# ruiminshen/yolo2-pytorch

Measured on NVIDIA H100. Metric: 416x416 images/sec, higher is better.
Workload: dtype f16

## Files before the change

### include/yolo2_b200.h

```cpp
#ifndef YOLO2_B200_H_
#define YOLO2_B200_H_

#ifdef __cplusplus
extern "C" {
#endif

typedef void* yb_stream_t;

#define YB_ERR_BAD_ARG (-1)
#define YB_ERR_UNSUPPORTED (-2)
#define YB_ERR_DRIVER (-3)

#define YB_OUT_F16_NHWC 0
#define YB_OUT_F32_NCHW 1
#define YB_CONV_A_TILED 1
#define YB_CONV_WIDE_N 2
#define YB_CONV_FORCE_BN(bn) ((bn) << 8)
#define YB_CONV_POOL2X2 16
#define YB_CONV_C32_IM2COL 32
#define YB_CONV_NO_STREAMK 8
#define YB_CONV_FORCE_STREAMK (1 << 30)
#define YB_CONV_NO_SMALLK (1 << 28)
#define YB_CONV_PLAIN_STORE (1 << 29)
#define YB_FILTER_THRESHOLD 0
#define YB_FILTER_FIX 1
#define YB_FILTER_NONE 2

int yb_version(void);
const char* yb_last_error(void);
int yb_debug_read(int out[4]);
int yb_conv_set_trace(void* dev_buf);

int yb_pack_weight_f16(const float* w_oihw, void* w_f16, int cout, int cin, int ksize, int mode, yb_stream_t stream);
int yb_bn_fold(const float* gamma, const float* beta, const float* running_mean, const float* running_var, float eps, float* scale,
               float* shift, int channels, yb_stream_t stream);

int yb_conv0_bn_leaky_pool_fwd(const float* x_nchw, const float* w_oihw, const float* scale, const float* shift, float slope,
                               void* y_nhwc_f16, int batch, int height, int width, int cout, yb_stream_t stream);
int yb_conv0_u8_bn_leaky_pool_fwd(const unsigned char* x_nhwc_u8, const float* w_oihw, const float* scale, const float* shift,
                                  float slope, void* y_nhwc_f16, int batch, int height, int width, int cout, yb_stream_t stream);
int yb_conv_bn_act_fwd(const void* x, const void* w, const float* scale, const float* shift, float slope, void* y, int batch,
                       int height, int width, int cin, int cout, int ksize, int x_ld, long long y_ld, int y_ch_off, int out_mode,
                       int flags, yb_stream_t stream);
int yb_conv_bn_act_stats_fwd(const void* x, const void* w, const float* scale, const float* shift, float slope, void* y, int batch,
                             int height, int width, int cin, int cout, int ksize, int x_ld, long long y_ld, int y_ch_off, int flags,
                             double* sums, yb_stream_t stream);
long long yb_conv_workspace_bytes(void);
int yb_conv_choice(int batch, int height, int width, int cin, int cout, int ksize, int out_mode, int flags, int with_workspace, int out[6]);
int yb_conv_bn_act_fwd_ws(const void* x, const void* w, const float* scale, const float* shift, float slope, void* y, int batch,
                          int height, int width, int cin, int cout, int ksize, int x_ld, long long y_ld, int y_ch_off, int out_mode,
                          int flags, void* workspace, long long workspace_bytes, yb_stream_t stream);
int yb_conv_bn_act_split_fwd(const void* x, const void* w_split, const float* scale, const float* shift, float slope, void* y, int batch,
                             int height, int width, int k_channels, int a_channels, int cout, int ksize, int x_ld, long long y_ld,
                             int y_ch_off, int lo_ch_off, int out_mode, int flags, void* workspace, long long workspace_bytes,
                             yb_stream_t stream);
int yb_pack_weight_split_f16(const float* w_oihw, void* w_f16, int cout, int cin, int ksize, int segments, int lo_mask, yb_stream_t stream);
int yb_maxpool2x2_split_f16(const void* x, void* y, int batch, int height, int width, int channels, int x_ld, int x_lo_off, int y_ld,
                            int y_lo_off, yb_stream_t stream);
int yb_conv_ref_fwd(const void* x, const void* w, const float* scale, const float* shift, float slope, void* y, int batch, int height,
                    int width, int cin, int cout, int ksize, int x_ld, long long y_ld, int y_ch_off, int out_mode, yb_stream_t stream);
int yb_maxpool2x2_f16(const void* x, void* y, int batch, int height, int width, int channels, int x_ld, yb_stream_t stream);
int yb_maxpool2x2_s1_f16(const void* x, void* y, int batch, int height, int width, int channels, int x_ld, yb_stream_t stream);
int yb_maxpool2x2_s1_bwd_f16(const void* x, const void* dy, void* dx, int batch, int height, int width, int channels, yb_stream_t stream);
int yb_reorg_f16(const void* x, void* y, int batch, int height, int width, int channels, int x_ld, int y_ld, int y_ch_off,
                 yb_stream_t stream);
int yb_reorg_f32_nchw(const float* x, float* y, int batch, int channels, int height, int width, int stride_h, int stride_w,
                      yb_stream_t stream);

int yb_decode_fwd(const float* feature, const float* anchors_hw, float* iou, float* center_offset, float* size_norm, float* yx_min,
                  float* yx_max, float* logits, float* prob, int batch, int rows, int cols, int num_anchors, int num_cls,
                  yb_stream_t stream);

int yb_filter_nms(const float* score, const float* yx_min, const float* yx_max, const float* prob, int batch, int n, int num_cls,
                  int mode, float threshold, float threshold_cls, float overlap, int limit, int* n_filtered, int* n_keep,
                  int* keep_idx, int* keep_box, int* n_det, int* det_keep, int* det_cls, float* det_score, int det_cap,
                  int* filt_box, int* best_cls, float* best_prob, yb_stream_t stream);
int yb_iou_matrix(const float* yx_min1, const float* yx_max1, const float* yx_min2, const float* yx_max2, float* out, int batch,
                  int n1, int n2, float min_union, yb_stream_t stream);

int yb_region_loss_fwd(const float* feature, const float* anchors_hw, const float* gt_yx_min, const float* gt_yx_max,
                       const long long* gt_cls, int batch, int rows, int cols, int num_anchors, int num_cls, int num_gt, float threshold,
                       int cross_entropy, float* losses, unsigned char* positive, unsigned char* negative, float* best_iou, int* pos_count,
                       float* partial, float* grad_terms, float* grad_bg, yb_stream_t stream);
int yb_region_loss_bwd(const float* grad_terms, const float* grad_bg, const float* weights5, float* dfeature, int batch, int rows, int cols,
                       int num_anchors, int num_cls, yb_stream_t stream);

int yb_conv0_raw_fwd(const float* x_nchw, const float* w_oihw, void* z_nhwc_f16, int batch, int height, int width, int cout,
                     yb_stream_t stream);
int yb_conv0_raw_stats_fwd(const float* x_nchw, const float* w_oihw, void* z_nhwc_f16, double* sums, int batch, int height, int width, int cout,
                           yb_stream_t stream);
int yb_pack_weight_dgrad_f16(const float* w_oihw, void* w_f16, int cout, int cin, int ksize, int cout_pad, yb_stream_t stream);
typedef struct yb_pack_unit {
  const float* w_oihw;
  void* out_fwd;
  void* out_dgrad;
  int cout, cin, ksize, cout_pad, block0, ci_blocks;
} yb_pack_unit;
int yb_pack_weights_batch(const yb_pack_unit* units_dev, int num_units, int total_blocks, yb_stream_t stream);
int yb_bn_stats(const void* z, long long ld, long long rows, int channels, double* sums, yb_stream_t stream);
int yb_bn_finalize(double* sums, long long rows, int channels, float eps, float momentum, float* running_mean, float* running_var,
                   float* mean, float* invstd, yb_stream_t stream);
int yb_bn_act_apply(const void* z, long long ld_z, const float* mean, const float* invstd, const float* gamma, const float* beta,
                    float slope, void* a, long long ld_a, int a_ch_off, int batch, int height, int width, int channels, int pool,
                    yb_stream_t stream);
int yb_bn_act_bwd(int mode, const void* z, long long ld_z, const float* mean, const float* invstd, const float* gamma, const float* beta,
                  float slope, const void* da, long long ld_da, int da_off, const void* dap, long long ld_dap, int dap_off, int batch,
                  int height, int width, int channels, int window, double* sums, void* dz, long long ld_dz, int has_bn, yb_stream_t stream);
int yb_bn_param_grad(double* sums, int channels, float* dgamma, float* dbeta, int reset, float scale, yb_stream_t stream);
int yb_reorg_bwd_f16(const void* dy, long long ld_dy, int dy_off, void* dx, int batch, int height, int width, int channels,
                     yb_stream_t stream);
int yb_head_grad_prepare(const float* dfeature, void* dz_nhwc_f16, float* dbias, int batch, int channels, int channels_pad, int cells,
                         yb_stream_t stream);
int yb_conv0_wgrad(const float* x_nchw, const void* dz_nhwc_f16, float* dw_oihw, int batch, int height, int width, yb_stream_t stream);
int yb_conv0_wgrad_bn(const float* x_nchw, const void* z_nhwc_f16, const void* dap, long long ld_dap, int dap_off, const float* mean, const float* invstd,
                      const float* gamma, const float* beta, float slope, const double* sums, float* dw_oihw, int batch, int height, int width,
                      yb_stream_t stream);
int yb_conv_wgrad(const void* x, const void* dz, float* dw_krsc, int batch, int height, int width, int cin, int cout, int ksize, int x_ld,
                  int dz_ld, yb_stream_t stream);
int yb_unpack_wgrad(const float* dw_krsc, float* dw_oihw, int cout, int cin, int ksize, float scale, yb_stream_t stream);

int yb_grad_guard(float* grads, long long count, float* found_inf, int zero_if_found, yb_stream_t stream);

int yb_resize_batch_u8(const void* src, const long long* src_off, const int* src_hw, void* dst, int batch, int height, int width, int swap_rb,
                       float* yx_min, float* yx_max, int slots, yb_stream_t stream);

int yb_resize_aug_batch_u8(const void* src, const long long* src_off, const int* src_hw, const int* crop, const float* margin, const unsigned char* flip,
                           void* dst, int batch, int height, int width, int swap_rb, float* yx_min, float* yx_max, int slots, yb_stream_t stream);

int yb_warp_affine_u8(const void* src, int src_h, int src_w, void* dst, int dst_h, int dst_w, const double* inverse_matrix6, const int* fill3,
                      yb_stream_t stream);

int yb_totensor_u8(const void* src_nhwc_u8, float* dst_nchw_f32, int batch, int height, int width, yb_stream_t stream);

#define YB_PH_BLUR 1
#define YB_PH_SWAP 2
#define YB_PH_BGR2HSV 3
#define YB_PH_HSV2RGB 4
#define YB_PH_LUT 5
int yb_photometric_batch_u8(const void* src, void* dst, int batch, int height, int width, const void* params, int param_stride, int stages,
                            yb_stream_t stream);

int yb_eval_match(const float* det_yx_min, const float* det_yx_max, const int* det_cls, const int* det_off, const float* gt_yx_min,
                  const float* gt_yx_max, const int* gt_cls, const int* gt_off, int batch, int num_cls, int max_gt, float threshold, float min_union,
                  unsigned char* tp, yb_stream_t stream);

int yb_mb_conv0_bn_relu_fwd(const float* x_nchw, const float* w_oihw, const float* scale, const float* shift, void* y_nhwc_f16, int batch,
                            int height, int width, yb_stream_t stream);
int yb_dwconv3x3_bn_relu_fwd(const void* x, const float* w_c9, const float* scale, const float* shift, void* y, int batch, int height,
                             int width, int channels, int stride, yb_stream_t stream);

int yb_stem7x7_bn_relu_fwd(const float* x_nchw, const float* w_oihw, const float* scale, const float* shift, void* y_nhwc_f16, int batch, int height, int width,
                           yb_stream_t stream);
int yb_maxpool3x3_s2_f16(const void* x, void* y, int batch, int height, int width, int channels, yb_stream_t stream);
int yb_subsample2_f16(const void* x, void* y, int batch, int height, int width, int channels, yb_stream_t stream);
int yb_add_relu_f16(const void* a, const void* b, void* out, long long count, yb_stream_t stream);

int yb_conv1x1_preact_fwd(const void* x, const void* w, const float* pre_scale, const float* pre_shift, int pre_relu, const float* scale,
                          const float* shift, float slope, void* y, int batch, int height, int width, int cin, int cout, int x_ld, long long y_ld,
                          int y_ch_off, int out_mode, int flags, void* workspace, long long workspace_bytes, yb_stream_t stream);
int yb_bn_relu_avgpool2x2_f16(const void* x, int x_ld, const float* scale, const float* shift, void* y, int batch, int height, int width,
                              int channels, yb_stream_t stream);
int yb_maxpool3x3_s2_ld_f16(const void* x, void* y, int y_ld, int y_ch_off, int batch, int height, int width, int channels, yb_stream_t stream);

int yb_stem7x7_raw_fwd(const float* x_nchw, const float* w_oihw, void* z_nhwc_f16, int batch, int height, int width, yb_stream_t stream);
int yb_stem7x7_wgrad(const float* x_nchw, const void* dz_nhwc_f16, float* dw_oihw, int batch, int height, int width, yb_stream_t stream);
int yb_maxpool3x3_s2_bwd_f16(const void* x, const void* dy, void* dx, int batch, int height, int width, int channels, yb_stream_t stream);
int yb_upsample2_zero_f16(const void* x, void* y, int batch, int height, int width, int channels, yb_stream_t stream);
int yb_residual_bwd_f16(const void* y, const void* g_a, const void* g_b, int stride_b, void* out, int batch, int height, int width, int channels,
                        yb_stream_t stream);

int yb_mb_conv0_split_fwd(const float* x_nchw, const float* w_oihw, const float* scale, const float* shift, void* y_hi_lo, int batch, int height, int width,
                          yb_stream_t stream);
int yb_dwconv3x3_split_fwd(const void* x_hi_lo, const float* w_c9, const float* scale, const float* shift, void* y_hi_lo, int batch, int height, int width,
                           int channels, int stride, yb_stream_t stream);
int yb_mb_conv0_raw_fwd(const float* x_nchw, const float* w_oihw, void* z_nhwc_f16, int batch, int height, int width, yb_stream_t stream);
int yb_mb_conv0_wgrad(const float* x_nchw, const void* dz_nhwc_f16, float* dw_oihw, int batch, int height, int width, yb_stream_t stream);
int yb_dwconv3x3_raw_fwd(const void* x, const float* w_c9, void* z, int batch, int height, int width, int channels, int stride, yb_stream_t stream);
int yb_dwconv3x3_dgrad(const void* dz, const float* w_c9, void* da, int batch, int height, int width, int channels, int stride, yb_stream_t stream);
int yb_dwconv3x3_wgrad(const void* a, const void* dz, float* dw_c9, int batch, int height, int width, int channels, int stride, yb_stream_t stream);

int yb_comm_version(int* nccl_version);
int yb_comm_unique_id(void* id128);
int yb_comm_init(void** comm, int nranks, const void* id128, int rank);
int yb_comm_destroy(void* comm);
int yb_allreduce_bucket(void* comm, void* buf, long long count, int dtype, yb_stream_t stream);
int yb_broadcast_buffer(void* comm, void* buf, long long count, int dtype, int root, yb_stream_t stream);

#ifdef __cplusplus
}
#endif
#endif
```

### yolo2-pytorch_b200/b200/engine.py

```python
import os

import torch

from . import ops

STRICT_KEEP = {'layers1.0': 'aw', 'layers1.2': 'aw', 'layers1.4': 'a', 'passthrough': 'aw', 'layers3.0': 'aw'}
PRECISIONS = ('fast', 'strict')


class ConvUnit(object):

    def __init__(self, conv, bn, act):
        self.conv, self.bn, self.act = conv, bn, act
        self._wver = None
        self._bver = None
        self.w16 = self.scale = self.shift = None
        self.split_a = self.split_w = False
        self.out_lo = False

    @property
    def cout(self):
        return self.conv.weight.shape[0]

    @property
    def cin(self):
        return self.conv.weight.shape[1]

    @property
    def ksize(self):
        return self.conv.weight.shape[2]

    @property
    def slope(self):
        return 0.1 if self.act else 1.0

    def refresh(self, first_layer=False, force=False):
        w = self.conv.weight
        wver = (w.data_ptr(), w._version)
        wver = wver + (self.split_a, self.split_w)
        if force or wver != self._wver:
            if first_layer:
                self.w16 = w.detach().contiguous()
            elif self.split_a or self.split_w:
                self.w16 = ops.pack_weight_split_f16(w.detach().contiguous(), self.split_a, self.split_w)
            else:
                self.w16 = ops.pack_weight_f16(w.detach().contiguous(), 0)
            self._wver = wver
        if self.bn is not None:
            ts = (self.bn.weight, self.bn.bias, self.bn.running_mean, self.bn.running_var)
            bver = tuple((t.data_ptr(), t._version) for t in ts)
            if bver != self._bver:
                self.scale, self.shift = ops.bn_fold(*(t.detach().contiguous() for t in ts), eps=self.bn.eps)
                self._bver = bver
        else:
            b = self.conv.bias
            bver = None if b is None else (b.data_ptr(), b._version)
            if bver != self._bver or self.scale is None:
                self.scale = torch.ones(self.cout, dtype=torch.float32, device=w.device)
                self.shift = (b.detach().float().contiguous().clone() if b is not None
                              else torch.zeros(self.cout, dtype=torch.float32, device=w.device))
                self._bver = bver


class StrictPlan(object):

    def __init__(self, eng, batch, height, width, device):
        f16 = dict(dtype=torch.float16, device=device)

        def buf(u, h, w):
            return torch.empty(batch, h, w, u.cout * (2 if u.out_lo else 1), **f16)

        h, w = height // 2, width // 2
        self.a0 = torch.empty(batch, h, w, eng.units1[0].cout, **f16)
        self.l1 = []
        for u, pooled in zip(eng.units1[1:], eng.pools1[1:]):
            out = buf(u, h, w)
            if pooled:
                h, w = h // 2, w // 2
                self.l1.append((out, buf(u, h, w)))
            else:
                self.l1.append((out, None))
        self.pt = buf(eng.unit_pt, h, w)
        h, w = h // 2, w // 2
        self.x1_pool = buf(eng.units1[-1], h, w)
        self.cat_c = eng.unit_pt.cout * 4 + eng.units2[-1].cout
        self.cat = torch.empty(batch, h, w, self.cat_c * (2 if eng.units3[0].split_a else 1), **f16)
        self.l2 = [buf(u, h, w) for u in eng.units2[:-1]]
        self.l3 = buf(eng.units3[0], h, w)
        self.feature = torch.empty(batch, eng.units3[1].cout, h, w, dtype=torch.float32, device=device)
        self.workspace = ops.conv_workspace(device)


class DarknetPlan(object):

    def __init__(self, units1, units2, unit_pt, units3, pools1, batch, height, width, device):
        f16 = dict(dtype=torch.float16, device=device)
        self.batch, self.height, self.width = batch, height, width
        h, w = height // 2, width // 2
        self.a0 = torch.empty(batch, h, w, units1[0].cout, **f16)
        self.l1 = []
        for u, pooled in zip(units1[1:], pools1[1:]):
            out = torch.empty(batch, h, w, u.cout, **f16)
            if pooled:
                h, w = h // 2, w // 2
                self.l1.append((out, torch.empty(batch, h, w, u.cout, **f16)))
            else:
                self.l1.append((out, None))
        self.h16, self.w16 = h, w
        self.pt = torch.empty(batch, h, w, unit_pt.cout, **f16)
        self.x1_pool = torch.empty(batch, h // 2, w // 2, units1[-1].cout, **f16)
        h, w = h // 2, w // 2
        self.h32, self.w32 = h, w
        self.cat_ch = unit_pt.cout * 4 + units2[-1].cout
        self.cat = torch.empty(batch, h, w, self.cat_ch, **f16)
        self.l2 = [torch.empty(batch, h, w, u.cout, **f16) for u in units2[:-1]]
        self.l3 = torch.empty(batch, h, w, units3[0].cout, **f16)
        self.feature = torch.empty(batch, units3[1].cout, h, w, dtype=torch.float32, device=device)
        self.workspace = ops.conv_workspace(device)


class DarknetEngine(object):
    def __init__(self, dnn):
        def unit(m):
            return ConvUnit(m.conv, m.bn if m.has_bn else None, m.has_act)

        self.units1, self.pools1, self._k1 = [], [], []
        mods = list(dnn.layers1)
        for i, m in enumerate(mods):
            if m.is_pool:
                continue
            self.units1.append(unit(m))
            self.pools1.append(i + 1 < len(mods) and mods[i + 1].is_pool)
            self._k1.append('layers1.%d' % i)
        self.units2 = [unit(m) for m in dnn.layers2 if not m.is_pool]
        self._k2 = ['layers2.%d' % i for i, m in enumerate(dnn.layers2) if not m.is_pool]
        self.unit_pt = unit(dnn.passthrough)
        self.units3 = [unit(m) for m in dnn.layers3]
        self.plans = {}
        if not self.pools1[0]:
            raise RuntimeError('Darknet: layers1.0 must be followed by MaxPool2d (fused first-layer kernel)')
        self.precision = 'fast'
        self.set_precision(os.environ.get('YB_PRECISION', 'fast'))

    def unit_keys(self):
        return self._k1 + self._k2 + ['passthrough', 'layers3.0', 'layers3.1']

    def set_precision(self, precision, keep=None):
        if precision not in PRECISIONS:
            raise ValueError('precision must be one of %s' % (PRECISIONS,))
        keep = STRICT_KEEP if keep is None else keep
        units = dict(zip(self.unit_keys(), self.all_units()))
        for key, u in units.items():
            k = keep.get(key, '') if precision == 'strict' else 'aw'
            u.split_a, u.split_w, u.out_lo = 'a' not in k, 'w' not in k, False
        units[self._k1[0]].split_a = units[self._k1[0]].split_w = False
        units[self._k1[1]].split_a = False
        chain1 = self.units1
        for prev, nxt in zip(chain1[:-1], chain1[1:]):
            prev.out_lo = nxt.split_a
        chain1[-1].out_lo = self.unit_pt.split_a or self.units2[0].split_a
        for prev, nxt in zip(self.units2[:-1], self.units2[1:]):
            prev.out_lo = nxt.split_a
        self.units2[-1].out_lo = self.unit_pt.out_lo = self.units3[0].split_a
        self.units3[0].out_lo = self.units3[1].split_a
        chain1[0].out_lo = False
        self.precision = precision
        self.plans = {}
        self.invalidate()

    def all_units(self):
        return self.units1 + self.units2 + [self.unit_pt] + self.units3

    def plan(self, batch, height, width, device, plan_id=0):
        key = (batch, height, width, str(device), plan_id)
        p = self.plans.get(key)
        if p is None and self.precision == 'strict':
            p = self.plans[key] = StrictPlan(self, batch, height, width, device)
        if p is None:
            p = DarknetPlan(self.units1, self.units2, self.unit_pt, self.units3, self.pools1, batch, height, width, device)
            self.plans[key] = p
        return p

    def refresh(self, force=False):
        for i, u in enumerate(self.all_units()):
            u.refresh(first_layer=(i == 0), force=force)

    def invalidate(self):
        for u in self.all_units():
            u._wver = None
            u._bver = None

    def forward(self, x, conv_flags=0, ref=False, collect=None, plan_id=0):
        if not x.is_cuda:
            raise RuntimeError('Darknet: input must be a CUDA tensor; there is no CPU fallback')
        u8 = x.dtype == torch.uint8
        if u8:
            b, h, w, c = x.shape
        else:
            b, c, h, w = x.shape
        if c != 3 or h % 32 or w % 32:
            raise ValueError('Darknet expects fp32 [B,3,H,W] or uint8 [B,H,W,3] with H, W multiples of 32, got %s' % (tuple(x.shape),))
        x = x.contiguous() if u8 else x.contiguous().float()
        self.refresh()
        p = self.plan(b, h, w, x.device, plan_id)
        if self.precision == 'strict':
            return self._forward_strict(x, u8, p, conv_flags, collect)

        def conv(u, src, dst, **kw):
            return ops.conv_bn_act(src, u.w16, u.scale, u.shift, u.slope, out=dst, flags=conv_flags, ref=ref, workspace=p.workspace, **kw)

        u0 = self.units1[0]
        conv0 = ops.conv0_u8_bn_leaky_pool if u8 else ops.conv0_bn_leaky_pool
        cur = conv0(x, u0.w16, u0.scale, u0.shift, u0.slope, out=p.a0)
        if collect is not None:
            collect['layers1.0(pooled)'] = cur
        x1 = None
        last1 = self.units1[-1]
        for u, (out, pooled), key in zip(self.units1[1:], p.l1, self._k1[1:]):
            fuse_pool = (pooled is not None and u is not last1 and collect is None and not ref and u.cin == 32 and u.ksize == 3
                         and u.cout <= 64 and (conv_flags & (ops.CONV_NO_SMALLK | ops.CONV_C32_IM2COL)) == 0 and conv_flags < 256)
            if fuse_pool:
                ops.conv_bn_act(cur, u.w16, u.scale, u.shift, u.slope, out=pooled, flags=conv_flags | ops.CONV_POOL2X2)
                cur = pooled
                continue
            conv(u, cur, out)
            if collect is not None:
                collect[key] = out
            x1 = out
            cur = ops.maxpool2x2(out, out=pooled) if pooled is not None else out
        conv(self.unit_pt, x1, p.pt)
        if collect is not None:
            collect['passthrough'] = p.pt
        ops.reorg_f16(p.pt, p.cat, 0)
        cur = ops.maxpool2x2(x1, out=p.x1_pool)
        for u, out, key in zip(self.units2[:-1], p.l2, self._k2):
            conv(u, cur, out)
            if collect is not None:
                collect[key] = out
            cur = out
        conv(self.units2[-1], cur, p.cat, y_ch_off=self.unit_pt.cout * 4)
        conv(self.units3[0], p.cat, p.l3)
        conv(self.units3[1], p.l3, p.feature, out_mode=ops.OUT_F32_NCHW)
        if collect is not None:
            collect['cat'] = p.cat
            collect['layers3.0'] = p.l3
        return p.feature

    def _forward_strict(self, x, u8, p, conv_flags, collect):
        def view(t, c, lo):
            return (t[..., :c].float() + t[..., c:2 * c].float()) if lo else t[..., :c]

        def conv(u, src, src_c, src_lo, dst, y_ch_off=0, lo_ch_off=None, out_mode=ops.OUT_F16_NHWC):
            split_a = u.split_a and src_lo
            if lo_ch_off is None:
                lo_ch_off = y_ch_off + u.cout if u.out_lo else -1
            if not (split_a or u.split_w or lo_ch_off >= 0):
                return ops.conv_bn_act(src, u.w16, u.scale, u.shift, u.slope, out=dst, flags=conv_flags, workspace=p.workspace, cin=src_c,
                                       y_ch_off=y_ch_off, out_mode=out_mode)
            if u.split_a and not src_lo:
                raise RuntimeError('strict plan: unit expects [hi | lo] input')
            return ops.conv_bn_act_split(src, u.w16, u.scale, u.shift, u.slope, dst, a_channels=src_c * (2 if split_a else 1), y_ch_off=y_ch_off,
                                         lo_ch_off=lo_ch_off, out_mode=out_mode, flags=conv_flags, workspace=p.workspace)

        u0 = self.units1[0]
        conv0 = ops.conv0_u8_bn_leaky_pool if u8 else ops.conv0_bn_leaky_pool
        cur, cur_c, cur_lo = conv0(x, u0.w16, u0.scale, u0.shift, u0.slope, out=p.a0), u0.cout, False
        if collect is not None:
            collect['layers1.0(pooled)'] = cur
        x1 = None
        for u, (out, pooled), key in zip(self.units1[1:], p.l1, self._k1[1:]):
            plain = not (u.split_a or u.split_w or u.out_lo)
            if (plain and pooled is not None and collect is None and u.cin == 32 and u.ksize == 3 and u.cout <= 64 and conv_flags == 0):
                ops.conv_bn_act(cur, u.w16, u.scale, u.shift, u.slope, out=pooled, flags=ops.CONV_POOL2X2)
                cur, cur_c, cur_lo = pooled, u.cout, False
                continue
            conv(u, cur, cur_c, cur_lo, out)
            if collect is not None:
                collect[key] = view(out, u.cout, u.out_lo)
            x1, x1_c, x1_lo = out, u.cout, u.out_lo
            cur, cur_c, cur_lo = out, u.cout, u.out_lo
            if pooled is not None:
                cur = ops.maxpool2x2_split(out, u.cout, pooled) if u.out_lo else ops.maxpool2x2(out, out=pooled)
        cat_lo = self.units3[0].split_a
        upt = self.unit_pt
        conv(upt, x1, x1_c, x1_lo, p.pt)
        if collect is not None:
            collect['passthrough'] = view(p.pt, upt.cout, upt.out_lo)
        ops.reorg_f16(p.pt, p.cat, 0, channels=upt.cout)
        if cat_lo:
            ops.reorg_f16(p.pt, p.cat, p.cat_c, channels=upt.cout, x_ch_off=upt.cout)
        last1 = self.units1[-1]
        cur = ops.maxpool2x2_split(x1, last1.cout, p.x1_pool) if last1.out_lo else ops.maxpool2x2(x1, out=p.x1_pool)
        cur_c, cur_lo = last1.cout, last1.out_lo
        for u, out, key in zip(self.units2[:-1], p.l2, self._k2):
            conv(u, cur, cur_c, cur_lo, out)
            if collect is not None:
                collect[key] = view(out, u.cout, u.out_lo)
            cur, cur_c, cur_lo = out, u.cout, u.out_lo
        u27 = self.units2[-1]
        conv(u27, cur, cur_c, cur_lo, p.cat, y_ch_off=upt.cout * 4, lo_ch_off=(p.cat_c + upt.cout * 4) if cat_lo else -1)
        u30, u31 = self.units3
        conv(u30, p.cat, p.cat_c, cat_lo, p.l3)
        conv(u31, p.l3, u30.cout, u30.out_lo, p.feature, out_mode=ops.OUT_F32_NCHW, lo_ch_off=-1)
        if collect is not None:
            collect['cat'] = view(p.cat, p.cat_c, cat_lo)
            collect['layers3.0'] = view(p.l3, u30.cout, u30.out_lo)
        return p.feature
```

### yolo2-pytorch_b200/b200/lib.py

```python
import ctypes
import os

_HERE = os.path.dirname(os.path.abspath(__file__))
LIB_PATH = os.environ.get('YB_LIB_PATH') or os.path.join(os.path.dirname(_HERE), 'libyolo2_b200.so')

c_int, c_float, c_void_p, c_longlong = ctypes.c_int, ctypes.c_float, ctypes.c_void_p, ctypes.c_longlong
P = c_void_p

SIGNATURES = {
    'yb_version': [],
    'yb_debug_read': [ctypes.POINTER(c_int * 4)],
    'yb_conv_set_trace': [P],
    'yb_pack_weight_f16': [P, P, c_int, c_int, c_int, c_int, P],
    'yb_bn_fold': [P, P, P, P, c_float, P, P, c_int, P],
    'yb_conv0_bn_leaky_pool_fwd': [P, P, P, P, c_float, P, c_int, c_int, c_int, c_int, P],
    'yb_conv0_u8_bn_leaky_pool_fwd': [P, P, P, P, c_float, P, c_int, c_int, c_int, c_int, P],
    'yb_conv_bn_act_fwd': [P, P, P, P, c_float, P, c_int, c_int, c_int, c_int, c_int, c_int, c_int, c_longlong, c_int, c_int, c_int, P],
    'yb_conv_bn_act_stats_fwd': [P, P, P, P, c_float, P, c_int, c_int, c_int, c_int, c_int, c_int, c_int, c_longlong, c_int, c_int, P, P],
    'yb_conv_workspace_bytes': [],
    'yb_conv_choice': [c_int, c_int, c_int, c_int, c_int, c_int, c_int, c_int, c_int, ctypes.POINTER(c_int * 6)],
    'yb_conv_bn_act_fwd_ws': [P, P, P, P, c_float, P, c_int, c_int, c_int, c_int, c_int, c_int, c_int, c_longlong, c_int, c_int, c_int, P,
                              c_longlong, P],
    'yb_conv_bn_act_split_fwd': [P, P, P, P, c_float, P, c_int, c_int, c_int, c_int, c_int, c_int, c_int, c_int, c_longlong, c_int, c_int, c_int,
                                 c_int, P, c_longlong, P],
    'yb_pack_weight_split_f16': [P, P, c_int, c_int, c_int, c_int, c_int, P],
    'yb_maxpool2x2_split_f16': [P, P, c_int, c_int, c_int, c_int, c_int, c_int, c_int, c_int, P],
    'yb_conv_ref_fwd': [P, P, P, P, c_float, P, c_int, c_int, c_int, c_int, c_int, c_int, c_int, c_longlong, c_int, c_int, P],
    'yb_maxpool2x2_f16': [P, P, c_int, c_int, c_int, c_int, c_int, P],
    'yb_maxpool2x2_s1_f16': [P, P, c_int, c_int, c_int, c_int, c_int, P],
    'yb_maxpool2x2_s1_bwd_f16': [P, P, P, c_int, c_int, c_int, c_int, P],
    'yb_reorg_f16': [P, P, c_int, c_int, c_int, c_int, c_int, c_int, c_int, P],
    'yb_reorg_f32_nchw': [P, P, c_int, c_int, c_int, c_int, c_int, c_int, P],
    'yb_decode_fwd': [P, P, P, P, P, P, P, P, P, c_int, c_int, c_int, c_int, c_int, P],
    'yb_filter_nms': [P, P, P, P, c_int, c_int, c_int, c_int, c_float, c_float, c_float, c_int, P, P, P, P, P, P, P, P, c_int, P, P, P, P],
    'yb_iou_matrix': [P, P, P, P, P, c_int, c_int, c_int, c_float, P],
    'yb_region_loss_fwd': [P, P, P, P, P, c_int, c_int, c_int, c_int, c_int, c_int, c_float, c_int, P, P, P, P, P, P, P, P, P],
    'yb_region_loss_bwd': [P, P, P, P, c_int, c_int, c_int, c_int, c_int, P],
    'yb_conv0_raw_fwd': [P, P, P, c_int, c_int, c_int, c_int, P],
    'yb_conv0_raw_stats_fwd': [P, P, P, P, c_int, c_int, c_int, c_int, P],
    'yb_pack_weight_dgrad_f16': [P, P, c_int, c_int, c_int, c_int, P],
    'yb_pack_weights_batch': [P, c_int, c_int, P],
    'yb_bn_stats': [P, c_longlong, c_longlong, c_int, P, P],
    'yb_bn_finalize': [P, c_longlong, c_int, c_float, c_float, P, P, P, P, P],
    'yb_bn_act_apply': [P, c_longlong, P, P, P, P, c_float, P, c_longlong, c_int, c_int, c_int, c_int, c_int, c_int, P],
    'yb_bn_act_bwd': [c_int, P, c_longlong, P, P, P, P, c_float, P, c_longlong, c_int, P, c_longlong, c_int, c_int, c_int, c_int, c_int, c_int,
                      P, P, c_longlong, c_int, P],
    'yb_bn_param_grad': [P, c_int, P, P, c_int, c_float, P],
    'yb_reorg_bwd_f16': [P, c_longlong, c_int, P, c_int, c_int, c_int, c_int, P],
    'yb_head_grad_prepare': [P, P, P, c_int, c_int, c_int, c_int, P],
    'yb_conv0_wgrad': [P, P, P, c_int, c_int, c_int, P],
    'yb_conv0_wgrad_bn': [P, P, P, c_longlong, c_int, P, P, P, P, c_float, P, P, c_int, c_int, c_int, P],
    'yb_conv_wgrad': [P, P, P, c_int, c_int, c_int, c_int, c_int, c_int, c_int, c_int, P],
    'yb_unpack_wgrad': [P, P, c_int, c_int, c_int, c_float, P],
    'yb_grad_guard': [P, c_longlong, P, c_int, P],
    'yb_resize_batch_u8': [P, P, P, P, c_int, c_int, c_int, c_int, P, P, c_int, P],
    'yb_resize_aug_batch_u8': [P, P, P, P, P, P, P, c_int, c_int, c_int, c_int, P, P, c_int, P],
    'yb_warp_affine_u8': [P, c_int, c_int, P, c_int, c_int, ctypes.POINTER(ctypes.c_double * 6), ctypes.POINTER(c_int * 3), P],
    'yb_totensor_u8': [P, P, c_int, c_int, c_int, P],
    'yb_photometric_batch_u8': [P, P, c_int, c_int, c_int, P, c_int, c_int, P],
    'yb_eval_match': [P, P, P, P, P, P, P, P, c_int, c_int, c_int, c_float, c_float, P, P],
    'yb_mb_conv0_raw_fwd': [P, P, P, c_int, c_int, c_int, P],
    'yb_mb_conv0_split_fwd': [P, P, P, P, P, c_int, c_int, c_int, P],
    'yb_dwconv3x3_split_fwd': [P, P, P, P, P, c_int, c_int, c_int, c_int, c_int, P],
    'yb_mb_conv0_wgrad': [P, P, P, c_int, c_int, c_int, P],
    'yb_dwconv3x3_raw_fwd': [P, P, P, c_int, c_int, c_int, c_int, c_int, P],
    'yb_dwconv3x3_dgrad': [P, P, P, c_int, c_int, c_int, c_int, c_int, P],
    'yb_dwconv3x3_wgrad': [P, P, P, c_int, c_int, c_int, c_int, c_int, P],
    'yb_stem7x7_bn_relu_fwd': [P, P, P, P, P, c_int, c_int, c_int, P],
    'yb_maxpool3x3_s2_f16': [P, P, c_int, c_int, c_int, c_int, P],
    'yb_subsample2_f16': [P, P, c_int, c_int, c_int, c_int, P],
    'yb_add_relu_f16': [P, P, P, c_longlong, P],
    'yb_stem7x7_raw_fwd': [P, P, P, c_int, c_int, c_int, P],
    'yb_stem7x7_wgrad': [P, P, P, c_int, c_int, c_int, P],
    'yb_maxpool3x3_s2_bwd_f16': [P, P, P, c_int, c_int, c_int, c_int, P],
    'yb_upsample2_zero_f16': [P, P, c_int, c_int, c_int, c_int, P],
    'yb_residual_bwd_f16': [P, P, P, c_int, P, c_int, c_int, c_int, c_int, P],
    'yb_comm_version': [ctypes.POINTER(c_int)],
    'yb_comm_unique_id': [P],
    'yb_comm_init': [ctypes.POINTER(P), c_int, P, c_int],
    'yb_comm_destroy': [P],
    'yb_allreduce_bucket': [P, P, c_longlong, c_int, P],
    'yb_broadcast_buffer': [P, P, c_longlong, c_int, c_int, P],
    'yb_mb_conv0_bn_relu_fwd': [P, P, P, P, P, c_int, c_int, c_int, P],
    'yb_dwconv3x3_bn_relu_fwd': [P, P, P, P, P, c_int, c_int, c_int, c_int, c_int, P],
    'yb_conv1x1_preact_fwd': [P, P, P, P, c_int, P, P, c_float, P, c_int, c_int, c_int, c_int, c_int, c_int, c_longlong, c_int, c_int, c_int, P,
                              c_longlong, P],
    'yb_bn_relu_avgpool2x2_f16': [P, c_int, P, P, P, c_int, c_int, c_int, c_int, P],
    'yb_maxpool3x3_s2_ld_f16': [P, P, c_int, c_int, c_int, c_int, c_int, c_int, P],
}

_lib = None


def load():
    global _lib
    if _lib is not None:
        return _lib
    if not os.path.exists(LIB_PATH):
        raise ImportError(
            'libyolo2_b200.so not found at %s -- build it with `python yolo2-pytorch_b200/build.py` '
            '(nvcc, sm_90a).  There is no CPU or PyTorch fallback for this path.' % LIB_PATH)
    lib = ctypes.CDLL(LIB_PATH)
    for name, argtypes in SIGNATURES.items():
        fn = getattr(lib, name)
        fn.argtypes = argtypes
        fn.restype = c_longlong if name == 'yb_conv_workspace_bytes' else c_int
    lib.yb_last_error.argtypes = []
    lib.yb_last_error.restype = ctypes.c_char_p
    _lib = lib
    return lib


def last_error():
    return load().yb_last_error().decode('utf-8', 'replace')


def debug_read():
    buf = (c_int * 4)()
    load().yb_debug_read(ctypes.byref(buf))
    return list(buf)


def check(rc, what):
    if rc != 0:
        raise RuntimeError('%s failed (code %d): %s' % (what, rc, last_error()))
```

### yolo2-pytorch_b200/b200/ops.py

```python
import ctypes

import torch

from . import lib as _l

OUT_F16_NHWC, OUT_F32_NCHW = 0, 1
CONV_A_TILED, CONV_WIDE_N = 1, 2
CONV_NO_STREAMK, CONV_FORCE_STREAMK, CONV_NO_SMALLK, CONV_PLAIN_STORE = 8, 1 << 30, 1 << 28, 1 << 29
CONV_POOL2X2, CONV_C32_IM2COL, CONV_C32_SWAP = 16, 32, 64
FILTER_THRESHOLD, FILTER_FIX, FILTER_NONE = 0, 1, 2


launch_count = 0


def _ck(rc, what):
    global launch_count
    _l.check(rc, what)
    launch_count += 1


def conv_force_bn(bn):
    return bn << 8


def conv_force_mt(mt):
    return mt << 20


def conv_force_pair(v):
    return v << 22


CONV_ALLOW_PAIR = 4


def _p(t):
    return None if t is None else ctypes.c_void_p(t.data_ptr())


def _s():
    return ctypes.c_void_p(torch.cuda.current_stream().cuda_stream)


def _req(t, dtype, name):
    if not (isinstance(t, torch.Tensor) and t.is_cuda):
        raise RuntimeError('%s must be a CUDA tensor: the GPU path has no CPU fallback' % name)
    if t.dtype != dtype:
        raise TypeError('%s must be %s, got %s' % (name, dtype, t.dtype))
    if not t.is_contiguous():
        raise ValueError('%s must be contiguous' % name)
    return t


def pack_weight_f16(w, mode=0):
    _req(w, torch.float32, 'weight')
    cout, cin, k, _ = w.shape
    shape = (cout, k, k, cin) if mode == 0 else (cin, k, k, cout)
    out = torch.empty(shape, dtype=torch.float16, device=w.device)
    _ck(_l.load().yb_pack_weight_f16(_p(w), _p(out), cout, cin, k, mode, _s()), 'yb_pack_weight_f16')
    return out


SPLIT_SEGMENTS = {(True, False): (2, 0b00), (False, True): (2, 0b10), (True, True): (3, 0b100)}


def pack_weight_split_f16(w, split_a, split_w):
    _req(w, torch.float32, 'weight')
    cout, cin, k, _ = w.shape
    segments, lo_mask = SPLIT_SEGMENTS[(bool(split_a), bool(split_w))]
    out = torch.empty(cout, k, k, segments * cin, dtype=torch.float16, device=w.device)
    _ck(_l.load().yb_pack_weight_split_f16(_p(w), _p(out), cout, cin, k, segments, lo_mask, _s()), 'yb_pack_weight_split_f16')
    return out


def bn_fold(gamma, beta, mean, var, eps=1e-5):
    for n, t in (('gamma', gamma), ('beta', beta), ('mean', mean), ('var', var)):
        _req(t, torch.float32, n)
    c = gamma.numel()
    scale = torch.empty(c, dtype=torch.float32, device=gamma.device)
    shift = torch.empty_like(scale)
    _ck(_l.load().yb_bn_fold(_p(gamma), _p(beta), _p(mean), _p(var), float(eps), _p(scale), _p(shift), c, _s()), 'yb_bn_fold')
    return scale, shift


def conv0_bn_leaky_pool(x, w, scale, shift, slope, out=None):
    _req(x, torch.float32, 'x'); _req(w, torch.float32, 'w'); _req(scale, torch.float32, 'scale'); _req(shift, torch.float32, 'shift')
    b, c, h, wd = x.shape
    if c != 3:
        raise ValueError('conv0 expects 3 input channels')
    cout = w.shape[0]
    if out is None:
        out = torch.empty(b, h // 2, wd // 2, cout, dtype=torch.float16, device=x.device)
    _req(out, torch.float16, 'out')
    _ck(_l.load().yb_conv0_bn_leaky_pool_fwd(_p(x), _p(w), _p(scale), _p(shift), float(slope), _p(out), b, h, wd, cout, _s()),
             'yb_conv0_bn_leaky_pool_fwd')
    return out


def conv0_u8_bn_leaky_pool(x, w, scale, shift, slope, out=None):
    _req(x, torch.uint8, 'x'); _req(w, torch.float32, 'w'); _req(scale, torch.float32, 'scale'); _req(shift, torch.float32, 'shift')
    b, h, wd, c = x.shape
    if c != 3:
        raise ValueError('conv0 expects 3 input channels')
    cout = w.shape[0]
    if out is None:
        out = torch.empty(b, h // 2, wd // 2, cout, dtype=torch.float16, device=x.device)
    _req(out, torch.float16, 'out')
    _ck(_l.load().yb_conv0_u8_bn_leaky_pool_fwd(_p(x), _p(w), _p(scale), _p(shift), float(slope), _p(out), b, h, wd, cout, _s()),
        'yb_conv0_u8_bn_leaky_pool_fwd')
    return out


def _conv_common(fn_name, x, w, scale, shift, slope, out, batch, height, width, cin, cout, k, x_ld, y_ld, y_ch_off, out_mode, flags,
                 workspace=None):
    if workspace is not None and fn_name == 'yb_conv_bn_act_fwd':
        fn_name = 'yb_conv_bn_act_fwd_ws'
    fn = getattr(_l.load(), fn_name)
    args = [_p(x), _p(w), _p(scale), _p(shift), float(slope), _p(out), batch, height, width, cin, cout, k, x_ld, y_ld, y_ch_off, out_mode]
    if fn_name != 'yb_conv_ref_fwd':
        args.append(flags)
    if fn_name == 'yb_conv_bn_act_fwd_ws':
        _req(workspace, torch.uint8, 'workspace')
        args += [_p(workspace), workspace.numel()]
    args.append(_s())
    _ck(fn(*args), fn_name)


def conv_workspace(device='cuda'):
    return torch.zeros(int(_l.load().yb_conv_workspace_bytes()), dtype=torch.uint8, device=device)


CONV_KERNELS = ('conv_igemm_kernel', 'conv_wide_kernel', 'conv_c32_kernel')


def conv_choice(batch, height, width, cin, cout, k, out_mode=OUT_F16_NHWC, flags=0, workspace=True):
    out = (ctypes.c_int * 6)()
    _l.check(_l.load().yb_conv_choice(batch, height, width, cin, cout, k, out_mode, flags, int(bool(workspace)), ctypes.byref(out)),
             'yb_conv_choice')
    return dict(kernel=CONV_KERNELS[out[0]], bk=out[1], bn=out[2], rows=out[3], streamk=bool(out[4]), grid=out[5])


def conv_bn_act(x, w, scale, shift, slope, out=None, out_mode=OUT_F16_NHWC, y_ch_off=0, cin=None, flags=0, ref=False, workspace=None):
    _req(x, torch.float16, 'x'); _req(w, torch.float16, 'w'); _req(scale, torch.float32, 'scale'); _req(shift, torch.float32, 'shift')
    b, h, wd, x_ld = x.shape
    cout, k, _, wcin = w.shape
    cin = wcin if cin is None else cin
    if cin != wcin:
        raise ValueError('weight Cin %d != %d' % (wcin, cin))
    if out is None:
        oh, ow = (h // 2, wd // 2) if (flags & CONV_POOL2X2) else (h, wd)
        out = (torch.empty(b, oh, ow, cout, dtype=torch.float16, device=x.device) if out_mode == OUT_F16_NHWC
               else torch.empty(b, cout, h, wd, dtype=torch.float32, device=x.device))
    if out_mode == OUT_F16_NHWC:
        _req(out, torch.float16, 'out')
        y_ld = out.shape[-1]
    else:
        _req(out, torch.float32, 'out')
        y_ld = 0
    _conv_common('yb_conv_ref_fwd' if ref else 'yb_conv_bn_act_fwd', x, w, scale, shift, slope, out, b, h, wd, cin, cout, k, x_ld, y_ld,
                 y_ch_off, out_mode, flags, workspace=None if ref else workspace)
    return out


def conv1x1_preact(x, w, pre_scale, pre_shift, pre_relu, scale, shift, slope, out=None, out_mode=OUT_F16_NHWC, y_ch_off=0, cin=None, flags=0,
                   workspace=None):
    _req(x, torch.float16, 'x'); _req(w, torch.float16, 'w'); _req(scale, torch.float32, 'scale'); _req(shift, torch.float32, 'shift')
    _req(pre_scale, torch.float32, 'pre_scale'); _req(pre_shift, torch.float32, 'pre_shift')
    b, h, wd, x_ld = x.shape
    cout, k, _, wcin = w.shape
    cin = wcin if cin is None else cin
    if cin != wcin or k != 1:
        raise ValueError('conv1x1_preact: weight [%d,%d,%d,%d] does not match a 1x1 conv over %d channels' % (cout, k, k, wcin, cin))
    if pre_scale.numel() < cin or pre_shift.numel() < cin:
        raise ValueError('conv1x1_preact: pre_scale / pre_shift need %d channels' % cin)
    if out is None:
        out = (torch.empty(b, h, wd, cout, dtype=torch.float16, device=x.device) if out_mode == OUT_F16_NHWC
               else torch.empty(b, cout, h, wd, dtype=torch.float32, device=x.device))
    if out_mode == OUT_F16_NHWC:
        _req(out, torch.float16, 'out')
        y_ld = out.shape[-1]
    else:
        _req(out, torch.float32, 'out')
        y_ld = 0
    ws_ptr, ws_bytes = (None, 0) if workspace is None else (_p(_req(workspace, torch.uint8, 'workspace')), workspace.numel())
    _ck(_l.load().yb_conv1x1_preact_fwd(_p(x), _p(w), _p(pre_scale), _p(pre_shift), int(bool(pre_relu)), _p(scale), _p(shift), float(slope),
                                        _p(out), b, h, wd, cin, cout, x_ld, y_ld, y_ch_off, out_mode, flags, ws_ptr, ws_bytes, _s()),
        'yb_conv1x1_preact_fwd')
    return out


def conv_bn_act_split(x, w, scale, shift, slope, out, a_channels, y_ch_off=0, lo_ch_off=-1, out_mode=OUT_F16_NHWC, flags=0, workspace=None):
    _req(x, torch.float16, 'x'); _req(w, torch.float16, 'w'); _req(scale, torch.float32, 'scale'); _req(shift, torch.float32, 'shift')
    b, h, wd, x_ld = x.shape
    cout, k, _, kch = w.shape
    if out_mode == OUT_F16_NHWC:
        _req(out, torch.float16, 'out')
        y_ld = out.shape[-1]
    else:
        _req(out, torch.float32, 'out')
        y_ld = 0
    ws_ptr, ws_bytes = (None, 0) if workspace is None else (_p(_req(workspace, torch.uint8, 'workspace')), workspace.numel())
    _ck(_l.load().yb_conv_bn_act_split_fwd(_p(x), _p(w), _p(scale), _p(shift), float(slope), _p(out), b, h, wd, kch, int(a_channels), cout, k, x_ld,
                                           y_ld, y_ch_off, lo_ch_off, out_mode, flags, ws_ptr, ws_bytes, _s()), 'yb_conv_bn_act_split_fwd')
    return out


def maxpool2x2_split(x, channels, out):
    _req(x, torch.float16, 'x'); _req(out, torch.float16, 'out')
    b, h, w, x_ld = x.shape
    _ck(_l.load().yb_maxpool2x2_split_f16(_p(x), _p(out), b, h, w, channels, x_ld, channels, out.shape[-1], channels, _s()), 'yb_maxpool2x2_split_f16')
    return out


def conv_bn_act_stats(x, w, scale, shift, slope, sums, out=None, flags=0):
    _req(x, torch.float16, 'x'); _req(w, torch.float16, 'w'); _req(scale, torch.float32, 'scale'); _req(shift, torch.float32, 'shift')
    _req(sums, torch.float64, 'sums')
    b, h, wd, x_ld = x.shape
    cout, k, _, cin = w.shape
    if sums.numel() != 2 * cout:
        raise ValueError('sums must hold 2 * Cout doubles')
    if out is None:
        out = torch.empty(b, h, wd, cout, dtype=torch.float16, device=x.device)
    _req(out, torch.float16, 'out')
    _ck(_l.load().yb_conv_bn_act_stats_fwd(_p(x), _p(w), _p(scale), _p(shift), float(slope), _p(out), b, h, wd, cin, cout, k, x_ld, out.shape[-1], 0,
                                           flags, _p(sums), _s()), 'yb_conv_bn_act_stats_fwd')
    return out


def maxpool2x2(x, channels=None, out=None):
    _req(x, torch.float16, 'x')
    b, h, w, x_ld = x.shape
    c = x_ld if channels is None else channels
    if out is None:
        out = torch.empty(b, h // 2, w // 2, c, dtype=torch.float16, device=x.device)
    _req(out, torch.float16, 'out')
    _ck(_l.load().yb_maxpool2x2_f16(_p(x), _p(out), b, h, w, c, x_ld, _s()), 'yb_maxpool2x2_f16')
    return out


def maxpool2x2_s1(x, out=None):
    _req(x, torch.float16, 'x')
    b, h, w, c = x.shape
    if out is None:
        out = torch.empty_like(x)
    _req(out, torch.float16, 'out')
    _ck(_l.load().yb_maxpool2x2_s1_f16(_p(x), _p(out), b, h, w, c, c, _s()), 'yb_maxpool2x2_s1_f16')
    return out


def reorg_f16(x, out, y_ch_off=0, channels=None, x_ch_off=0):
    _req(x, torch.float16, 'x'); _req(out, torch.float16, 'out')
    b, h, w, x_ld = x.shape
    c = x_ld if channels is None else channels
    if x_ch_off % 8 or x_ch_off + c > x_ld:
        raise ValueError('reorg: bad channel slice')
    xp = ctypes.c_void_p(x.data_ptr() + 2 * x_ch_off)
    _ck(_l.load().yb_reorg_f16(xp, _p(out), b, h, w, c, x_ld, out.shape[-1], y_ch_off, _s()), 'yb_reorg_f16')
    return out


def reorg_f32_nchw(x, stride_h=2, stride_w=2):
    _req(x, torch.float32, 'x')
    b, c, h, w = x.shape
    out = torch.empty(b, c * stride_h * stride_w, h // stride_h, w // stride_w, dtype=torch.float32, device=x.device)
    if out.numel():
        _ck(_l.load().yb_reorg_f32_nchw(_p(x), _p(out), b, c, h, w, stride_h, stride_w, _s()), 'yb_reorg_f32_nchw')
    return out


def decode(feature, anchors, num_cls, with_prob=True):
    _req(feature, torch.float32, 'feature'); _req(anchors, torch.float32, 'anchors')
    b, ch, rows, cols = feature.shape
    a = anchors.shape[0]
    cells = rows * cols
    dev = feature.device
    out = dict(
        iou=torch.empty(b, cells, a, dtype=torch.float32, device=dev),
        center_offset=torch.empty(b, cells, a, 2, dtype=torch.float32, device=dev),
        size_norm=torch.empty(b, cells, a, 2, dtype=torch.float32, device=dev),
        yx_min=torch.empty(b, cells, a, 2, dtype=torch.float32, device=dev),
        yx_max=torch.empty(b, cells, a, 2, dtype=torch.float32, device=dev),
    )
    logits = prob = None
    if num_cls > 1:
        logits = out['logits'] = torch.empty(b, cells, a, num_cls, dtype=torch.float32, device=dev)
    if with_prob:
        prob = out['prob'] = torch.empty(b, cells, a, max(num_cls, 1), dtype=torch.float32, device=dev)
    if ch != a * (5 + (num_cls if num_cls > 1 else 0)):
        raise ValueError('feature has %d channels, expected %d' % (ch, a * (5 + (num_cls if num_cls > 1 else 0))))
    _ck(_l.load().yb_decode_fwd(_p(feature), _p(anchors), _p(out['iou']), _p(out['center_offset']), _p(out['size_norm']),
                                     _p(out['yx_min']), _p(out['yx_max']), _p(logits), _p(prob), b, rows, cols, a, num_cls, _s()),
             'yb_decode_fwd')
    return out


def filter_nms(score, yx_min, yx_max, prob, mode, threshold, threshold_cls, overlap, limit=200, expand=False, details=False):
    _req(score, torch.float32, 'score'); _req(yx_min, torch.float32, 'yx_min'); _req(yx_max, torch.float32, 'yx_max')
    if prob is not None:
        _req(prob, torch.float32, 'prob')
    b, n = score.shape
    num_cls = prob.shape[-1] if prob is not None else 1
    dev = score.device
    i32 = dict(dtype=torch.int32, device=dev)
    res = dict(n_filtered=torch.empty(b, **i32), n_keep=torch.empty(b, **i32),
               keep_idx=torch.empty(b, limit, **i32), keep_box=torch.empty(b, limit, **i32))
    n_det = det_keep = det_cls = det_score = None
    det_cap = 0
    if expand:
        det_cap = limit * num_cls
        n_det = res['n_det'] = torch.empty(b, **i32)
        det_keep = res['det_keep'] = torch.empty(b, det_cap, **i32)
        det_cls = res['det_cls'] = torch.empty(b, det_cap, **i32)
        det_score = res['det_score'] = torch.empty(b, det_cap, dtype=torch.float32, device=dev)
    filt_box = best_cls = best_prob = None
    if details:
        filt_box = res['filt_box'] = torch.empty(b, n, **i32)
        if prob is not None:
            best_cls = res['best_cls'] = torch.empty(b, n, **i32)
            best_prob = res['best_prob'] = torch.empty(b, n, dtype=torch.float32, device=dev)
    _ck(_l.load().yb_filter_nms(_p(score), _p(yx_min), _p(yx_max), _p(prob), b, n, num_cls, mode, float(threshold),
                                     float(threshold_cls), float(overlap), limit, _p(res['n_filtered']), _p(res['n_keep']),
                                     _p(res['keep_idx']), _p(res['keep_box']), _p(n_det), _p(det_keep), _p(det_cls), _p(det_score),
                                     det_cap, _p(filt_box), _p(best_cls), _p(best_prob), _s()), 'yb_filter_nms')
    return res


def iou_matrix(yx_min1, yx_max1, yx_min2, yx_max2, min_union=1.1920928955078125e-07):
    for n, t in (('yx_min1', yx_min1), ('yx_max1', yx_max1), ('yx_min2', yx_min2), ('yx_max2', yx_max2)):
        _req(t, torch.float32, n)
    batched = yx_min1.dim() == 3
    b = yx_min1.shape[0] if batched else 1
    n1, n2 = yx_min1.shape[-2], yx_min2.shape[-2]
    out = torch.empty((b, n1, n2) if batched else (n1, n2), dtype=torch.float32, device=yx_min1.device)
    _ck(_l.load().yb_iou_matrix(_p(yx_min1), _p(yx_max1), _p(yx_min2), _p(yx_max2), _p(out), b, n1, n2, float(min_union), _s()),
             'yb_iou_matrix')
    return out


def region_loss_forward(feature, anchors, gt_yx_min, gt_yx_max, gt_cls, threshold, cross_entropy=True):
    _req(feature, torch.float32, 'feature'); _req(anchors, torch.float32, 'anchors')
    _req(gt_yx_min, torch.float32, 'gt_yx_min'); _req(gt_yx_max, torch.float32, 'gt_yx_max')
    b, ch, rows, cols = feature.shape
    a = anchors.shape[0]
    per = ch // a
    num_cls = per - 5 if per > 5 else 1
    g = gt_yx_min.shape[1]
    if num_cls > 1:
        _req(gt_cls, torch.int64, 'gt_cls')
    cells = rows * cols
    dev = feature.device
    out = dict(losses=torch.empty(5, dtype=torch.float32, device=dev),
               positive=torch.empty(b, cells, a, dtype=torch.uint8, device=dev),
               negative=torch.empty(b, cells, a, dtype=torch.uint8, device=dev),
               best_iou=torch.empty(b, cells, a, dtype=torch.float32, device=dev),
               grad_terms=torch.empty_like(feature),
               grad_bg=torch.empty(b, a, cells, dtype=torch.float32, device=dev))
    pos_count = torch.empty(b, dtype=torch.int32, device=dev)
    partial = torch.empty(b * 5, dtype=torch.float32, device=dev)
    _ck(_l.load().yb_region_loss_fwd(_p(feature), _p(anchors), _p(gt_yx_min), _p(gt_yx_max), _p(gt_cls if num_cls > 1 else None), b, rows,
                                     cols, a, num_cls, g, float(threshold), int(bool(cross_entropy)), _p(out['losses']),
                                     _p(out['positive']), _p(out['negative']), _p(out['best_iou']), _p(pos_count), _p(partial),
                                     _p(out['grad_terms']), _p(out['grad_bg']), _s()), 'yb_region_loss_fwd')
    out['pos_count'] = pos_count
    return out


def region_loss_backward(grad_terms, grad_bg, weights5, num_anchors):
    _req(grad_terms, torch.float32, 'grad_terms'); _req(grad_bg, torch.float32, 'grad_bg'); _req(weights5, torch.float32, 'weights5')
    b, ch, rows, cols = grad_terms.shape
    per = ch // num_anchors
    num_cls = per - 5 if per > 5 else 1
    out = torch.empty_like(grad_terms)
    _ck(_l.load().yb_region_loss_bwd(_p(grad_terms), _p(grad_bg), _p(weights5), _p(out), b, rows, cols, num_anchors, num_cls, _s()),
        'yb_region_loss_bwd')
    return out


def call(name, *args):
    conv = [(_p(a) if isinstance(a, torch.Tensor) or a is None else a) for a in args]
    _ck(getattr(_l.load(), name)(*conv, _s()), name)
```

### yolo2-pytorch_b200/b200/pipeline.py

```python
import torch

from . import ops


class DetectPipeline(object):
    RESULT_KEYS = ('n_filtered', 'n_keep', 'keep_box', 'n_det', 'det_keep', 'det_cls', 'det_score', 'best_cls', 'iou', 'yx_min', 'yx_max')

    def __init__(self, inference, config, batch, height, width, slots=2, lanes=1, use_graph=True, limit=200, device=None, uint8_input=False):
        self.inference = inference
        self.dnn = inference.dnn
        self.engine = self.dnn.engine
        self.config = config
        self.batch, self.height, self.width = batch, height, width
        self.device = torch.device('cuda', torch.cuda.current_device()) if device is None else device
        self.limit = limit
        self.fix = config.getboolean('detect', 'fix')
        self.mode = ops.FILTER_FIX if self.fix else ops.FILTER_THRESHOLD
        self.threshold = 0.0 if self.fix else config.getfloat('detect', 'threshold')
        self.threshold_cls = config.getfloat('detect', 'threshold_cls') if self.fix else 0.0
        self.overlap = config.getfloat('detect', 'overlap')
        self.anchors = inference.anchors.detach().to(device=self.device, dtype=torch.float32).contiguous()
        if uint8_input:
            self.x = [torch.zeros(batch, height, width, 3, dtype=torch.uint8, device=self.device) for _ in range(slots)]
        else:
            self.x = [torch.zeros(batch, 3, height, width, dtype=torch.float32, device=self.device) for _ in range(slots)]
        self.lanes = max(1, min(lanes, slots))
        self.streams = [torch.cuda.Stream(device=self.device) for _ in range(self.lanes)]
        self.out = [None] * slots
        self.graphs = [None] * slots
        self.host = [None] * slots
        self.use_graph = use_graph
        self.copy_stream = torch.cuda.Stream(device=self.device)
        self.loaded = [None] * slots
        self.done = [None] * slots
        self.launches_per_run = None

    def lane_of(self, slot):
        return slot % self.lanes

    def _forward(self, x, plan_id=0):
        feature = self.engine.forward(x, plan_id=plan_id)
        a = self.anchors.size(0)
        per = feature.size(1) // a
        num_cls = per - 5 if per > 5 else 1
        dec = ops.decode(feature, self.anchors, num_cls, with_prob=True)
        b = feature.size(0)
        n = dec['iou'][0].numel()
        res = ops.filter_nms(dec['iou'].view(b, n), dec['yx_min'].view(b, n, 2), dec['yx_max'].view(b, n, 2),
                             dec['prob'].view(b, n, -1), self.mode, self.threshold, self.threshold_cls, self.overlap, self.limit,
                             expand=True, details=True)
        out = dict(feature=feature)
        out.update(dec)
        out.update(res)
        return out

    def prepare(self):
        cur = torch.cuda.current_stream(self.device)
        for lane, st in enumerate(self.streams):
            st.wait_stream(cur)
            with torch.cuda.stream(st):
                for _ in range(2):
                    before = ops.launch_count
                    self.out[lane] = self._forward(self.x[lane], plan_id=lane)
                    self.launches_per_run = ops.launch_count - before
            cur.wait_stream(st)
        torch.cuda.synchronize(self.device)
        if self.use_graph:
            for s in range(len(self.x)):
                g = torch.cuda.CUDAGraph()
                with torch.cuda.graph(g, stream=self.streams[self.lane_of(s)]):
                    self.out[s] = self._forward(self.x[s], plan_id=self.lane_of(s))
                self.graphs[s] = g
            torch.cuda.synchronize(self.device)
        return self

    def load(self, slot, host_tensor):
        if self.done[slot] is not None:
            self.copy_stream.wait_event(self.done[slot])
        with torch.cuda.stream(self.copy_stream):
            self.x[slot].copy_(host_tensor, non_blocking=True)
            ev = torch.cuda.Event()
            ev.record(self.copy_stream)
        self.loaded[slot] = ev

    def run(self, slot, fetch=False):
        st = self.streams[self.lane_of(slot)]
        if self.loaded[slot] is not None:
            st.wait_event(self.loaded[slot])
            self.loaded[slot] = None
        with torch.cuda.stream(st):
            if self.graphs[slot] is not None:
                self.graphs[slot].replay()
            else:
                self.out[slot] = self._forward(self.x[slot], plan_id=self.lane_of(slot))
            if fetch:
                self._fetch(slot)
            ev = torch.cuda.Event()
            ev.record(st)
        self.done[slot] = ev
        return self.out[slot]

    def _fetch(self, slot):
        out = self.out[slot]
        if self.host[slot] is None:
            self.host[slot] = {k: torch.empty(out[k].shape, dtype=out[k].dtype, pin_memory=True) for k in self.RESULT_KEYS}
        for k in self.RESULT_KEYS:
            self.host[slot][k].copy_(out[k], non_blocking=True)
        return self.host[slot]

    def fetch(self, slot):
        st = self.streams[self.lane_of(slot)]
        with torch.cuda.stream(st):
            host = self._fetch(slot)
            ev = torch.cuda.Event()
            ev.record(st)
        self.done[slot] = ev
        return host

    def wait_all(self, stream=None):
        stream = torch.cuda.current_stream(self.device) if stream is None else stream
        for st in self.streams:
            stream.wait_stream(st)

    def start_after(self, event):
        for st in self.streams:
            st.wait_event(event)
        self.copy_stream.wait_event(event)

    def result_bytes(self):
        out = self.out[0]
        return sum(out[k].numel() * out[k].element_size() for k in self.RESULT_KEYS)

    def detections(self, host, bi):
        nk = int(host['n_keep'][bi])
        if nk == 0:
            return None
        kbox = host['keep_box'][bi, :nk].long()
        iou = host['iou'][bi].reshape(-1)[kbox]
        yx_min, yx_max = host['yx_min'][bi].reshape(-1, 2), host['yx_max'][bi].reshape(-1, 2)
        if not self.fix:
            return iou, yx_min[kbox], yx_max[kbox], host['best_cls'][bi][kbox].long(), iou
        nd = int(host['n_det'][bi])
        dbox = kbox[host['det_keep'][bi, :nd].long()]
        return iou, yx_min[dbox], yx_max[dbox], host['det_cls'][bi, :nd].long(), host['det_score'][bi, :nd]
```

### yolo2-pytorch_b200/csrc/capi.cu

```cuda
#include "../../include/yolo2_b200.h"
#include "yb_common.h"
#include <stdarg.h>
#include <stdint.h>

namespace yb {

char* err_buf() {
  static thread_local char buf[512] = {0};
  return buf;
}

int fail(int code, const char* fmt, ...) {
  va_list ap;
  va_start(ap, fmt);
  vsnprintf(err_buf(), 512, fmt, ap);
  va_end(ap);
  return code;
}

int check_launch(const char* what) {
  const cudaError_t e = cudaGetLastError();
  if (e != cudaSuccess) return fail(static_cast<int>(e), "%s: %s", what, cudaGetErrorString(e));
  return 0;
}

int sm_count() {
  static int cached[64] = {0};
  int dev = 0;
  if (cudaGetDevice(&dev) != cudaSuccess || dev < 0 || dev >= 64) return 132;
  if (cached[dev] == 0) {
    int n = 0;
    if (cudaDeviceGetAttribute(&n, cudaDevAttrMultiProcessorCount, dev) != cudaSuccess || n <= 0) n = 132;
    cached[dev] = n;
  }
  return cached[dev];
}

static int* g_dbg_host = nullptr;
static int* g_dbg_dev = nullptr;

int* debug_word_device() {
  static bool tried = false;
  if (!tried) {
    tried = true;
    void* h = nullptr;
    if (cudaHostAlloc(&h, 4 * sizeof(int), cudaHostAllocMapped) == cudaSuccess) {
      memset(h, 0, 4 * sizeof(int));
      void* d = nullptr;
      if (cudaHostGetDevicePointer(&d, h, 0) == cudaSuccess) {
        g_dbg_host = static_cast<int*>(h);
        g_dbg_dev = static_cast<int*>(d);
      }
    } else {
      cudaGetLastError();
    }
  }
  return g_dbg_dev;
}

long long conv_workspace_bytes();
int conv_choice(int, int, int, int, int, int, int, int, int, int*);
int conv_igemm_forward(const void*, const void*, const float*, const float*, float, void*, int, int, int, int, int, int, int, long long,
                       int, int, int, void*, long long, double*, int, int, const float*, const float*, int, cudaStream_t);
int bn_relu_avgpool2x2(const void*, int, const float*, const float*, void*, int, int, int, int, cudaStream_t);
int maxpool3x3_s2_ld(const void*, void*, int, int, int, int, int, int, cudaStream_t);
int pack_weight_split(const float*, void*, int, int, int, int, int, cudaStream_t);
int maxpool2x2_split(const void*, void*, int, int, int, int, int, int, int, int, cudaStream_t);
int conv_ref_forward(const void*, const void*, const float*, const float*, float, void*, int, int, int, int, int, int, int, long long,
                     int, int, cudaStream_t);
int pack_weight(const float*, void*, int, int, int, int, int, cudaStream_t);
int pack_weights_batch(const void*, int, int, cudaStream_t);
void conv_set_trace(void*);
int bn_fold(const float*, const float*, const float*, const float*, float, float*, float*, int, cudaStream_t);
int conv0_tc_forward(const void*, int, const float*, const float*, const float*, float, void*, int, int, int, int, int, double*, cudaStream_t);
int maxpool2x2(const void*, void*, int, int, int, int, int, cudaStream_t);
int maxpool2x2_s1(const void*, void*, int, int, int, int, int, cudaStream_t);
int maxpool2x2_s1_bwd(const void*, const void*, void*, int, int, int, int, cudaStream_t);
int reorg_nhwc(const void*, void*, int, int, int, int, int, int, int, cudaStream_t);
int reorg_nchw(const float*, float*, int, int, int, int, int, int, cudaStream_t);
int decode_forward(const float*, const float*, float*, float*, float*, float*, float*, float*, float*, int, int, int, int, int,
                   cudaStream_t);
int filter_nms(const float*, const float*, const float*, const float*, int, int, int, int, float, float, float, int, int*, int*, int*,
               int*, int*, int*, int*, float*, int, int*, int*, float*, cudaStream_t);
int iou_matrix(const float*, const float*, const float*, const float*, float*, int, int, int, float, cudaStream_t);
int region_loss_forward(const float*, const float*, const float*, const float*, const long long*, int, int, int, int, int, int, float, int,
                        float*, unsigned char*, unsigned char*, float*, int*, float*, float*, float*, cudaStream_t);
int region_loss_backward(const float*, const float*, const float*, float*, int, int, int, int, int, cudaStream_t);
int bn_stats(const void*, long long, long long, int, double*, cudaStream_t);
int bn_finalize(double*, long long, int, float, float, float*, float*, float*, float*, cudaStream_t);
int bn_act_apply(const void*, long long, const float*, const float*, const float*, const float*, float, void*, long long, int, int, int, int, int,
                 int, cudaStream_t);
int bn_act_bwd(int, const void*, long long, const float*, const float*, const float*, const float*, float, const void*, long long, int,
               const void*, long long, int, int, int, int, int, int, double*, void*, long long, int, cudaStream_t);
int bn_param_grad(double*, int, float*, float*, int, float, cudaStream_t);
int reorg_bwd(const void*, long long, int, void*, int, int, int, int, cudaStream_t);
int head_grad_prepare(const float*, void*, float*, int, int, int, int, cudaStream_t);
int conv0_wgrad(const float*, const void*, float*, int, int, int, cudaStream_t);
int conv0_wgrad_bn(const float*, const void*, const void*, long long, int, const float*, const float*, const float*, const float*, float, const double*, float*, int, int, int,
                   cudaStream_t);
int resize_batch_u8(const void*, const long long*, const int*, void*, int, int, int, int, float*, float*, int, cudaStream_t);
int totensor_u8(const void*, float*, int, int, int, cudaStream_t);
int photometric_batch_u8(const void*, void*, int, int, int, const void*, int, int, cudaStream_t);
int warp_affine_u8(const void*, int, int, void*, int, int, const double*, const int*, cudaStream_t);
int resize_aug_batch_u8(const void*, const long long*, const int*, const int*, const float*, const unsigned char*, void*, int, int, int, int, float*, float*,
                        int, cudaStream_t);
int eval_match(const float*, const float*, const int*, const int*, const float*, const float*, const int*, const int*, int, int, int, float, float,
               unsigned char*, cudaStream_t);
int unpack_wgrad(const float*, float*, int, int, int, float, cudaStream_t);
int grad_guard(float*, long long, float*, int, cudaStream_t);
int conv_wgrad_forward(const void*, const void*, float*, int, int, int, int, int, int, int, int, cudaStream_t);
int stem7x7(const float*, const float*, const float*, const float*, void*, int, int, int, int, cudaStream_t);
int stem7x7_wgrad(const float*, const void*, float*, int, int, int, cudaStream_t);
int maxpool3x3_s2(const void*, void*, int, int, int, int, cudaStream_t);
int maxpool3x3_s2_bwd(const void*, const void*, void*, int, int, int, int, cudaStream_t);
int subsample2(const void*, void*, int, int, int, int, cudaStream_t);
int upsample2_zero(const void*, void*, int, int, int, int, cudaStream_t);
int add_relu(const void*, const void*, void*, long long, cudaStream_t);
int residual_bwd(const void*, const void*, const void*, int, void*, int, int, int, int, cudaStream_t);
int comm_version(int*);
int comm_unique_id(void*);
int comm_init(void**, int, const void*, int);
int comm_destroy(void*);
int allreduce_bucket(void*, void*, long long, int, cudaStream_t);
int broadcast_buffer(void*, void*, long long, int, int, cudaStream_t);
int mb_conv0(const float*, const float*, const float*, const float*, void*, int, int, int, int, int, cudaStream_t);
int dwconv3x3_split(const void*, const float*, const float*, const float*, void*, int, int, int, int, int, cudaStream_t);
int dwconv3x3(const void*, const float*, const float*, const float*, void*, int, int, int, int, int, int, cudaStream_t);
int dw_dgrad(const void*, const float*, void*, int, int, int, int, int, cudaStream_t);
int dw_wgrad(const void*, const void*, float*, int, int, int, int, int, cudaStream_t);
int mb_conv0_wgrad(const float*, const void*, float*, int, int, int, cudaStream_t);

}

#define S(stream) static_cast<cudaStream_t>(stream)

extern "C" {

int yb_version(void) { return 100; }

const char* yb_last_error(void) { return yb::err_buf(); }

int yb_debug_read(int out[4]) {
  if (out == nullptr) return YB_ERR_BAD_ARG;
  if (yb::g_dbg_host == nullptr) { out[0] = out[1] = out[2] = out[3] = 0; return 0; }
  for (int i = 0; i < 4; ++i) { out[i] = yb::g_dbg_host[i]; yb::g_dbg_host[i] = 0; }
  return 0;
}

int yb_conv_set_trace(void* dev_buf) { yb::conv_set_trace(dev_buf); return 0; }

int yb_pack_weight_f16(const float* w_oihw, void* w_f16, int cout, int cin, int ksize, int mode, yb_stream_t stream) {
  return yb::pack_weight(w_oihw, w_f16, cout, cin, ksize, mode, 0, S(stream));
}

int yb_bn_fold(const float* gamma, const float* beta, const float* running_mean, const float* running_var, float eps, float* scale,
               float* shift, int channels, yb_stream_t stream) {
  return yb::bn_fold(gamma, beta, running_mean, running_var, eps, scale, shift, channels, S(stream));
}

int yb_conv0_bn_leaky_pool_fwd(const float* x_nchw, const float* w_oihw, const float* scale, const float* shift, float slope,
                               void* y_nhwc_f16, int batch, int height, int width, int cout, yb_stream_t stream) {
  return yb::conv0_tc_forward(x_nchw, 0, w_oihw, scale, shift, slope, y_nhwc_f16, batch, height, width, cout, 0, nullptr, S(stream));
}

int yb_conv0_u8_bn_leaky_pool_fwd(const unsigned char* x_nhwc_u8, const float* w_oihw, const float* scale, const float* shift,
                                  float slope, void* y_nhwc_f16, int batch, int height, int width, int cout, yb_stream_t stream) {
  return yb::conv0_tc_forward(x_nhwc_u8, 1, w_oihw, scale, shift, slope, y_nhwc_f16, batch, height, width, cout, 0, nullptr, S(stream));
}

int yb_conv_bn_act_fwd(const void* x, const void* w, const float* scale, const float* shift, float slope, void* y, int batch,
                       int height, int width, int cin, int cout, int ksize, int x_ld, long long y_ld, int y_ch_off, int out_mode,
                       int flags, yb_stream_t stream) {
  return yb::conv_igemm_forward(x, w, scale, shift, slope, y, batch, height, width, cin, cout, ksize, x_ld, y_ld, y_ch_off, out_mode,
                                flags, nullptr, 0, nullptr, 0, -1, nullptr, nullptr, 0, S(stream));
}

int yb_conv_bn_act_stats_fwd(const void* x, const void* w, const float* scale, const float* shift, float slope, void* y, int batch,
                             int height, int width, int cin, int cout, int ksize, int x_ld, long long y_ld, int y_ch_off, int flags,
                             double* sums, yb_stream_t stream) {
  return yb::conv_igemm_forward(x, w, scale, shift, slope, y, batch, height, width, cin, cout, ksize, x_ld, y_ld, y_ch_off, 0, flags, nullptr, 0,
                                sums, 0, -1, nullptr, nullptr, 0, S(stream));
}

long long yb_conv_workspace_bytes(void) { return yb::conv_workspace_bytes(); }

int yb_conv_choice(int batch, int height, int width, int cin, int cout, int ksize, int out_mode, int flags, int with_workspace, int out[6]) {
  return yb::conv_choice(batch, height, width, cin, cout, ksize, out_mode, flags, with_workspace, out);
}

int yb_conv_bn_act_fwd_ws(const void* x, const void* w, const float* scale, const float* shift, float slope, void* y, int batch,
                          int height, int width, int cin, int cout, int ksize, int x_ld, long long y_ld, int y_ch_off, int out_mode,
                          int flags, void* workspace, long long workspace_bytes, yb_stream_t stream) {
  return yb::conv_igemm_forward(x, w, scale, shift, slope, y, batch, height, width, cin, cout, ksize, x_ld, y_ld, y_ch_off, out_mode,
                                flags, workspace, workspace_bytes, nullptr, 0, -1, nullptr, nullptr, 0, S(stream));
}

int yb_conv_bn_act_split_fwd(const void* x, const void* w_split, const float* scale, const float* shift, float slope, void* y, int batch,
                             int height, int width, int k_channels, int a_channels, int cout, int ksize, int x_ld, long long y_ld,
                             int y_ch_off, int lo_ch_off, int out_mode, int flags, void* workspace, long long workspace_bytes,
                             yb_stream_t stream) {
  return yb::conv_igemm_forward(x, w_split, scale, shift, slope, y, batch, height, width, k_channels, cout, ksize, x_ld, y_ld, y_ch_off,
                                out_mode, flags, workspace, workspace_bytes, nullptr, a_channels, lo_ch_off, nullptr, nullptr, 0,
                                S(stream));
}

int yb_conv1x1_preact_fwd(const void* x, const void* w, const float* pre_scale, const float* pre_shift, int pre_relu, const float* scale,
                          const float* shift, float slope, void* y, int batch, int height, int width, int cin, int cout, int x_ld, long long y_ld,
                          int y_ch_off, int out_mode, int flags, void* workspace, long long workspace_bytes, yb_stream_t stream) {
  if (pre_scale == nullptr) return yb::fail(YB_ERR_BAD_ARG, "conv_preact: null pre_scale");
  return yb::conv_igemm_forward(x, w, scale, shift, slope, y, batch, height, width, cin, cout, 1, x_ld, y_ld, y_ch_off, out_mode, flags,
                                workspace, workspace_bytes, nullptr, 0, -1, pre_scale, pre_shift, pre_relu, S(stream));
}

int yb_bn_relu_avgpool2x2_f16(const void* x, int x_ld, const float* scale, const float* shift, void* y, int batch, int height, int width,
                              int channels, yb_stream_t stream) {
  return yb::bn_relu_avgpool2x2(x, x_ld, scale, shift, y, batch, height, width, channels, S(stream));
}

int yb_maxpool3x3_s2_ld_f16(const void* x, void* y, int y_ld, int y_ch_off, int batch, int height, int width, int channels, yb_stream_t stream) {
  return yb::maxpool3x3_s2_ld(x, y, y_ld, y_ch_off, batch, height, width, channels, S(stream));
}

int yb_pack_weight_split_f16(const float* w_oihw, void* w_f16, int cout, int cin, int ksize, int segments, int lo_mask, yb_stream_t stream) {
  return yb::pack_weight_split(w_oihw, w_f16, cout, cin, ksize, segments, lo_mask, S(stream));
}

int yb_maxpool2x2_split_f16(const void* x, void* y, int batch, int height, int width, int channels, int x_ld, int x_lo_off, int y_ld,
                            int y_lo_off, yb_stream_t stream) {
  return yb::maxpool2x2_split(x, y, batch, height, width, channels, x_ld, x_lo_off, y_ld, y_lo_off, S(stream));
}

int yb_conv_ref_fwd(const void* x, const void* w, const float* scale, const float* shift, float slope, void* y, int batch, int height,
                    int width, int cin, int cout, int ksize, int x_ld, long long y_ld, int y_ch_off, int out_mode, yb_stream_t stream) {
  return yb::conv_ref_forward(x, w, scale, shift, slope, y, batch, height, width, cin, cout, ksize, x_ld, y_ld, y_ch_off, out_mode,
                              S(stream));
}

int yb_maxpool2x2_f16(const void* x, void* y, int batch, int height, int width, int channels, int x_ld, yb_stream_t stream) {
  return yb::maxpool2x2(x, y, batch, height, width, channels, x_ld, S(stream));
}

int yb_maxpool2x2_s1_f16(const void* x, void* y, int batch, int height, int width, int channels, int x_ld, yb_stream_t stream) {
  return yb::maxpool2x2_s1(x, y, batch, height, width, channels, x_ld, S(stream));
}

int yb_maxpool2x2_s1_bwd_f16(const void* x, const void* dy, void* dx, int batch, int height, int width, int channels, yb_stream_t stream) {
  return yb::maxpool2x2_s1_bwd(x, dy, dx, batch, height, width, channels, S(stream));
}

int yb_reorg_f16(const void* x, void* y, int batch, int height, int width, int channels, int x_ld, int y_ld, int y_ch_off,
                 yb_stream_t stream) {
  return yb::reorg_nhwc(x, y, batch, height, width, channels, x_ld, y_ld, y_ch_off, S(stream));
}

int yb_reorg_f32_nchw(const float* x, float* y, int batch, int channels, int height, int width, int stride_h, int stride_w,
                      yb_stream_t stream) {
  return yb::reorg_nchw(x, y, batch, channels, height, width, stride_h, stride_w, S(stream));
}

int yb_decode_fwd(const float* feature, const float* anchors_hw, float* iou, float* center_offset, float* size_norm, float* yx_min,
                  float* yx_max, float* logits, float* prob, int batch, int rows, int cols, int num_anchors, int num_cls,
                  yb_stream_t stream) {
  return yb::decode_forward(feature, anchors_hw, iou, center_offset, size_norm, yx_min, yx_max, logits, prob, batch, rows, cols,
                            num_anchors, num_cls, S(stream));
}

int yb_filter_nms(const float* score, const float* yx_min, const float* yx_max, const float* prob, int batch, int n, int num_cls,
                  int mode, float threshold, float threshold_cls, float overlap, int limit, int* n_filtered, int* n_keep,
                  int* keep_idx, int* keep_box, int* n_det, int* det_keep, int* det_cls, float* det_score, int det_cap,
                  int* filt_box, int* best_cls, float* best_prob, yb_stream_t stream) {
  return yb::filter_nms(score, yx_min, yx_max, prob, batch, n, num_cls, mode, threshold, threshold_cls, overlap, limit, n_filtered,
                        n_keep, keep_idx, keep_box, n_det, det_keep, det_cls, det_score, det_cap, filt_box, best_cls, best_prob,
                        S(stream));
}

int yb_iou_matrix(const float* yx_min1, const float* yx_max1, const float* yx_min2, const float* yx_max2, float* out, int batch,
                  int n1, int n2, float min_union, yb_stream_t stream) {
  return yb::iou_matrix(yx_min1, yx_max1, yx_min2, yx_max2, out, batch, n1, n2, min_union, S(stream));
}

int yb_region_loss_fwd(const float* feature, const float* anchors_hw, const float* gt_yx_min, const float* gt_yx_max,
                       const long long* gt_cls, int batch, int rows, int cols, int num_anchors, int num_cls, int num_gt, float threshold,
                       int cross_entropy, float* losses, unsigned char* positive, unsigned char* negative, float* best_iou, int* pos_count,
                       float* partial, float* grad_terms, float* grad_bg, yb_stream_t stream) {
  return yb::region_loss_forward(feature, anchors_hw, gt_yx_min, gt_yx_max, gt_cls, batch, rows, cols, num_anchors, num_cls, num_gt,
                                 threshold, cross_entropy, losses, positive, negative, best_iou, pos_count, partial, grad_terms, grad_bg,
                                 S(stream));
}

int yb_region_loss_bwd(const float* grad_terms, const float* grad_bg, const float* weights5, float* dfeature, int batch, int rows, int cols,
                       int num_anchors, int num_cls, yb_stream_t stream) {
  return yb::region_loss_backward(grad_terms, grad_bg, weights5, dfeature, batch, rows, cols, num_anchors, num_cls, S(stream));
}

int yb_conv0_raw_fwd(const float* x_nchw, const float* w_oihw, void* z_nhwc_f16, int batch, int height, int width, int cout,
                     yb_stream_t stream) {
  return yb::conv0_tc_forward(x_nchw, 0, w_oihw, nullptr, nullptr, 1.f, z_nhwc_f16, batch, height, width, cout, 1, nullptr, S(stream));
}

int yb_conv0_raw_stats_fwd(const float* x_nchw, const float* w_oihw, void* z_nhwc_f16, double* sums, int batch, int height, int width, int cout,
                           yb_stream_t stream) {
  return yb::conv0_tc_forward(x_nchw, 0, w_oihw, nullptr, nullptr, 1.f, z_nhwc_f16, batch, height, width, cout, 1, sums, S(stream));
}

int yb_pack_weights_batch(const yb_pack_unit* units_dev, int num_units, int total_blocks, yb_stream_t stream) {
  return yb::pack_weights_batch(units_dev, num_units, total_blocks, S(stream));
}

int yb_pack_weight_dgrad_f16(const float* w_oihw, void* w_f16, int cout, int cin, int ksize, int cout_pad, yb_stream_t stream) {
  return yb::pack_weight(w_oihw, w_f16, cout, cin, ksize, 1, cout_pad, S(stream));
}

int yb_bn_stats(const void* z, long long ld, long long rows, int channels, double* sums, yb_stream_t stream) {
  return yb::bn_stats(z, ld, rows, channels, sums, S(stream));
}

int yb_bn_finalize(double* sums, long long rows, int channels, float eps, float momentum, float* running_mean, float* running_var,
                   float* mean, float* invstd, yb_stream_t stream) {
  return yb::bn_finalize(sums, rows, channels, eps, momentum, running_mean, running_var, mean, invstd, S(stream));
}

int yb_bn_act_apply(const void* z, long long ld_z, const float* mean, const float* invstd, const float* gamma, const float* beta,
                    float slope, void* a, long long ld_a, int a_ch_off, int batch, int height, int width, int channels, int pool,
                    yb_stream_t stream) {
  return yb::bn_act_apply(z, ld_z, mean, invstd, gamma, beta, slope, a, ld_a, a_ch_off, batch, height, width, channels, pool, S(stream));
}

int yb_bn_act_bwd(int mode, const void* z, long long ld_z, const float* mean, const float* invstd, const float* gamma, const float* beta,
                  float slope, const void* da, long long ld_da, int da_off, const void* dap, long long ld_dap, int dap_off, int batch,
                  int height, int width, int channels, int window, double* sums, void* dz, long long ld_dz, int has_bn, yb_stream_t stream) {
  return yb::bn_act_bwd(mode, z, ld_z, mean, invstd, gamma, beta, slope, da, ld_da, da_off, dap, ld_dap, dap_off, batch, height, width,
                        channels, window, sums, dz, ld_dz, has_bn, S(stream));
}

int yb_bn_param_grad(double* sums, int channels, float* dgamma, float* dbeta, int reset, float scale, yb_stream_t stream) {
  return yb::bn_param_grad(sums, channels, dgamma, dbeta, reset, scale, S(stream));
}

int yb_reorg_bwd_f16(const void* dy, long long ld_dy, int dy_off, void* dx, int batch, int height, int width, int channels,
                     yb_stream_t stream) {
  return yb::reorg_bwd(dy, ld_dy, dy_off, dx, batch, height, width, channels, S(stream));
}

int yb_head_grad_prepare(const float* dfeature, void* dz_nhwc_f16, float* dbias, int batch, int channels, int channels_pad, int cells,
                         yb_stream_t stream) {
  return yb::head_grad_prepare(dfeature, dz_nhwc_f16, dbias, batch, channels, channels_pad, cells, S(stream));
}

int yb_conv0_wgrad(const float* x_nchw, const void* dz_nhwc_f16, float* dw_oihw, int batch, int height, int width, yb_stream_t stream) {
  return yb::conv0_wgrad(x_nchw, dz_nhwc_f16, dw_oihw, batch, height, width, S(stream));
}

int yb_conv0_wgrad_bn(const float* x_nchw, const void* z_nhwc_f16, const void* dap, long long ld_dap, int dap_off, const float* mean, const float* invstd,
                      const float* gamma, const float* beta, float slope, const double* sums, float* dw_oihw, int batch, int height, int width,
                      yb_stream_t stream) {
  return yb::conv0_wgrad_bn(x_nchw, z_nhwc_f16, dap, ld_dap, dap_off, mean, invstd, gamma, beta, slope, sums, dw_oihw, batch, height, width, S(stream));
}

int yb_conv_wgrad(const void* x, const void* dz, float* dw_krsc, int batch, int height, int width, int cin, int cout, int ksize, int x_ld,
                  int dz_ld, yb_stream_t stream) {
  return yb::conv_wgrad_forward(x, dz, dw_krsc, batch, height, width, cin, cout, ksize, x_ld, dz_ld, S(stream));
}

int yb_unpack_wgrad(const float* dw_krsc, float* dw_oihw, int cout, int cin, int ksize, float scale, yb_stream_t stream) {
  return yb::unpack_wgrad(dw_krsc, dw_oihw, cout, cin, ksize, scale, S(stream));
}

int yb_grad_guard(float* grads, long long count, float* found_inf, int zero_if_found, yb_stream_t stream) {
  return yb::grad_guard(grads, count, found_inf, zero_if_found, S(stream));
}

int yb_resize_batch_u8(const void* src, const long long* src_off, const int* src_hw, void* dst, int batch, int height, int width, int swap_rb,
                       float* yx_min, float* yx_max, int slots, yb_stream_t stream) {
  return yb::resize_batch_u8(src, src_off, src_hw, dst, batch, height, width, swap_rb, yx_min, yx_max, slots, S(stream));
}

int yb_resize_aug_batch_u8(const void* src, const long long* src_off, const int* src_hw, const int* crop, const float* margin, const unsigned char* flip,
                           void* dst, int batch, int height, int width, int swap_rb, float* yx_min, float* yx_max, int slots, yb_stream_t stream) {
  return yb::resize_aug_batch_u8(src, src_off, src_hw, crop, margin, flip, dst, batch, height, width, swap_rb, yx_min, yx_max, slots, S(stream));
}

int yb_warp_affine_u8(const void* src, int src_h, int src_w, void* dst, int dst_h, int dst_w, const double* inverse_matrix6, const int* fill3,
                      yb_stream_t stream) {
  return yb::warp_affine_u8(src, src_h, src_w, dst, dst_h, dst_w, inverse_matrix6, fill3, S(stream));
}

int yb_totensor_u8(const void* src_nhwc_u8, float* dst_nchw_f32, int batch, int height, int width, yb_stream_t stream) {
  return yb::totensor_u8(src_nhwc_u8, dst_nchw_f32, batch, height, width, S(stream));
}

int yb_photometric_batch_u8(const void* src, void* dst, int batch, int height, int width, const void* params, int param_stride, int stages,
                            yb_stream_t stream) {
  return yb::photometric_batch_u8(src, dst, batch, height, width, params, param_stride, stages, S(stream));
}

int yb_eval_match(const float* det_yx_min, const float* det_yx_max, const int* det_cls, const int* det_off, const float* gt_yx_min,
                  const float* gt_yx_max, const int* gt_cls, const int* gt_off, int batch, int num_cls, int max_gt, float threshold, float min_union,
                  unsigned char* tp, yb_stream_t stream) {
  return yb::eval_match(det_yx_min, det_yx_max, det_cls, det_off, gt_yx_min, gt_yx_max, gt_cls, gt_off, batch, num_cls, max_gt, threshold, min_union, tp,
                        S(stream));
}

int yb_mb_conv0_bn_relu_fwd(const float* x_nchw, const float* w_oihw, const float* scale, const float* shift, void* y_nhwc_f16, int batch,
                            int height, int width, yb_stream_t stream) {
  return yb::mb_conv0(x_nchw, w_oihw, scale, shift, y_nhwc_f16, batch, height, width, 0, 0, S(stream));
}

int yb_mb_conv0_split_fwd(const float* x_nchw, const float* w_oihw, const float* scale, const float* shift, void* y_hi_lo, int batch, int height, int width,
                          yb_stream_t stream) {
  return yb::mb_conv0(x_nchw, w_oihw, scale, shift, y_hi_lo, batch, height, width, 0, 1, S(stream));
}

int yb_dwconv3x3_split_fwd(const void* x_hi_lo, const float* w_c9, const float* scale, const float* shift, void* y_hi_lo, int batch, int height, int width,
                           int channels, int stride, yb_stream_t stream) {
  return yb::dwconv3x3_split(x_hi_lo, w_c9, scale, shift, y_hi_lo, batch, height, width, channels, stride, S(stream));
}

int yb_mb_conv0_raw_fwd(const float* x_nchw, const float* w_oihw, void* z_nhwc_f16, int batch, int height, int width, yb_stream_t stream) {
  return yb::mb_conv0(x_nchw, w_oihw, nullptr, nullptr, z_nhwc_f16, batch, height, width, 1, 0, S(stream));
}

int yb_mb_conv0_wgrad(const float* x_nchw, const void* dz_nhwc_f16, float* dw_oihw, int batch, int height, int width, yb_stream_t stream) {
  return yb::mb_conv0_wgrad(x_nchw, dz_nhwc_f16, dw_oihw, batch, height, width, S(stream));
}

int yb_dwconv3x3_raw_fwd(const void* x, const float* w_c9, void* z, int batch, int height, int width, int channels, int stride, yb_stream_t stream) {
  return yb::dwconv3x3(x, w_c9, nullptr, nullptr, z, batch, height, width, channels, stride, 1, S(stream));
}

int yb_dwconv3x3_dgrad(const void* dz, const float* w_c9, void* da, int batch, int height, int width, int channels, int stride, yb_stream_t stream) {
  return yb::dw_dgrad(dz, w_c9, da, batch, height, width, channels, stride, S(stream));
}

int yb_dwconv3x3_wgrad(const void* a, const void* dz, float* dw_c9, int batch, int height, int width, int channels, int stride, yb_stream_t stream) {
  return yb::dw_wgrad(a, dz, dw_c9, batch, height, width, channels, stride, S(stream));
}

int yb_dwconv3x3_bn_relu_fwd(const void* x, const float* w_c9, const float* scale, const float* shift, void* y, int batch, int height,
                             int width, int channels, int stride, yb_stream_t stream) {
  return yb::dwconv3x3(x, w_c9, scale, shift, y, batch, height, width, channels, stride, 0, S(stream));
}

int yb_stem7x7_bn_relu_fwd(const float* x_nchw, const float* w_oihw, const float* scale, const float* shift, void* y_nhwc_f16, int batch, int height, int width,
                           yb_stream_t stream) {
  return yb::stem7x7(x_nchw, w_oihw, scale, shift, y_nhwc_f16, batch, height, width, 0, S(stream));
}

int yb_maxpool3x3_s2_f16(const void* x, void* y, int batch, int height, int width, int channels, yb_stream_t stream) {
  return yb::maxpool3x3_s2(x, y, batch, height, width, channels, S(stream));
}

int yb_subsample2_f16(const void* x, void* y, int batch, int height, int width, int channels, yb_stream_t stream) {
  return yb::subsample2(x, y, batch, height, width, channels, S(stream));
}

int yb_add_relu_f16(const void* a, const void* b, void* out, long long count, yb_stream_t stream) { return yb::add_relu(a, b, out, count, S(stream)); }

int yb_stem7x7_raw_fwd(const float* x_nchw, const float* w_oihw, void* z_nhwc_f16, int batch, int height, int width, yb_stream_t stream) {
  return yb::stem7x7(x_nchw, w_oihw, nullptr, nullptr, z_nhwc_f16, batch, height, width, 1, S(stream));
}

int yb_stem7x7_wgrad(const float* x_nchw, const void* dz_nhwc_f16, float* dw_oihw, int batch, int height, int width, yb_stream_t stream) {
  return yb::stem7x7_wgrad(x_nchw, dz_nhwc_f16, dw_oihw, batch, height, width, S(stream));
}

int yb_maxpool3x3_s2_bwd_f16(const void* x, const void* dy, void* dx, int batch, int height, int width, int channels, yb_stream_t stream) {
  return yb::maxpool3x3_s2_bwd(x, dy, dx, batch, height, width, channels, S(stream));
}

int yb_upsample2_zero_f16(const void* x, void* y, int batch, int height, int width, int channels, yb_stream_t stream) {
  return yb::upsample2_zero(x, y, batch, height, width, channels, S(stream));
}

int yb_residual_bwd_f16(const void* y, const void* g_a, const void* g_b, int stride_b, void* out, int batch, int height, int width, int channels,
                        yb_stream_t stream) {
  return yb::residual_bwd(y, g_a, g_b, stride_b, out, batch, height, width, channels, S(stream));
}

int yb_comm_version(int* nccl_version) { return yb::comm_version(nccl_version); }

int yb_comm_unique_id(void* id128) { return yb::comm_unique_id(id128); }

int yb_comm_init(void** comm, int nranks, const void* id128, int rank) { return yb::comm_init(comm, nranks, id128, rank); }

int yb_comm_destroy(void* comm) { return yb::comm_destroy(comm); }

int yb_allreduce_bucket(void* comm, void* buf, long long count, int dtype, yb_stream_t stream) {
  return yb::allreduce_bucket(comm, buf, count, dtype, S(stream));
}

int yb_broadcast_buffer(void* comm, void* buf, long long count, int dtype, int root, yb_stream_t stream) {
  return yb::broadcast_buffer(comm, buf, count, dtype, root, S(stream));
}

}
```

### yolo2-pytorch_b200/csrc/conv_igemm.cu

```cuda
#include "yb_common.h"
#include "yb_ptx.cuh"
#include <stdlib.h>

namespace yb {

struct ConvParams {
  int m_total;
  int height, width;
  int cin, cout;
  int ksize, pad;
  int kb_per_tap;
  int num_kb;
  int m_tiles, n_tiles;
  int a_im2col;
  const float* scale;
  const float* shift;
  float slope;
  void* y;
  long long y_ld;
  int y_ch_off;
  int out_mode;
  int hw;
  int skip;
  int* dbg;
  int streamk;
  int sk_base, sk_rem;
  float* ws;
  unsigned* flags;
  unsigned long long* trace;
  double* stats;
  int a_wrap;
  long long lo_off;
  int tma_store;
};

#define YB_TRACE(role, slot) do { if (p.trace != nullptr && blockIdx.x == 0 && (slot) < 256) p.trace[(role) * 256 + (slot)] = clock64(); } while (0)


constexpr int BM = 128;

constexpr int UMMA_K = 16;
constexpr int kMmaThreads = 128;
constexpr int kProducerWarp = 4;
constexpr int kEpiWarp0 = 5;
constexpr int kEpiThreads = 128;
constexpr int kThreads = kMmaThreads + 32 + kEpiThreads;
constexpr int kSmemLimit = 232448;

struct WorkIter {
  int tile, kb0, kb1;
  int streamk, num_kb, num_tiles, stride, s, cur_end;
  __device__ __forceinline__ static int sk_start(int c, int base, int rem) { return c * base + (c < rem ? c : rem); }
  __device__ __forceinline__ WorkIter(const ConvParams& p, int unit_id, int num_units, int ntiles) {
    streamk = p.streamk; num_kb = p.num_kb; num_tiles = ntiles; stride = num_units;
    if (streamk) {
      s = sk_start(unit_id, p.sk_base, p.sk_rem);
      cur_end = sk_start(unit_id + 1, p.sk_base, p.sk_rem);
      tile = 0; kb0 = 0; kb1 = 0;
      advance();
    } else {
      tile = unit_id; kb0 = 0; kb1 = num_kb; s = 0; cur_end = 0;
    }
  }
  __device__ __forceinline__ void advance() {
    if (cur_end <= s) { tile = num_tiles; return; }
    tile = (cur_end - 1) / num_kb;
    const int tile_start = tile * num_kb;
    const int seg_start = s > tile_start ? s : tile_start;
    kb0 = seg_start - tile_start;
    kb1 = cur_end - tile_start;
    cur_end = seg_start;
  }
  __device__ __forceinline__ bool valid() const { return tile < num_tiles; }
  __device__ __forceinline__ void next() { if (streamk) advance(); else tile += stride; }
};

__device__ __forceinline__ unsigned ld_acquire_gpu(const unsigned* p) {
  unsigned v;
  asm volatile("ld.acquire.gpu.global.u32 %0, [%1];" : "=r"(v) : "l"(p) : "memory");
  return v;
}
__device__ __forceinline__ void st_release_gpu(unsigned* p, unsigned v) {
  asm volatile("st.release.gpu.global.u32 [%0], %1;" :: "l"(p), "r"(v) : "memory");
}

template <int BN, int BK, int MT, int kPreCh = 0>
struct ConvCfg {
  static constexpr int kSwizzle = BK * 2;
  static constexpr int kASubBytes = BM * BK * 2;
  static constexpr int kABytes = MT * kASubBytes;
  static constexpr int kBBytes = BN * BK * 2;
  static constexpr int kStageBytes = kABytes + kBBytes;
  static constexpr int kAccCols = MT * BN;
  static constexpr int kAccBytes = kAccCols * kAccPitch * 4;
  static constexpr bool kMergedA = (MT == 2);
  static constexpr int kRowsPerTile = BM * MT;
  static constexpr int kOutBytes = BM * 128;
  static constexpr int kFixedBytes = kAccBytes + kOutBytes + 1024  + 2 * 2 * BN * 4  + 2 * BN * 4  + 256  +
                                     2 * kPreCh * 4 ;
  static constexpr int kStages = ((kSmemLimit - kFixedBytes) / kStageBytes) > 8 ? 8 : ((kSmemLimit - kFixedBytes) / kStageBytes);
  static constexpr int kSmemBytes = kStages * kStageBytes + kFixedBytes;
  static_assert(kAccCols <= 128, "accumulator does not fit the MMA warpgroup's registers");
  static_assert(kStages >= 2, "shared memory budget");
};

struct PreAct {
  const float* scale;
  const float* shift;
  int relu;
};
constexpr int kPreMaxCh = 1920;

template <int BK, int MT>
__device__ __forceinline__ void preact_stage(uint32_t a, const float* tab_scale, const float* tab_shift, int c0, int relu) {
  constexpr int kChunks = BK / 8;
  constexpr int kRowsPerPass = kMmaThreads / kChunks;
  const int c = threadIdx.x % kChunks;
  const int r0 = threadIdx.x / kChunks;
#pragma unroll 1
  for (int pass = 0; pass < 2; ++pass) {
    const int half = pass ^ ((r0 / (64 / BK)) & 1);
    const int ch = c0 + c * 8 + half * 4;
    const float4 sc = *reinterpret_cast<const float4*>(tab_scale + ch);
    const float4 sh = *reinterpret_cast<const float4*>(tab_shift + ch);
#pragma unroll 1
    for (int i = 0; i < MT * BM / kRowsPerPass; ++i) {
      const int r = r0 + i * kRowsPerPass;
      const int pc = (BK == 64) ? (c ^ (r & 7)) : (c ^ ((r >> 1) & 3));
      const uint32_t addr = a + r * (BK * 2) + pc * 16 + half * 8;
      uint32_t v0, v1;
      asm volatile("ld.shared.v2.b32 {%0, %1}, [%2];" : "=r"(v0), "=r"(v1) : "r"(addr) : "memory");
      const float2 f0 = __half22float2(*reinterpret_cast<__half2*>(&v0));
      const float2 f1 = __half22float2(*reinterpret_cast<__half2*>(&v1));
      float y0 = __fmaf_rn(sc.x, f0.x, sh.x), y1 = __fmaf_rn(sc.y, f0.y, sh.y);
      float y2 = __fmaf_rn(sc.z, f1.x, sh.z), y3 = __fmaf_rn(sc.w, f1.y, sh.w);
      if (relu) { y0 = fmaxf(y0, 0.f); y1 = fmaxf(y1, 0.f); y2 = fmaxf(y2, 0.f); y3 = fmaxf(y3, 0.f); }
      __half2 h0 = __floats2half2_rn(y0, y1), h1 = __floats2half2_rn(y2, y3);
      asm volatile("st.shared.v2.b32 [%0], {%1, %2};" :: "r"(addr), "r"(*reinterpret_cast<uint32_t*>(&h0)), "r"(*reinterpret_cast<uint32_t*>(&h1))
                   : "memory");
    }
  }
}

template <int BN, int BK, int MT, bool kPre>
__device__ __forceinline__ void conv_igemm_body(const CUtensorMap& tmap_a, const CUtensorMap& tmap_b, const CUtensorMap& tmap_y,
                                                const ConvParams p, const PreAct pre) {
  using Cfg = ConvCfg<BN, BK, MT, kPre ? kPreMaxCh : 0>;
  constexpr int kStages = Cfg::kStages;
  constexpr bool kMergedA = Cfg::kMergedA;
  extern __shared__ uint8_t smem_raw[];
  const uint32_t smem_base = (smem_u32(smem_raw) + 1023u) & ~1023u;
  uint8_t* smem_gen = smem_raw + (smem_base - smem_u32(smem_raw));
  const uint32_t smem_a = smem_base;
  const uint32_t smem_b = smem_base + kStages * Cfg::kABytes;
  const uint32_t smem_o = smem_base + kStages * Cfg::kStageBytes;
  float* sacc = reinterpret_cast<float*>(smem_gen + kStages * Cfg::kStageBytes + Cfg::kOutBytes);
  float* ep_scale = sacc + Cfg::kAccCols * kAccPitch;
  float* ep_shift = ep_scale + 2 * BN;
  float* ep_stats = ep_shift + 2 * BN;
  uint64_t* bars = reinterpret_cast<uint64_t*>(ep_stats + 2 * BN);
  const uint32_t bar_full = smem_u32(bars);
  const uint32_t bar_empty = bar_full + 8 * kStages;
  const uint32_t bar_tfull = bar_empty + 8 * kStages;
  const uint32_t bar_tempty = bar_tfull + 8;

  const int warp = threadIdx.x >> 5;
  const int lane = threadIdx.x & 31;
  const int num_tiles = p.m_tiles * p.n_tiles;
  const int unit_id = static_cast<int>(blockIdx.x);
  const int num_units = static_cast<int>(gridDim.x);

  if (threadIdx.x == 0) {
    for (int i = 0; i < kStages; ++i) {
      mbar_init(bar_full + 8 * i, 1);
      mbar_init(bar_empty + 8 * i, 4);
    }
    mbar_init(bar_tfull, 4);
    mbar_init(bar_tempty, 4);
    fence_mbar_init();
    fence_proxy_async_smem();
    tma_prefetch_desc(&tmap_a);
    tma_prefetch_desc(&tmap_b);
    if (p.tma_store) tma_prefetch_desc(&tmap_y);
  }
  __syncthreads();
  pdl_trigger();
  pdl_wait();

  if (warp == kProducerWarp) {
    if (lane == 0) {
      int stage = 0;
      uint32_t phase = 0;
      int tr_p = 0;
      for (WorkIter it(p, unit_id, num_units, num_tiles); it.valid(); it.next()) {
        const int tile = it.tile;
        const int n_tile = tile % p.n_tiles;
        const int m_tile = tile / p.n_tiles;
        const int m_cta = m_tile * Cfg::kRowsPerTile;
        int img[MT], h0[MT], w0[MT];
        int nsub = 0;
#pragma unroll
        for (int t = 0; t < MT; ++t) {
          const int ms = m_cta + t * BM;
          if (ms < p.m_total) nsub = t + 1;
          img[t] = ms / p.hw;
          const int rem = ms - img[t] * p.hw;
          h0[t] = rem / p.width;
          w0[t] = rem - h0[t] * p.width;
        }
        if (p.skip & 1) nsub = 0;
        if (kMergedA && nsub) nsub = MT;
        const uint32_t tx_bytes = nsub * Cfg::kASubBytes + ((p.skip & 2) ? 0 : Cfg::kBBytes);
        for (int kb = it.kb0; kb < it.kb1; ++kb) {
          const int tap = kb / p.kb_per_tap;
          const int c0 = (kb - tap * p.kb_per_tap) * BK;
          const int ca = c0 >= p.a_wrap ? c0 - p.a_wrap : c0;
          const int r = tap / p.ksize;
          const int s = tap - r * p.ksize;
          mbar_wait(bar_empty + 8 * stage, phase ^ 1, p.dbg, 0x100 | stage);
          YB_TRACE(0, tr_p); ++tr_p;
          const uint32_t full = bar_full + 8 * stage;
          mbar_arrive_expect_tx(full, tx_bytes);
          if (kMergedA) {
            if (!(p.skip & 1)) {
              const uint32_t dst = smem_a + stage * Cfg::kABytes;
              if (p.a_im2col) tma_load_im2col_4d(dst, &tmap_a, full, ca, w0[0] - p.pad, h0[0] - p.pad, img[0], static_cast<uint16_t>(s), static_cast<uint16_t>(r));
              else tma_load_2d(dst, &tmap_a, full, ca, m_cta);
            }
          } else {
#pragma unroll
          for (int t = 0; t < MT; ++t) {
            if (t < nsub) {
              const uint32_t dst = smem_a + stage * Cfg::kABytes + t * Cfg::kASubBytes;
              if (p.a_im2col) tma_load_im2col_4d(dst, &tmap_a, full, ca, w0[t] - p.pad, h0[t] - p.pad, img[t], static_cast<uint16_t>(s), static_cast<uint16_t>(r));
              else tma_load_2d(dst, &tmap_a, full, ca, m_cta + t * BM);
            }
          }
          }
          if (!(p.skip & 2)) tma_load_2d(smem_b + stage * Cfg::kBBytes, &tmap_b, full, tap * p.cin + c0, n_tile * BN);
          if (++stage == kStages) { stage = 0; phase ^= 1; }
        }
      }
    }
  } else if (warp < kProducerWarp) {
    float acc[MT][2][BN / 2];
    int stage = 0;
    uint32_t phase = 0;
    uint32_t acc_phase = 0;
    int tr_m = 0;
    float* pre_scale = reinterpret_cast<float*>(reinterpret_cast<uint8_t*>(bars) + 256);
    float* pre_shift = pre_scale + kPreMaxCh;
    if constexpr (kPre) {
      for (int i = threadIdx.x; i < p.cin; i += kMmaThreads) { pre_scale[i] = __ldg(pre.scale + i); pre_shift[i] = __ldg(pre.shift + i); }
      asm volatile("bar.sync 2, %0;" :: "n"(kMmaThreads) : "memory");
    }
    for (WorkIter it(p, unit_id, num_units, num_tiles); it.valid(); it.next()) {
      const int kb_first = it.kb0, kb_last = it.kb1 - 1;
      int prev = -1;
      for (int kb = kb_first; kb <= kb_last; ++kb) {
        mbar_wait(bar_full + 8 * stage, phase, p.dbg, 0x300 | stage);
        if (threadIdx.x == 0) { YB_TRACE(1, tr_m); ++tr_m; }
        if constexpr (kPre) {
          preact_stage<BK, MT>(smem_a + stage * Cfg::kABytes, pre_scale, pre_shift, kb * BK, pre.relu);
          fence_proxy_async_smem();
          asm volatile("bar.sync 2, %0;" :: "n"(kMmaThreads) : "memory");
        }
        if (!(p.skip & 4)) {
          const uint64_t bdesc = make_kmajor_desc<Cfg::kSwizzle>(smem_b + stage * Cfg::kBBytes);
          wgmma_fence();
#pragma unroll
          for (int t = 0; t < MT; ++t) {
#pragma unroll
            for (int h = 0; h < 2; ++h) {
              const uint64_t adesc = make_kmajor_desc<Cfg::kSwizzle>(smem_a + stage * Cfg::kABytes + t * Cfg::kASubBytes + h * 64 * Cfg::kSwizzle);
#pragma unroll
              for (int k = 0; k < BK / UMMA_K; ++k)
                wgmma_f16<BN>(acc[t][h], adesc + 2 * k, bdesc + 2 * k, ((kb - kb_first) | k) != 0);
            }
          }
          wgmma_commit();
          wgmma_wait<1>();
        }
        if (prev >= 0) { __syncwarp(); if (lane == 0) mbar_arrive(bar_empty + 8 * prev); }
        prev = stage;
        if (++stage == kStages) { stage = 0; phase ^= 1; }
      }
      wgmma_wait<0>();
#pragma unroll
      for (int t = 0; t < MT; ++t)
#pragma unroll
        for (int h = 0; h < 2; ++h) fence_regs(acc[t][h]);
      __syncwarp();
      if (lane == 0) mbar_arrive(bar_empty + 8 * prev);
      mbar_wait(bar_tempty, acc_phase ^ 1, p.dbg, 0x200);
#pragma unroll
      for (int t = 0; t < MT; ++t)
#pragma unroll
        for (int h = 0; h < 2; ++h) sacc_store<BN>(sacc, h * 64, t * BN, acc[t][h]);
      __syncwarp();
      if (lane == 0) mbar_arrive(bar_tfull);
      acc_phase ^= 1;
    }
  } else {
    const int q = warp - kEpiWarp0;
    const int et = threadIdx.x - kEpiWarp0 * 32;
    uint32_t acc_phase = 0;
    int buf = 0;
    for (WorkIter it(p, unit_id, num_units, num_tiles); it.valid(); it.next()) {
      const int tile = it.tile;
      const int n_tile = tile % p.n_tiles;
      const int m_tile = tile / p.n_tiles;
      const int n0 = n_tile * BN;
      const bool sk_dump = it.kb1 < p.num_kb;
      const bool sk_collect = !sk_dump && it.kb0 > 0;
      int sk_lo = 0;
      const int m_cta = m_tile * Cfg::kRowsPerTile;
      float* sc = ep_scale + buf * BN;
      float* sh = ep_shift + buf * BN;
      buf ^= 1;
      for (int i = et; i < BN; i += kEpiThreads) {
        const int c = n0 + i;
        sc[i] = (c < p.cout) ? __ldg(p.scale + c) : 0.f;
        sh[i] = (c < p.cout) ? __ldg(p.shift + c) : 0.f;
        if (p.stats != nullptr) { ep_stats[i] = 0.f; ep_stats[BN + i] = 0.f; }
      }
      if (sk_collect) {
        const int u = tile * p.num_kb;
        const int wide = p.sk_rem * (p.sk_base + 1);
        sk_lo = u < wide ? u / (p.sk_base + 1) : p.sk_rem + (u - wide) / p.sk_base;
        if (et == 0) {
          for (int j = sk_lo; j < static_cast<int>(blockIdx.x); ++j) {
            uint32_t spins = 0;
            uint64_t t0 = 0;
            while (ld_acquire_gpu(p.flags + j) == 0u) {
              if ((++spins & 0x3FFu) == 0) {
                const uint64_t now = globaltimer_ns();
                if (t0 == 0) t0 = now;
                if (now - t0 > 4000000000ull) {
                  if (p.dbg != nullptr) { p.dbg[0] = 0x0BAD0500; p.dbg[1] = static_cast<int>(blockIdx.x); p.dbg[2] = j; p.dbg[3] = tile; __threadfence_system(); }
                  __trap();
                }
              }
            }
          }
        }
      }
      asm volatile("bar.sync 1, %0;" :: "n"(kEpiThreads) : "memory");
      mbar_wait(bar_tfull, acc_phase, p.dbg, 0x400);
      if (sk_dump) {
        float* wsp = p.ws + static_cast<size_t>(blockIdx.x) * (MT * BN * 128);
#pragma unroll 1
        for (int t = 0; t < MT; ++t) {
          if (m_cta + t * BM >= p.m_total) break;
#pragma unroll 1
          for (int cc = 0; cc < BN / 32; ++cc) {
            if (n0 + cc * 32 >= p.cout) break;
            uint32_t v[32];
            sacc_ld_x32(sacc, q * 32 + lane, t * BN + cc * 32, v);
            float4* dst = reinterpret_cast<float4*>(wsp + (static_cast<size_t>(t * (BN / 32) + cc) * 128 + q * 32 + lane) * 32);
#pragma unroll
            for (int g = 0; g < 8; ++g)
              dst[g] = make_float4(__uint_as_float(v[4 * g]), __uint_as_float(v[4 * g + 1]), __uint_as_float(v[4 * g + 2]), __uint_as_float(v[4 * g + 3]));
          }
        }
        __threadfence();
        asm volatile("bar.sync 1, %0;" :: "n"(kEpiThreads) : "memory");
        if (et == 0) st_release_gpu(p.flags + blockIdx.x, 1u);
        if (lane == 0) mbar_arrive(bar_tempty);
        acc_phase ^= 1;
        continue;
      }
#pragma unroll 1
      for (int t = 0; t < MT; ++t) {
        if (m_cta + t * BM >= p.m_total) break;
        const int row = m_cta + t * BM + q * 32 + lane;
        const bool row_ok = row < p.m_total;
        int img = 0, pix = 0;
        if (p.out_mode == 1) { img = row / p.hw; pix = row - img * p.hw; }
        if (p.tma_store) {
#pragma unroll 1
          for (int c2 = 0; c2 < BN / 64; ++c2) {
            if (n0 + c2 * 64 >= p.cout) break;
            uint4 pk[8];
            uint32_t vv[2][32];
            sacc_ld_x32(sacc, q * 32 + lane, t * BN + (c2 * 2) * 32, vv[0]);
            sacc_ld_x32(sacc, q * 32 + lane, t * BN + (c2 * 2 + 1) * 32, vv[1]);
#pragma unroll
            for (int hh = 0; hh < 2; ++hh) {
              const int cc = c2 * 2 + hh;
              uint32_t (&v)[32] = vv[hh];
              const int cbase = n0 + cc * 32;
              if (sk_collect && cbase < p.cout) {
                for (int j = sk_lo; j < static_cast<int>(blockIdx.x); ++j) {
                  const float4* src = reinterpret_cast<const float4*>(p.ws + static_cast<size_t>(j) * (MT * BN * 128) +
                                                                      (static_cast<size_t>(t * (BN / 32) + cc) * 128 + q * 32 + lane) * 32);
#pragma unroll
                  for (int g = 0; g < 8; ++g) {
                    const float4 a = __ldcg(src + g);
                    v[4 * g] = __float_as_uint(__uint_as_float(v[4 * g]) + a.x);
                    v[4 * g + 1] = __float_as_uint(__uint_as_float(v[4 * g + 1]) + a.y);
                    v[4 * g + 2] = __float_as_uint(__uint_as_float(v[4 * g + 2]) + a.z);
                    v[4 * g + 3] = __float_as_uint(__uint_as_float(v[4 * g + 3]) + a.w);
                  }
                }
              }
              float f[32];
#pragma unroll
              for (int j = 0; j < 32; ++j) {
                float x = __uint_as_float(v[j]) * sc[cc * 32 + j] + sh[cc * 32 + j];
                f[j] = x > 0.f ? x : x * p.slope;
              }
              if (p.stats != nullptr && cbase < p.cout) {
                float a1[32], a2[32];
#pragma unroll
                for (int j = 0; j < 32; ++j) {
                  const float r = row_ok ? __half2float(__float2half_rn(f[j])) : 0.f;
                  a1[j] = r; a2[j] = r * r;
                }
#pragma unroll
                for (int s = 16; s >= 1; s >>= 1) {
                  const bool up = (lane & s) != 0;
#pragma unroll
                  for (int j = 0; j < s; ++j) {
                    const float k1 = up ? a1[j + s] : a1[j], g1 = up ? a1[j] : a1[j + s];
                    const float k2 = up ? a2[j + s] : a2[j], g2 = up ? a2[j] : a2[j + s];
                    a1[j] = k1 + __shfl_xor_sync(0xffffffffu, g1, s);
                    a2[j] = k2 + __shfl_xor_sync(0xffffffffu, g2, s);
                  }
                }
                atomicAdd(&ep_stats[cc * 32 + lane], a1[0]);
                atomicAdd(&ep_stats[BN + cc * 32 + lane], a2[0]);
              }
#pragma unroll
              for (int g = 0; g < 4; ++g) {
                __half2 h0 = __floats2half2_rn(f[g * 8 + 0], f[g * 8 + 1]);
                __half2 h1 = __floats2half2_rn(f[g * 8 + 2], f[g * 8 + 3]);
                __half2 h2 = __floats2half2_rn(f[g * 8 + 4], f[g * 8 + 5]);
                __half2 h3 = __floats2half2_rn(f[g * 8 + 6], f[g * 8 + 7]);
                pk[hh * 4 + g].x = *reinterpret_cast<uint32_t*>(&h0);
                pk[hh * 4 + g].y = *reinterpret_cast<uint32_t*>(&h1);
                pk[hh * 4 + g].z = *reinterpret_cast<uint32_t*>(&h2);
                pk[hh * 4 + g].w = *reinterpret_cast<uint32_t*>(&h3);
              }
            }
            if (lane == 0) tma_store_wait_read<0>();
            __syncwarp();
            {
              const uint32_t slice = smem_o + q * 4096 + lane * 128;
#pragma unroll
              for (int c = 0; c < 8; ++c) st_shared_v4(slice + ((c ^ (lane & 7)) << 4), pk[c]);
            }
            fence_proxy_async_smem();
            __syncwarp();
            if (lane == 0 && !(p.skip & 8)) {
              tma_store_2d(&tmap_y, smem_o + q * 4096, n0 + c2 * 64, m_cta + t * BM + q * 32);
              tma_store_commit();
            }
          }
          continue;
        }
#pragma unroll 1
        for (int cc = 0; cc < BN / 32; ++cc) {
          uint32_t v[32];
          sacc_ld_x32(sacc, q * 32 + lane, t * BN + cc * 32, v);
          const int cbase = n0 + cc * 32;
          if (cbase >= p.cout) continue;
          if (sk_collect) {
            for (int j = sk_lo; j < static_cast<int>(blockIdx.x); ++j) {
              const float4* src = reinterpret_cast<const float4*>(p.ws + static_cast<size_t>(j) * (MT * BN * 128) +
                                                                  (static_cast<size_t>(t * (BN / 32) + cc) * 128 + q * 32 + lane) * 32);
#pragma unroll
              for (int g = 0; g < 8; ++g) {
                const float4 a = __ldcg(src + g);
                v[4 * g] = __float_as_uint(__uint_as_float(v[4 * g]) + a.x);
                v[4 * g + 1] = __float_as_uint(__uint_as_float(v[4 * g + 1]) + a.y);
                v[4 * g + 2] = __float_as_uint(__uint_as_float(v[4 * g + 2]) + a.z);
                v[4 * g + 3] = __float_as_uint(__uint_as_float(v[4 * g + 3]) + a.w);
              }
            }
          }
          float f[32];
#pragma unroll
          for (int j = 0; j < 32; ++j) {
            float x = __uint_as_float(v[j]) * sc[cc * 32 + j] + sh[cc * 32 + j];
            f[j] = x > 0.f ? x : x * p.slope;
          }
          if (p.skip & 8) continue;
          if (p.stats != nullptr) {
            float a1[32], a2[32];
#pragma unroll
            for (int j = 0; j < 32; ++j) {
              const float r = row_ok ? __half2float(__float2half_rn(f[j])) : 0.f;
              a1[j] = r; a2[j] = r * r;
            }
#pragma unroll
            for (int s = 16; s >= 1; s >>= 1) {
              const bool up = (lane & s) != 0;
#pragma unroll
              for (int j = 0; j < s; ++j) {
                const float k1 = up ? a1[j + s] : a1[j], g1 = up ? a1[j] : a1[j + s];
                const float k2 = up ? a2[j + s] : a2[j], g2 = up ? a2[j] : a2[j + s];
                a1[j] = k1 + __shfl_xor_sync(0xffffffffu, g1, s);
                a2[j] = k2 + __shfl_xor_sync(0xffffffffu, g2, s);
              }
            }
            atomicAdd(&ep_stats[cc * 32 + lane], a1[0]);
            atomicAdd(&ep_stats[BN + cc * 32 + lane], a2[0]);
          }
          if (p.out_mode == 0) {
            if (row_ok) {
              __half* dst = reinterpret_cast<__half*>(p.y) + static_cast<long long>(row) * p.y_ld + p.y_ch_off + cbase;
#pragma unroll
              for (int g = 0; g < 4; ++g) {
                if (cbase + g * 8 < p.cout) {
                  uint4 pk;
                  __half2 h0 = __floats2half2_rn(f[g * 8 + 0], f[g * 8 + 1]);
                  __half2 h1 = __floats2half2_rn(f[g * 8 + 2], f[g * 8 + 3]);
                  __half2 h2 = __floats2half2_rn(f[g * 8 + 4], f[g * 8 + 5]);
                  __half2 h3 = __floats2half2_rn(f[g * 8 + 6], f[g * 8 + 7]);
                  pk.x = *reinterpret_cast<uint32_t*>(&h0);
                  pk.y = *reinterpret_cast<uint32_t*>(&h1);
                  pk.z = *reinterpret_cast<uint32_t*>(&h2);
                  pk.w = *reinterpret_cast<uint32_t*>(&h3);
                  *reinterpret_cast<uint4*>(dst + g * 8) = pk;
                  if (p.lo_off != 0) {
                    const float2 r0 = __half22float2(h0), r1 = __half22float2(h1), r2 = __half22float2(h2), r3 = __half22float2(h3);
                    __half2 l0 = __floats2half2_rn(f[g * 8 + 0] - r0.x, f[g * 8 + 1] - r0.y);
                    __half2 l1 = __floats2half2_rn(f[g * 8 + 2] - r1.x, f[g * 8 + 3] - r1.y);
                    __half2 l2 = __floats2half2_rn(f[g * 8 + 4] - r2.x, f[g * 8 + 5] - r2.y);
                    __half2 l3 = __floats2half2_rn(f[g * 8 + 6] - r3.x, f[g * 8 + 7] - r3.y);
                    uint4 pl;
                    pl.x = *reinterpret_cast<uint32_t*>(&l0);
                    pl.y = *reinterpret_cast<uint32_t*>(&l1);
                    pl.z = *reinterpret_cast<uint32_t*>(&l2);
                    pl.w = *reinterpret_cast<uint32_t*>(&l3);
                    *reinterpret_cast<uint4*>(dst + p.lo_off + g * 8) = pl;
                  }
                }
              }
            }
          } else {
            if (row_ok) {
              float* dst = reinterpret_cast<float*>(p.y) + (static_cast<long long>(img) * p.cout + cbase) * p.hw + pix;
#pragma unroll
              for (int j = 0; j < 32; ++j) {
                if (cbase + j < p.cout) dst[static_cast<long long>(j) * p.hw] = f[j];
              }
            }
          }
        }
      }
      __syncwarp();
      if (lane == 0) mbar_arrive(bar_tempty);
      if (p.stats != nullptr) {
        asm volatile("bar.sync 1, %0;" :: "n"(kEpiThreads) : "memory");
        for (int i = et; i < BN; i += kEpiThreads) {
          if (n0 + i < p.cout) {
            atomicAdd(p.stats + n0 + i, static_cast<double>(ep_stats[i]));
            atomicAdd(p.stats + p.cout + n0 + i, static_cast<double>(ep_stats[BN + i]));
          }
        }
        asm volatile("bar.sync 1, %0;" :: "n"(kEpiThreads) : "memory");
      }
      if (sk_collect) {
        asm volatile("bar.sync 1, %0;" :: "n"(kEpiThreads) : "memory");
        for (int j = sk_lo + et; j < static_cast<int>(blockIdx.x); j += kEpiThreads) p.flags[j] = 0u;
      }
      acc_phase ^= 1;
    }
    if (p.tma_store && lane == 0) tma_store_wait<0>();
  }
}

template <int BN, int BK, int MT>
__global__ void __launch_bounds__(kThreads, 1)
conv_igemm_kernel(const __grid_constant__ CUtensorMap tmap_a, const __grid_constant__ CUtensorMap tmap_b,
                  const __grid_constant__ CUtensorMap tmap_y, const ConvParams p) {
  conv_igemm_body<BN, BK, MT, false>(tmap_a, tmap_b, tmap_y, p, PreAct{nullptr, nullptr, 0});
}

template <int BN, int BK, int MT>
__global__ void __launch_bounds__(kThreads, 1)
conv_preact_kernel(const __grid_constant__ CUtensorMap tmap_a, const __grid_constant__ CUtensorMap tmap_b,
                   const __grid_constant__ CUtensorMap tmap_y, const ConvParams p, const PreAct pre) {
  conv_igemm_body<BN, BK, MT, true>(tmap_a, tmap_b, tmap_y, p, pre);
}

constexpr int kWideThreads = 384;
constexpr int kWideRows = 256;
constexpr int kWideBN = 128;

template <int BK>
struct WideCfg {
  static constexpr int kSwizzle = BK * 2;
  static constexpr int kABytes = kWideRows * BK * 2;
  static constexpr int kBBytes = kWideBN * BK * 2;
  static constexpr int kStageBytes = kABytes + kBBytes;
  static constexpr int kOutBytes = 128 * 128;
  static constexpr int kFixedBytes = 2 * kOutBytes + 1024  + 256 ;
  static constexpr int kStages = ((kSmemLimit - kFixedBytes) / kStageBytes) > 8 ? 8 : ((kSmemLimit - kFixedBytes) / kStageBytes);
  static constexpr int kSmemBytes = kStages * kStageBytes + kFixedBytes;
  static constexpr int kWsFloats = kWideRows * kWideBN;
  static_assert(kStages >= 3, "shared memory budget");
};

template <int BK>
__global__ void __launch_bounds__(kWideThreads, 1)
conv_wide_kernel(const __grid_constant__ CUtensorMap tmap_a, const __grid_constant__ CUtensorMap tmap_b,
                 const __grid_constant__ CUtensorMap tmap_y, const ConvParams p) {
  using Cfg = WideCfg<BK>;
  constexpr int kStages = Cfg::kStages;
  extern __shared__ uint8_t smem_raw[];
  const uint32_t smem_base = (smem_u32(smem_raw) + 1023u) & ~1023u;
  const uint32_t smem_a = smem_base;
  const uint32_t smem_b = smem_base + kStages * Cfg::kABytes;
  const uint32_t smem_o = smem_base + kStages * Cfg::kStageBytes;
  const uint32_t bar_full = smem_o + 2 * Cfg::kOutBytes;
  const uint32_t bar_empty = bar_full + 8 * kStages;
  const int num_tiles = p.m_tiles * p.n_tiles;
  const int unit_id = static_cast<int>(blockIdx.x);
  const int num_units = static_cast<int>(gridDim.x);

  if (threadIdx.x == 0) {
    for (int i = 0; i < kStages; ++i) {
      mbar_init(bar_full + 8 * i, 1);
      mbar_init(bar_empty + 8 * i, 8);
    }
    fence_mbar_init();
    fence_proxy_async_smem();
    tma_prefetch_desc(&tmap_a);
    tma_prefetch_desc(&tmap_b);
    tma_prefetch_desc(&tmap_y);
  }
  __syncthreads();
  pdl_trigger();
  pdl_wait();

  if (threadIdx.x < 128) {
    setmaxnreg_dec<40>();
    if (threadIdx.x == 0) {
      int stage = 0;
      uint32_t phase = 0;
      for (WorkIter it(p, unit_id, num_units, num_tiles); it.valid(); it.next()) {
        const int n_tile = it.tile % p.n_tiles;
        const int m_cta = (it.tile / p.n_tiles) * kWideRows;
        const int img = m_cta / p.hw;
        const int rem = m_cta - img * p.hw;
        const int h0 = rem / p.width;
        const int w0 = rem - h0 * p.width;
        for (int kb = it.kb0; kb < it.kb1; ++kb) {
          const int tap = kb / p.kb_per_tap;
          const int c0 = (kb - tap * p.kb_per_tap) * BK;
          const int ca = c0 >= p.a_wrap ? c0 - p.a_wrap : c0;
          const int r = tap / p.ksize;
          const int s = tap - r * p.ksize;
          mbar_wait(bar_empty + 8 * stage, phase ^ 1, p.dbg, 0x600 | stage);
          const uint32_t full = bar_full + 8 * stage;
          mbar_arrive_expect_tx(full, Cfg::kStageBytes);
          const uint32_t dst = smem_a + stage * Cfg::kABytes;
          if (p.a_im2col) tma_load_im2col_4d(dst, &tmap_a, full, ca, w0 - p.pad, h0 - p.pad, img, static_cast<uint16_t>(s), static_cast<uint16_t>(r));
          else tma_load_2d(dst, &tmap_a, full, ca, m_cta);
          tma_load_2d(smem_b + stage * Cfg::kBBytes, &tmap_b, full, tap * p.cin + c0, n_tile * kWideBN);
          if (++stage == kStages) { stage = 0; phase ^= 1; }
        }
      }
    }
    return;
  }
  setmaxnreg_inc<232>();
  const int cw = (threadIdx.x >> 7) - 1;
  const int t = threadIdx.x & 127;
  const int warp = t >> 5;
  const int lane = t & 31;
  const bool leader = threadIdx.x == 128;
  const uint32_t stage_o = smem_o + cw * Cfg::kOutBytes;
  float acc[2][64];
  int stage = 0;
  uint32_t phase = 0;
  for (WorkIter it(p, unit_id, num_units, num_tiles); it.valid(); it.next()) {
    const int kb_first = it.kb0, kb_last = it.kb1 - 1;
    int prev = -1;
    for (int kb = kb_first; kb <= kb_last; ++kb) {
      mbar_wait(bar_full + 8 * stage, phase, p.dbg, 0x700 | stage);
      const uint64_t bdesc = make_kmajor_desc<Cfg::kSwizzle>(smem_b + stage * Cfg::kBBytes);
      wgmma_fence();
#pragma unroll
      for (int h = 0; h < 2; ++h) {
        const uint64_t adesc = make_kmajor_desc<Cfg::kSwizzle>(smem_a + stage * Cfg::kABytes + (cw * 128 + h * 64) * Cfg::kSwizzle);
#pragma unroll
        for (int k = 0; k < BK / UMMA_K; ++k)
          wgmma_f16<kWideBN>(acc[h], adesc + 2 * k, bdesc + 2 * k, ((kb - kb_first) | k) != 0);
      }
      wgmma_commit();
      wgmma_wait<1>();
      if (prev >= 0) { __syncwarp(); if (lane == 0) mbar_arrive(bar_empty + 8 * prev); }
      prev = stage;
      if (++stage == kStages) { stage = 0; phase ^= 1; }
    }
    wgmma_wait<0>();
    fence_regs(acc[0]);
    fence_regs(acc[1]);
    __syncwarp();
    if (lane == 0) mbar_arrive(bar_empty + 8 * prev);

    const int tile = it.tile;
    const int n0 = (tile % p.n_tiles) * kWideBN;
    const int m_base = (tile / p.n_tiles) * kWideRows + cw * 128;
    const bool sk_dump = it.kb1 < p.num_kb;
    const bool sk_collect = !sk_dump && it.kb0 > 0;
    if (sk_dump) {
      float4* dst = reinterpret_cast<float4*>(p.ws + static_cast<size_t>(blockIdx.x) * Cfg::kWsFloats) + cw * 32 * 128 + t;
#pragma unroll
      for (int g = 0; g < 32; ++g)
        dst[g * 128] = make_float4(acc[g >> 4][4 * (g & 15)], acc[g >> 4][4 * (g & 15) + 1], acc[g >> 4][4 * (g & 15) + 2], acc[g >> 4][4 * (g & 15) + 3]);
      __threadfence();
      asm volatile("bar.sync 1, 256;" ::: "memory");
      if (leader) st_release_gpu(p.flags + blockIdx.x, 1u);
      continue;
    }
    int sk_lo = 0;
    if (sk_collect) {
      const int u = tile * p.num_kb;
      const int wide = p.sk_rem * (p.sk_base + 1);
      sk_lo = u < wide ? u / (p.sk_base + 1) : p.sk_rem + (u - wide) / p.sk_base;
      if (leader) {
        for (int j = sk_lo; j < static_cast<int>(blockIdx.x); ++j) {
          uint32_t spins = 0;
          uint64_t t0 = 0;
          while (ld_acquire_gpu(p.flags + j) == 0u) {
            if ((++spins & 0x3FFu) == 0) {
              const uint64_t now = globaltimer_ns();
              if (t0 == 0) t0 = now;
              if (now - t0 > 4000000000ull) {
                if (p.dbg != nullptr) { p.dbg[0] = 0x0BAD0800; p.dbg[1] = static_cast<int>(blockIdx.x); p.dbg[2] = j; p.dbg[3] = tile; __threadfence_system(); }
                __trap();
              }
            }
          }
        }
      }
      asm volatile("bar.sync 1, 256;" ::: "memory");
      for (int j = sk_lo; j < static_cast<int>(blockIdx.x); ++j) {
        const float4* src = reinterpret_cast<const float4*>(p.ws + static_cast<size_t>(j) * Cfg::kWsFloats) + cw * 32 * 128 + t;
#pragma unroll
        for (int g = 0; g < 32; ++g) {
          const float4 a = __ldcg(src + g * 128);
          float* d = &acc[g >> 4][4 * (g & 15)];
          d[0] += a.x; d[1] += a.y; d[2] += a.z; d[3] += a.w;
        }
      }
    }
#pragma unroll
    for (int c2 = 0; c2 < 2; ++c2) {
      if (n0 + c2 * 64 < p.cout) {
        if (t == 0) tma_store_wait_read<0>();
        asm volatile("bar.sync %0, 128;" :: "r"(2 + cw) : "memory");
#pragma unroll
        for (int jj = 0; jj < 8; ++jj) {
          const int col = n0 + c2 * 64 + 8 * jj + 2 * (lane & 3);
          const bool ok = col < p.cout;
          const float sc0 = ok ? __ldg(p.scale + col) : 0.f, sc1 = ok ? __ldg(p.scale + col + 1) : 0.f;
          const float sh0 = ok ? __ldg(p.shift + col) : 0.f, sh1 = ok ? __ldg(p.shift + col + 1) : 0.f;
#pragma unroll
          for (int h = 0; h < 2; ++h) {
#pragma unroll
            for (int hh = 0; hh < 2; ++hh) {
              const int j = c2 * 8 + jj;
              float x0 = acc[h][4 * j + 2 * hh] * sc0 + sh0;
              float x1 = acc[h][4 * j + 2 * hh + 1] * sc1 + sh1;
              x0 = x0 > 0.f ? x0 : x0 * p.slope;
              x1 = x1 > 0.f ? x1 : x1 * p.slope;
              __half2 v = __floats2half2_rn(x0, x1);
              const int r = h * 64 + warp * 16 + (lane >> 2) + hh * 8;
              const uint32_t addr = stage_o + r * 128 + ((jj ^ (r & 7)) << 4) + 4 * (lane & 3);
              asm volatile("st.shared.b32 [%0], %1;" :: "r"(addr), "r"(*reinterpret_cast<uint32_t*>(&v)) : "memory");
            }
          }
        }
        fence_proxy_async_smem();
        asm volatile("bar.sync %0, 128;" :: "r"(2 + cw) : "memory");
        if (t == 0) {
#pragma unroll
          for (int g = 0; g < 4; ++g)
            if (m_base + 32 * g < p.m_total) tma_store_2d(&tmap_y, stage_o + g * 4096, n0 + c2 * 64, m_base + 32 * g);
          tma_store_commit();
        }
      }
    }
    if (sk_collect) {
      asm volatile("bar.sync 1, 256;" ::: "memory");
      for (int j = sk_lo + t + 128 * cw; j < static_cast<int>(blockIdx.x); j += 256) p.flags[j] = 0u;
    }
  }
  if (t == 0) tma_store_wait<0>();
}

struct C32Params {
  int batch, height, width, cout;
  int tiles_w, tiles_h, num_tiles;
  const float* scale;
  const float* shift;
  float slope;
  int pool;
  int swap_lbo;
  int skip;
  int* dbg;
  unsigned long long* trace;
  double* stats;
};

struct C32Cfg {
  static constexpr int TH = 16, TW = 8, HH = TH + 2, HW = TW + 2;
  static constexpr int kPlaneData = HH * HW * 16;
  static constexpr int kPlane = (kPlaneData + 127) / 128 * 128;
  static constexpr int kHalo = 4 * kPlane;
  static constexpr int kStages = 4;
  static constexpr int BN = 64;
  static constexpr int kBTap = BN * 32 * 2;
  static constexpr int kBBytes = 9 * kBTap;
  static constexpr int kOutBytes = 128 * 128;
  static constexpr int kGroups = 2;
  static constexpr int kAccBytes = BN * kAccPitch * 4;
  static constexpr int kEpiThreads = kGroups * 128;
  static constexpr int kThreads = 128 + 32 + kEpiThreads;
  static constexpr int kSmemBytes = 1024 + kBBytes + 2 * kGroups * kOutBytes + kStages * kHalo + kGroups * kAccBytes + 2 * BN * 4 + 256 + 2 * BN * 4 ;
  static_assert(kSmemBytes <= kSmemLimit, "c32: shared memory budget");
};

__global__ void __launch_bounds__(C32Cfg::kThreads, 1)
conv_c32_kernel(const __grid_constant__ CUtensorMap tmap_x, const __grid_constant__ CUtensorMap tmap_w,
                const __grid_constant__ CUtensorMap tmap_y, const C32Params p) {
  using Cfg = C32Cfg;
  constexpr int BN = Cfg::BN;
  constexpr int kGroups = Cfg::kGroups;
  extern __shared__ uint8_t smem_raw[];
  const uint32_t smem_base = (smem_u32(smem_raw) + 1023u) & ~1023u;
  uint8_t* smem_gen = smem_raw + (smem_base - smem_u32(smem_raw));
  const uint32_t smem_b = smem_base;
  const uint32_t smem_o = smem_b + Cfg::kBBytes;
  const uint32_t smem_h = smem_o + 2 * kGroups * Cfg::kOutBytes;
  float* sacc = reinterpret_cast<float*>(smem_gen + Cfg::kBBytes + 2 * kGroups * Cfg::kOutBytes + Cfg::kStages * Cfg::kHalo);
  float* ep_scale = sacc + kGroups * BN * kAccPitch;
  float* ep_shift = ep_scale + BN;
  uint64_t* bars = reinterpret_cast<uint64_t*>(ep_shift + BN);
  const uint32_t bar_full = smem_u32(bars);
  const uint32_t bar_empty = bar_full + 8 * Cfg::kStages;
  const uint32_t bar_tfull = bar_empty + 8 * Cfg::kStages;
  const uint32_t bar_tempty = bar_tfull + 8 * kGroups;
  const uint32_t bar_w = bar_tempty + 8 * kGroups;
  float* ep_stats = reinterpret_cast<float*>(reinterpret_cast<uint8_t*>(bars) + 256);
  const int warp = threadIdx.x >> 5, lane = threadIdx.x & 31;

  if (threadIdx.x == 0) {
    for (int i = 0; i < Cfg::kStages; ++i) { mbar_init(bar_full + 8 * i, 1); mbar_init(bar_empty + 8 * i, 4); }
    for (int i = 0; i < kGroups; ++i) { mbar_init(bar_tfull + 8 * i, 4); mbar_init(bar_tempty + 8 * i, 4); }
    mbar_init(bar_w, 1);
    fence_mbar_init();
    fence_proxy_async_smem();
    tma_prefetch_desc(&tmap_x);
    tma_prefetch_desc(&tmap_w);
    tma_prefetch_desc(&tmap_y);
  }
  __syncthreads();
  pdl_trigger();

  if (warp == kProducerWarp) {
    if (lane == 0) {
      mbar_arrive_expect_tx(bar_w, Cfg::kBBytes);
      for (int t = 0; t < 9; ++t) tma_load_2d(smem_b + t * Cfg::kBTap, &tmap_w, bar_w, t * 32, 0);
      int stage = 0; uint32_t phase = 0; int tr = 0;
      for (int tile = blockIdx.x; tile < p.num_tiles; tile += gridDim.x) {
        const int tw = tile % p.tiles_w;
        const int rest = tile / p.tiles_w;
        const int th = rest % p.tiles_h;
        const int n = rest / p.tiles_h;
        mbar_wait(bar_empty + 8 * stage, phase ^ 1, p.dbg, 0xB00 | stage);
        YB_TRACE(0, tr); ++tr;
        if (p.skip & 1) {
          mbar_arrive(bar_full + 8 * stage);
        } else {
          mbar_arrive_expect_tx(bar_full + 8 * stage, 4 * Cfg::kPlaneData);
          for (int c = 0; c < 4; ++c)
            tma_load_4d(smem_h + stage * Cfg::kHalo + c * Cfg::kPlane, &tmap_x, bar_full + 8 * stage, c * 8, tw * Cfg::TW - 1, th * Cfg::TH - 1, n);
        }
        if (++stage == Cfg::kStages) { stage = 0; phase ^= 1; }
      }
    }
  } else if (warp < kProducerWarp) {
    const uint32_t lbo = p.swap_lbo ? Cfg::HW * 16 : Cfg::kPlane;
    const uint32_t sbo = p.swap_lbo ? Cfg::kPlane : Cfg::HW * 16;
    float acc[2][BN / 2];
    int stage = 0; uint32_t phase = 0; int tr = 0;
    mbar_wait(bar_w, 0, p.dbg, 0xB10);
    int local = 0;
    for (int tile = blockIdx.x; tile < p.num_tiles; tile += gridDim.x, ++local) {
      mbar_wait(bar_full + 8 * stage, phase, p.dbg, 0xB30 | stage);
      if (threadIdx.x == 0) { YB_TRACE(1, tr); ++tr; }
      const uint32_t halo = smem_h + stage * Cfg::kHalo;
      if (!(p.skip & 4)) {
        wgmma_fence();
#pragma unroll
        for (int h = 0; h < 2; ++h) {
#pragma unroll
          for (int t = 0; t < 9; ++t) {
            const uint32_t win = halo + ((h * 8 + t / 3) * Cfg::HW + (t % 3)) * 16;
            const uint64_t bdesc = make_kmajor_desc<64>(smem_b + t * Cfg::kBTap);
            wgmma_f16<BN>(acc[h], make_kmajor_desc_noswz(win, lbo, sbo), bdesc, t != 0);
            wgmma_f16<BN>(acc[h], make_kmajor_desc_noswz(win + 2 * Cfg::kPlane, lbo, sbo), bdesc + 2, 1);
          }
        }
        wgmma_commit();
        wgmma_wait<0>();
      }
      fence_regs(acc[0]);
      fence_regs(acc[1]);
      __syncwarp();
      if (lane == 0) mbar_arrive(bar_empty + 8 * stage);
      if (++stage == Cfg::kStages) { stage = 0; phase ^= 1; }
      const int grp = local % kGroups;
      const uint32_t use = static_cast<uint32_t>(local / kGroups);
      mbar_wait(bar_tempty + 8 * grp, (use & 1) ^ 1, p.dbg, 0xB20 | grp);
      float* tile_acc = sacc + grp * BN * kAccPitch;
      sacc_store<BN>(tile_acc, 0, 0, acc[0]);
      sacc_store<BN>(tile_acc, 64, 0, acc[1]);
      __syncwarp();
      if (lane == 0) mbar_arrive(bar_tfull + 8 * grp);
    }
  } else {
    const int ew = warp - kEpiWarp0;
    const int q = ew & 3;
    const int grp = ew >> 2;
    const int gt = (threadIdx.x - kEpiWarp0 * 32) & 127;
    const int et = threadIdx.x - kEpiWarp0 * 32;
    const float* tile_acc = sacc + grp * BN * kAccPitch;
    int tr = 0;
    for (int i = et; i < BN; i += Cfg::kEpiThreads) {
      ep_scale[i] = (i < p.cout) ? __ldg(p.scale + i) : 0.f;
      ep_shift[i] = (i < p.cout) ? __ldg(p.shift + i) : 0.f;
      ep_stats[i] = 0.f; ep_stats[BN + i] = 0.f;
    }
    asm volatile("bar.sync 8, %0;" :: "n"(Cfg::kEpiThreads) : "memory");
    const int m = q * 32 + lane;
    int srow = m;
    bool writer = true;
    if (p.pool) {
      writer = ((lane & 1) == 0) && ((lane & 8) == 0);
      srow = (q * 2 + (lane >> 4)) * 4 + ((lane & 7) >> 1);
    }
    int local = 0;
    for (int tile = blockIdx.x; tile < p.num_tiles; tile += gridDim.x, ++local) {
      if (local % kGroups != grp) continue;
      const uint32_t use = static_cast<uint32_t>(local / kGroups);
      const int tw = tile % p.tiles_w;
      const int rest = tile / p.tiles_w;
      const int th = rest % p.tiles_h;
      const int n = rest / p.tiles_h;
      mbar_wait(bar_tfull + 8 * grp, use & 1, p.dbg, 0xB40 | grp);
      if (et == 0) { YB_TRACE(2, tr); ++tr; }
      uint4 pk[8];
#pragma unroll
      for (int half = 0; half < 2; ++half) {
        uint32_t v[32];
        sacc_ld_x32(tile_acc, m, half * 32, v);
        if (half == 1) {
          __syncwarp();
          if (lane == 0) mbar_arrive(bar_tempty + 8 * grp);
        }
        float f[32];
#pragma unroll
        for (int j4 = 0; j4 < 8; ++j4) {
          const float4 s4 = *reinterpret_cast<const float4*>(ep_scale + half * 32 + j4 * 4);
          const float4 h4 = *reinterpret_cast<const float4*>(ep_shift + half * 32 + j4 * 4);
          const float x0 = __uint_as_float(v[j4 * 4 + 0]) * s4.x + h4.x, x1 = __uint_as_float(v[j4 * 4 + 1]) * s4.y + h4.y;
          const float x2 = __uint_as_float(v[j4 * 4 + 2]) * s4.z + h4.z, x3 = __uint_as_float(v[j4 * 4 + 3]) * s4.w + h4.w;
          f[j4 * 4 + 0] = x0 > 0.f ? x0 : x0 * p.slope; f[j4 * 4 + 1] = x1 > 0.f ? x1 : x1 * p.slope;
          f[j4 * 4 + 2] = x2 > 0.f ? x2 : x2 * p.slope; f[j4 * 4 + 3] = x3 > 0.f ? x3 : x3 * p.slope;
        }
        if (p.stats != nullptr) {
          float a1[32], a2[32];
#pragma unroll
          for (int j = 0; j < 32; ++j) {
            const float r = __half2float(__float2half_rn(f[j]));
            a1[j] = r; a2[j] = r * r;
          }
#pragma unroll
          for (int sft = 16; sft >= 1; sft >>= 1) {
            const bool up = (lane & sft) != 0;
#pragma unroll
            for (int j = 0; j < sft; ++j) {
              const float k1 = up ? a1[j + sft] : a1[j], g1 = up ? a1[j] : a1[j + sft];
              const float k2 = up ? a2[j + sft] : a2[j], g2 = up ? a2[j] : a2[j + sft];
              a1[j] = k1 + __shfl_xor_sync(0xffffffffu, g1, sft);
              a2[j] = k2 + __shfl_xor_sync(0xffffffffu, g2, sft);
            }
          }
          atomicAdd(&ep_stats[half * 32 + lane], a1[0]);
          atomicAdd(&ep_stats[BN + half * 32 + lane], a2[0]);
        }
        if (p.pool) {
#pragma unroll
          for (int j = 0; j < 32; ++j) {
            f[j] = fmaxf(f[j], __shfl_xor_sync(0xffffffffu, f[j], 1));
            f[j] = fmaxf(f[j], __shfl_xor_sync(0xffffffffu, f[j], 8));
          }
        }
#pragma unroll
        for (int g = 0; g < 4; ++g) {
          __half2 h0 = __floats2half2_rn(f[g * 8 + 0], f[g * 8 + 1]), h1 = __floats2half2_rn(f[g * 8 + 2], f[g * 8 + 3]);
          __half2 h2 = __floats2half2_rn(f[g * 8 + 4], f[g * 8 + 5]), h3 = __floats2half2_rn(f[g * 8 + 6], f[g * 8 + 7]);
          pk[half * 4 + g].x = *reinterpret_cast<uint32_t*>(&h0); pk[half * 4 + g].y = *reinterpret_cast<uint32_t*>(&h1);
          pk[half * 4 + g].z = *reinterpret_cast<uint32_t*>(&h2); pk[half * 4 + g].w = *reinterpret_cast<uint32_t*>(&h3);
        }
      }
      const uint32_t obuf = smem_o + (grp * 2 + (use & 1)) * Cfg::kOutBytes;
      if (gt == 0) tma_store_wait_read<1>();
      asm volatile("bar.sync %0, 128;" :: "r"(1 + grp) : "memory");
      if (et == 0) { YB_TRACE(2, tr); ++tr; }
      if (writer) {
#pragma unroll
        for (int c = 0; c < 8; ++c) st_shared_v4(obuf + srow * 128 + ((c ^ (srow & 7)) << 4), pk[c]);
      }
      fence_proxy_async_smem();
      asm volatile("bar.sync %0, 128;" :: "r"(1 + grp) : "memory");
      if (gt == 0 && !(p.skip & 8)) {
        if (p.pool) tma_store_4d(&tmap_y, obuf, 0, tw * (Cfg::TW / 2), th * (Cfg::TH / 2), n);
        else tma_store_4d(&tmap_y, obuf, 0, tw * Cfg::TW, th * Cfg::TH, n);
        tma_store_commit();
      }
      if (et == 0) { YB_TRACE(2, tr); ++tr; }
    }
    if (gt == 0) tma_store_wait<0>();
    if (p.stats != nullptr) {
      asm volatile("bar.sync 8, %0;" :: "n"(Cfg::kEpiThreads) : "memory");
      for (int i = et; i < p.cout; i += Cfg::kEpiThreads) {
        atomicAdd(p.stats + i, static_cast<double>(ep_stats[i]));
        atomicAdd(p.stats + p.cout + i, static_cast<double>(ep_stats[BN + i]));
      }
    }
  }
}

constexpr long long kSkFlagBytes = 4096;
constexpr long long kSkSlotBytes = kWideRows * kWideBN * 4;
long long conv_workspace_bytes() { return kSkFlagBytes + kSkSlotBytes * sm_count(); }

constexpr int kKernelIgemm = 0;
constexpr int kKernelWide = 1;
constexpr int kKernelC32 = 2;
struct ConvChoice {
  int kernel, bk, bn, mt, streamk, grid;
};

static unsigned long long* g_conv_trace = nullptr;
void conv_set_trace(void* dev_ptr) { g_conv_trace = static_cast<unsigned long long*>(dev_ptr); }

typedef CUresult (*EncodeTiledFn)(CUtensorMap*, CUtensorMapDataType, cuuint32_t, void*, const cuuint64_t*, const cuuint64_t*,
                                  const cuuint32_t*, const cuuint32_t*, CUtensorMapInterleave, CUtensorMapSwizzle,
                                  CUtensorMapL2promotion, CUtensorMapFloatOOBfill);
typedef CUresult (*EncodeIm2colFn)(CUtensorMap*, CUtensorMapDataType, cuuint32_t, void*, const cuuint64_t*, const cuuint64_t*,
                                   const int*, const int*, cuuint32_t, cuuint32_t, const cuuint32_t*, CUtensorMapInterleave,
                                   CUtensorMapSwizzle, CUtensorMapL2promotion, CUtensorMapFloatOOBfill);

static int get_encoders(EncodeTiledFn* tiled, EncodeIm2colFn* im2col) {
  static EncodeTiledFn s_tiled = nullptr;
  static EncodeIm2colFn s_im2col = nullptr;
  if (s_tiled == nullptr || s_im2col == nullptr) {
    void* f0 = nullptr;
    void* f1 = nullptr;
    cudaDriverEntryPointQueryResult q0, q1;
    YB_CUDA(cudaGetDriverEntryPoint("cuTensorMapEncodeTiled", &f0, cudaEnableDefault, &q0));
    YB_CUDA(cudaGetDriverEntryPoint("cuTensorMapEncodeIm2col", &f1, cudaEnableDefault, &q1));
    if (f0 == nullptr || f1 == nullptr || q0 != cudaDriverEntryPointSuccess || q1 != cudaDriverEntryPointSuccess)
      return fail(YB_ERR_DRIVER, "cuTensorMapEncode* driver entry points unavailable");
    s_tiled = reinterpret_cast<EncodeTiledFn>(f0);
    s_im2col = reinterpret_cast<EncodeIm2colFn>(f1);
  }
  *tiled = s_tiled;
  *im2col = s_im2col;
  return 0;
}

int get_tensor_map_encoders(EncodeTiledFn* tiled, EncodeIm2colFn* im2col) { return get_encoders(tiled, im2col); }

template <int BN, int BK, int MT>
static int launch_conv(const CUtensorMap& ta, const CUtensorMap& tb, const CUtensorMap& ty, const ConvParams& p, const PreAct* pre,
                       cudaStream_t stream) {
  using Cfg = ConvCfg<BN, BK, MT>;
  using PreCfg = ConvCfg<BN, BK, MT, kPreMaxCh>;
  static bool attr_set = false, pre_attr_set = false;
  if (pre == nullptr && !attr_set) {
    YB_CUDA(cudaFuncSetAttribute(conv_igemm_kernel<BN, BK, MT>, cudaFuncAttributeMaxDynamicSharedMemorySize, Cfg::kSmemBytes));
    attr_set = true;
  }
  if (pre != nullptr && !pre_attr_set) {
    YB_CUDA(cudaFuncSetAttribute(conv_preact_kernel<BN, BK, MT>, cudaFuncAttributeMaxDynamicSharedMemorySize, PreCfg::kSmemBytes));
    pre_attr_set = true;
  }
  const int tiles = p.m_tiles * p.n_tiles;
  cudaLaunchConfig_t cfg;
  memset(&cfg, 0, sizeof(cfg));
  cudaLaunchAttribute attr[1];
  int nattr = 0;
  static const int use_pdl = getenv("YB_PDL") ? atoi(getenv("YB_PDL")) : 0;
  if (use_pdl) {
    attr[nattr].id = cudaLaunchAttributeProgrammaticStreamSerialization;
    attr[nattr].val.programmaticStreamSerializationAllowed = 1;
    ++nattr;
  }
  if (p.streamk) cfg.gridDim = dim3(sm_count());
  else cfg.gridDim = dim3(tiles < sm_count() ? tiles : sm_count());
  cfg.blockDim = dim3(kThreads);
  cfg.dynamicSmemBytes = pre != nullptr ? PreCfg::kSmemBytes : Cfg::kSmemBytes;
  cfg.stream = stream;
  cfg.attrs = attr; cfg.numAttrs = nattr;
  if (pre != nullptr) {
    YB_CUDA(cudaLaunchKernelEx(&cfg, conv_preact_kernel<BN, BK, MT>, ta, tb, ty, p, *pre));
    return check_launch("conv_preact_kernel");
  }
  YB_CUDA(cudaLaunchKernelEx(&cfg, conv_igemm_kernel<BN, BK, MT>, ta, tb, ty, p));
  return check_launch("conv_igemm_kernel");
}

template <int BK>
static int launch_wide(const CUtensorMap& ta, const CUtensorMap& tb, const CUtensorMap& ty, const ConvParams& p, int grid, cudaStream_t stream) {
  using Cfg = WideCfg<BK>;
  static bool attr_set = false;
  if (!attr_set) {
    YB_CUDA(cudaFuncSetAttribute(conv_wide_kernel<BK>, cudaFuncAttributeMaxDynamicSharedMemorySize, Cfg::kSmemBytes));
    attr_set = true;
  }
  cudaLaunchConfig_t cfg;
  memset(&cfg, 0, sizeof(cfg));
  cudaLaunchAttribute attr[1];
  int nattr = 0;
  static const int use_pdl = getenv("YB_PDL") ? atoi(getenv("YB_PDL")) : 0;
  if (use_pdl) {
    attr[nattr].id = cudaLaunchAttributeProgrammaticStreamSerialization;
    attr[nattr].val.programmaticStreamSerializationAllowed = 1;
    ++nattr;
  }
  cfg.gridDim = dim3(grid);
  cfg.blockDim = dim3(kWideThreads);
  cfg.dynamicSmemBytes = Cfg::kSmemBytes;
  cfg.stream = stream;
  cfg.attrs = attr; cfg.numAttrs = nattr;
  YB_CUDA(cudaLaunchKernelEx(&cfg, conv_wide_kernel<BK>, ta, tb, ty, p));
  return check_launch("conv_wide_kernel");
}

template <int BK>
static int dispatch_conv(int bn, int mt, int grid, const CUtensorMap& ta, const CUtensorMap& tb, const CUtensorMap& ty, const ConvParams& p,
                         const PreAct* pre, cudaStream_t stream) {
  if (mt == 2 && bn == 128) return launch_wide<BK>(ta, tb, ty, p, grid, stream);
  if (mt == 2) return launch_conv<64, BK, 2>(ta, tb, ty, p, pre, stream);
  if (bn == 64) return launch_conv<64, BK, 1>(ta, tb, ty, p, pre, stream);
  return launch_conv<128, BK, 1>(ta, tb, ty, p, pre, stream);
}

static int conv_c32_forward(const void* x, const void* w, const float* scale, const float* shift, float slope, void* y, int batch,
                            int height, int width, int cout, int x_ld, long long y_ld, int y_ch_off, int pool, int flags, double* stats,
                            cudaStream_t stream) {
  using Cfg = C32Cfg;
  EncodeTiledFn enc_tiled;
  EncodeIm2colFn enc_im2col;
  int rc = get_encoders(&enc_tiled, &enc_im2col);
  if (rc) return rc;
  YB_REQUIRE(!pool || (height % 2 == 0 && width % 2 == 0), "conv: fused 2x2 max-pool needs even H and W");
  C32Params p;
  p.batch = batch; p.height = height; p.width = width; p.cout = cout;
  p.tiles_w = (width + Cfg::TW - 1) / Cfg::TW;
  p.tiles_h = (height + Cfg::TH - 1) / Cfg::TH;
  const long long nt = static_cast<long long>(batch) * p.tiles_w * p.tiles_h;
  YB_REQUIRE(nt < (1ll << 31), "conv: too many tiles");
  p.num_tiles = static_cast<int>(nt);
  p.scale = scale; p.shift = shift; p.slope = slope;
  p.pool = pool;
  p.swap_lbo = (flags >> 6) & 1;
  p.skip = (flags >> 24) & 0xF;
  p.dbg = debug_word_device();
  p.trace = g_conv_trace;
  p.stats = stats;
  YB_REQUIRE(stats == nullptr || (!pool && height % Cfg::TH == 0 && width % Cfg::TW == 0),
             "conv: fused statistics on the Cin = 32 kernel need H %% 16 == 0, W %% 8 == 0 and no fused pool");
  alignas(64) CUtensorMap tx, tw, ty;
  CUresult cr;
  {
    const cuuint64_t dims[4] = {32, static_cast<cuuint64_t>(width), static_cast<cuuint64_t>(height), static_cast<cuuint64_t>(batch)};
    const cuuint64_t strides[3] = {static_cast<cuuint64_t>(x_ld) * 2, static_cast<cuuint64_t>(x_ld) * 2 * width,
                                   static_cast<cuuint64_t>(x_ld) * 2 * width * height};
    const cuuint32_t box[4] = {8, Cfg::HW, Cfg::HH, 1};
    const cuuint32_t estr[4] = {1, 1, 1, 1};
    cr = enc_tiled(&tx, CU_TENSOR_MAP_DATA_TYPE_FLOAT16, 4, const_cast<void*>(x), dims, strides, box, estr, CU_TENSOR_MAP_INTERLEAVE_NONE,
                   CU_TENSOR_MAP_SWIZZLE_NONE, CU_TENSOR_MAP_L2_PROMOTION_L2_128B, CU_TENSOR_MAP_FLOAT_OOB_FILL_NONE);
    if (cr != CUDA_SUCCESS) return fail(YB_ERR_DRIVER, "cuTensorMapEncodeTiled(halo) failed (%d)", static_cast<int>(cr));
  }
  {
    const cuuint64_t dims[2] = {9 * 32, static_cast<cuuint64_t>(cout)};
    const cuuint64_t strides[1] = {9 * 32 * 2};
    const cuuint32_t box[2] = {32, 64};
    const cuuint32_t estr[2] = {1, 1};
    cr = enc_tiled(&tw, CU_TENSOR_MAP_DATA_TYPE_FLOAT16, 2, const_cast<void*>(w), dims, strides, box, estr, CU_TENSOR_MAP_INTERLEAVE_NONE,
                   CU_TENSOR_MAP_SWIZZLE_64B, CU_TENSOR_MAP_L2_PROMOTION_L2_256B, CU_TENSOR_MAP_FLOAT_OOB_FILL_NONE);
    if (cr != CUDA_SUCCESS) return fail(YB_ERR_DRIVER, "cuTensorMapEncodeTiled(W) failed (%d)", static_cast<int>(cr));
  }
  {
    const int oh = pool ? height / 2 : height, ow = pool ? width / 2 : width;
    const cuuint64_t dims[4] = {static_cast<cuuint64_t>(cout), static_cast<cuuint64_t>(ow), static_cast<cuuint64_t>(oh), static_cast<cuuint64_t>(batch)};
    const cuuint64_t strides[3] = {static_cast<cuuint64_t>(y_ld) * 2, static_cast<cuuint64_t>(y_ld) * 2 * ow, static_cast<cuuint64_t>(y_ld) * 2 * ow * oh};
    const cuuint32_t box[4] = {64, static_cast<cuuint32_t>(pool ? Cfg::TW / 2 : Cfg::TW), static_cast<cuuint32_t>(pool ? Cfg::TH / 2 : Cfg::TH), 1};
    const cuuint32_t estr[4] = {1, 1, 1, 1};
    cr = enc_tiled(&ty, CU_TENSOR_MAP_DATA_TYPE_FLOAT16, 4, static_cast<__half*>(y) + y_ch_off, dims, strides, box, estr,
                   CU_TENSOR_MAP_INTERLEAVE_NONE, CU_TENSOR_MAP_SWIZZLE_128B, CU_TENSOR_MAP_L2_PROMOTION_NONE, CU_TENSOR_MAP_FLOAT_OOB_FILL_NONE);
    if (cr != CUDA_SUCCESS) return fail(YB_ERR_DRIVER, "cuTensorMapEncodeTiled(Y) failed (%d)", static_cast<int>(cr));
  }
  static bool attr_set = false;
  if (!attr_set) {
    YB_CUDA(cudaFuncSetAttribute(conv_c32_kernel, cudaFuncAttributeMaxDynamicSharedMemorySize, Cfg::kSmemBytes));
    attr_set = true;
  }
  const int grid = p.num_tiles < sm_count() ? p.num_tiles : sm_count();
  conv_c32_kernel<<<grid, Cfg::kThreads, Cfg::kSmemBytes, stream>>>(tx, tw, ty, p);
  return check_launch("conv_c32_kernel");
}

constexpr double kKbNsIm2col = 240.0;
constexpr double kKbNsTiled = 100.0;
constexpr double kFeedBytesPerNs = 130.0;
constexpr double kEpiNsPerOut = 0.15;
constexpr double kWideEpiNsPerOut = 0.08;
constexpr double kSkNs = 16000.0;
constexpr double kSkNsWide = 9000.0;
int conv_choose(int batch, int height, int width, int cin, int cout, int ksize, int a_channels, int out_mode, int flags, bool workspace_ok,
                bool stats, bool lo, bool pre, ConvChoice* out) {
  ConvChoice c;
  memset(&c, 0, sizeof(c));
  const int sms = sm_count();
  const bool split = a_channels != cin || lo;
  if (!split && cin == 32 && ksize == 3 && cout <= 64 && out_mode == 0 && ((flags >> 28) & 1) == 0 && ((flags >> 5) & 1) == 0 && ((flags >> 8) & 0xFFFF) == 0) {
    const long long tiles = static_cast<long long>(batch) * ((width + C32Cfg::TW - 1) / C32Cfg::TW) * ((height + C32Cfg::TH - 1) / C32Cfg::TH);
    c.kernel = kKernelC32; c.bk = 32; c.bn = C32Cfg::BN; c.mt = 1;
    c.grid = static_cast<int>(tiles < sms ? tiles : sms);
    *out = c;
    return 0;
  }
  if ((flags >> 4) & 1) return fail(YB_ERR_UNSUPPORTED, "conv: YB_CONV_POOL2X2 is only implemented for the Cin = 32 3x3 layer");
  const int bk = (cin % 64 == 0 && a_channels % 64 == 0) ? 64 : 32;
  const bool sk_possible = !stats && workspace_ok && (flags & 8) == 0;
  const bool sk_force = sk_possible && ((flags >> 30) & 1);
  const bool wide_ok = out_mode == 0 && !lo && !stats && !pre && ((flags >> 24) & 0xF) == 0 && ((flags >> 29) & 1) == 0;
  const int force_bn = (flags >> 8) & 0x3FF;
  const int force_mt = (flags >> 20) & 0x3;
  const int force_pair = (flags >> 22) & 0x3;
  YB_REQUIRE(force_pair != 2, "conv: CTA-pair tiles need two-CTA tensor-core instructions, which sm_90 does not have");
  YB_REQUIRE(!force_bn || ((force_bn == 64 || force_bn == 128) && (force_mt != 2 || force_bn == 64 || wide_ok)),
             "conv: BLOCK_N=%d x %d M-subtiles is not a tile shape of this launch (64 x 1, 128 x 1, 64 x 2; 128 x 2 for fp16 NHWC "
             "outputs without residual or statistics)", force_bn, force_mt ? force_mt : 1);
  const long long m_total = static_cast<long long>(batch) * height * width;
  const int num_kb = ksize * ksize * (cin / bk);
  double best = 1e300;
  for (int cbn = 64; cbn <= 128; cbn *= 2) {
    if (force_bn && cbn != force_bn) continue;
    if (!force_bn && cbn > 64 && cbn / 2 >= cout) continue;
    for (int cmt = 1; cmt <= 2; ++cmt) {
      if (force_mt && cmt != force_mt) continue;
      const bool cwide = cmt * cbn > 128;
      if (cwide && !wide_ok) continue;
      const int rows_tile = BM * cmt;
      const double tiles = static_cast<double>((m_total + rows_tile - 1) / rows_tile) * ((cout + cbn - 1) / cbn);
      const double rounds = static_cast<double>((static_cast<long long>(tiles) + sms - 1) / sms);
      const double kb_ns = (ksize == 3 ? kKbNsIm2col : kKbNsTiled) + (cmt * BM + cbn) * bk * 2.0 / kFeedBytesPerNs;
      const double main_ns = num_kb * kb_ns;
      const double outs = static_cast<double>(rows_tile) * cbn;
      const double tile_ns = cwide ? main_ns + outs * kWideEpiNsPerOut : (main_ns > outs * kEpiNsPerOut ? main_ns : outs * kEpiNsPerOut);
      double t = rounds * tile_ns;
      int csk = 0;
      if (sk_possible) {
        const double units = tiles * num_kb;
        const double per_cta = static_cast<double>((static_cast<long long>(units) + sms - 1) / sms);
        const double tsk = per_cta * kb_ns + (cwide ? kSkNsWide : kSkNs);
        const bool ok = per_cta >= 4.0 && num_kb >= 2;
        const bool idle = tiles <= sms / 2;
        if (ok && (sk_force || (idle && tsk < 0.93 * t))) { t = tsk; csk = 1; }
      }
      if (sk_force && !csk) continue;
      if (t < best * 0.9999 || (t <= best * 1.0001 && cbn > c.bn)) { best = t; c.bn = cbn; c.mt = cmt; c.streamk = csk; }
    }
  }
  if (c.bn == 0) { c.bn = force_bn ? force_bn : 128; c.mt = force_mt ? force_mt : 1; c.streamk = 0; }
  YB_REQUIRE((c.bn == 64 || c.bn == 128) && (c.mt == 1 || c.mt == 2) && (c.mt * c.bn <= 128 || wide_ok), "conv: tile %d x %d", c.bn, c.mt);
  c.kernel = c.mt * c.bn > 128 ? kKernelWide : kKernelIgemm;
  c.bk = bk;
  const long long tiles = ((m_total + BM * c.mt - 1) / (BM * c.mt)) * ((cout + c.bn - 1) / c.bn);
  c.grid = c.streamk ? sms : static_cast<int>(tiles < sms ? tiles : sms);
  *out = c;
  return 0;
}

int conv_choice(int batch, int height, int width, int cin, int cout, int ksize, int out_mode, int flags, int with_workspace, int* out) {
  YB_REQUIRE(out != nullptr && batch > 0 && height > 0 && width > 0 && cin % 32 == 0 && cout > 0 && (ksize == 1 || ksize == 3),
             "conv_choice: bad shape");
  ConvChoice c;
  const int rc = conv_choose(batch, height, width, cin, cout, ksize, cin, out_mode, flags, with_workspace != 0, false, false, false, &c);
  if (rc) return rc;
  out[0] = c.kernel; out[1] = c.bk; out[2] = c.bn; out[3] = c.kernel == kKernelC32 ? C32Cfg::TH * C32Cfg::TW : BM * c.mt;
  out[4] = c.streamk; out[5] = c.grid;
  return 0;
}

int conv_igemm_forward(const void* x, const void* w, const float* scale, const float* shift, float slope, void* y, int batch,
                       int height, int width, int cin, int cout, int ksize, int x_ld, long long y_ld, int y_ch_off, int out_mode,
                       int flags, void* workspace, long long workspace_bytes, double* stats, int a_channels, int lo_ch_off,
                       const float* pre_scale, const float* pre_shift, int pre_relu, cudaStream_t stream) {
  YB_REQUIRE(x && w && scale && shift && y, "conv: null pointer");
  const bool pre = pre_scale != nullptr;
  if (pre) {
    YB_REQUIRE(pre_shift != nullptr && (pre_relu == 0 || pre_relu == 1), "conv_preact: pre_shift must be given, pre_relu 0 or 1");
    YB_REQUIRE(ksize == 1, "conv_preact: k=%d, the pre-activation form is 1x1 only", ksize);
    YB_REQUIRE(a_channels <= 0 || a_channels == cin, "conv_preact: split-precision operands are not supported");
    YB_REQUIRE(lo_ch_off < 0 && stats == nullptr, "conv_preact: no residual output and no fused statistics");
    YB_REQUIRE(cin <= kPreMaxCh, "conv_preact: Cin=%d exceeds the %d-channel pre-activation table", cin, kPreMaxCh);
  }
  const PreAct pre_act{pre_scale, pre_shift, pre_relu};
  if (a_channels <= 0) a_channels = cin;
  YB_REQUIRE(a_channels <= cin && a_channels % 32 == 0 && cin - a_channels <= a_channels, "conv: a_channels=%d does not fit cin=%d", a_channels, cin);
  YB_REQUIRE(lo_ch_off < 0 || (out_mode == 0 && stats == nullptr && lo_ch_off % 8 == 0 && lo_ch_off >= y_ch_off + cout && lo_ch_off + cout <= y_ld),
             "conv: lo_ch_off=%d (needs fp16 NHWC output with room for a second Cout-wide slice)", lo_ch_off);
  YB_REQUIRE(stats == nullptr || out_mode == 0, "conv: fused statistics need the fp16 NHWC output");
  YB_REQUIRE(ksize == 1 || ksize == 3, "conv: ksize %d unsupported (1 or 3)", ksize);
  YB_REQUIRE(batch > 0 && height > 0 && width > 0, "conv: bad shape");
  YB_REQUIRE(cin % 32 == 0, "conv: Cin=%d must be a multiple of 32 (layer 0 uses yb_conv0_*)", cin);
  YB_REQUIRE(x_ld >= a_channels && x_ld % 8 == 0, "conv: x_ld=%d", x_ld);
  YB_REQUIRE((reinterpret_cast<uintptr_t>(x) & 15) == 0 && (reinterpret_cast<uintptr_t>(w) & 15) == 0, "conv: x/w must be 16B aligned");
  YB_REQUIRE(out_mode == 0 || out_mode == 1, "conv: out_mode");
  if (out_mode == 0) {
    YB_REQUIRE(cout % 8 == 0 && y_ld % 8 == 0 && y_ch_off % 8 == 0 && (reinterpret_cast<uintptr_t>(y) & 15) == 0,
               "conv: fp16 NHWC output needs Cout, y_ld, y_ch_off multiples of 8 and a 16B aligned pointer");
  }
  const long long m_total_ll = static_cast<long long>(batch) * height * width;
  YB_REQUIRE(m_total_ll < (1ll << 31) - kWideRows, "conv: too many pixels");
  const bool ws_ok = workspace != nullptr && workspace_bytes >= conv_workspace_bytes() && (reinterpret_cast<uintptr_t>(workspace) & 255) == 0;
  ConvChoice ch;
  int rc = conv_choose(batch, height, width, cin, cout, ksize, a_channels, out_mode, flags, ws_ok, stats != nullptr, lo_ch_off >= 0, pre, &ch);
  if (rc) return rc;
  YB_REQUIRE(!pre || ch.kernel == kKernelIgemm, "conv_preact: no pre-activation form of kernel %d", ch.kernel);
  if (ch.kernel == kKernelC32)
    return conv_c32_forward(x, w, scale, shift, slope, y, batch, height, width, cout, x_ld, y_ld, y_ch_off, (flags >> 4) & 1, flags, stats, stream);
  const int bk = ch.bk, bn = ch.bn, mt = ch.mt, streamk = ch.streamk;
  static const int k1x1_im2col = getenv("YB_CONV_1X1_IM2COL") ? atoi(getenv("YB_CONV_1X1_IM2COL")) : 0;
  const int a_im2col = (ksize == 3) ? 1 : ((k1x1_im2col && !(flags & 1) && !pre) ? 1 : 0);

  EncodeTiledFn enc_tiled;
  EncodeIm2colFn enc_im2col;
  rc = get_encoders(&enc_tiled, &enc_im2col);
  if (rc) return rc;

  ConvParams p;
  p.m_total = static_cast<int>(m_total_ll);
  p.height = height; p.width = width; p.cin = cin; p.cout = cout; p.ksize = ksize; p.pad = (ksize - 1) / 2;
  p.kb_per_tap = cin / bk;
  p.num_kb = ksize * ksize * p.kb_per_tap;
  const int rows_tile = BM * mt;
  p.m_tiles = (p.m_total + rows_tile - 1) / rows_tile;
  p.n_tiles = (cout + bn - 1) / bn;
  p.a_im2col = a_im2col;
  p.scale = scale; p.shift = shift; p.slope = slope;
  p.y = y; p.y_ld = y_ld; p.y_ch_off = y_ch_off; p.out_mode = out_mode;
  p.hw = height * width;
  p.dbg = debug_word_device();
  p.trace = g_conv_trace;
  p.skip = (flags >> 24) & 0xF;
  p.streamk = streamk;
  p.stats = stats;
  p.tma_store = 0;
  p.a_wrap = a_channels;
  p.lo_off = lo_ch_off >= 0 ? static_cast<long long>(lo_ch_off - y_ch_off) : 0;
  p.sk_base = 0; p.sk_rem = 0; p.ws = nullptr; p.flags = nullptr;
  if (streamk) {
    const long long units = static_cast<long long>(p.m_tiles) * p.n_tiles * p.num_kb;
    YB_REQUIRE(units < (1ll << 31), "conv: stream-K unit count overflows");
    p.sk_base = static_cast<int>(units / sm_count());
    p.sk_rem = static_cast<int>(units % sm_count());
    p.flags = static_cast<unsigned*>(workspace);
    p.ws = reinterpret_cast<float*>(static_cast<char*>(workspace) + kSkFlagBytes);
  }

  const CUtensorMapSwizzle swz = (bk == 64) ? CU_TENSOR_MAP_SWIZZLE_128B : CU_TENSOR_MAP_SWIZZLE_64B;
  alignas(64) CUtensorMap ta, tb;
  CUresult cr;
  const int a_rows = BM * mt;
  if (a_im2col) {
    const cuuint64_t dims[4] = {static_cast<cuuint64_t>(a_channels), static_cast<cuuint64_t>(width), static_cast<cuuint64_t>(height),
                                static_cast<cuuint64_t>(batch)};
    const cuuint64_t strides[3] = {static_cast<cuuint64_t>(x_ld) * 2, static_cast<cuuint64_t>(x_ld) * 2 * width,
                                   static_cast<cuuint64_t>(x_ld) * 2 * width * height};
    const int lower[2] = {-p.pad, -p.pad};
    const int upper[2] = {p.pad - (ksize - 1), p.pad - (ksize - 1)};
    const cuuint32_t estr[4] = {1, 1, 1, 1};
    cr = enc_im2col(&ta, CU_TENSOR_MAP_DATA_TYPE_FLOAT16, 4, const_cast<void*>(x), dims, strides, lower, upper,
                    static_cast<cuuint32_t>(bk), static_cast<cuuint32_t>(a_rows), estr, CU_TENSOR_MAP_INTERLEAVE_NONE, swz, CU_TENSOR_MAP_L2_PROMOTION_L2_128B,
                    CU_TENSOR_MAP_FLOAT_OOB_FILL_NONE);
    if (cr != CUDA_SUCCESS) return fail(YB_ERR_DRIVER, "cuTensorMapEncodeIm2col failed (%d)", static_cast<int>(cr));
    int drv = 0;
    cudaDriverGetVersion(&drv);
    const unsigned long long span_bytes = static_cast<unsigned long long>(x_ld) * 2ull * width * height * batch;
    if (drv <= 13010 && span_bytes < 131072ull) reinterpret_cast<uint64_t*>(&ta)[1] &= ~(1ull << 21);
  } else {
    const cuuint64_t dims[2] = {static_cast<cuuint64_t>(a_channels), static_cast<cuuint64_t>(p.m_total)};
    const cuuint64_t strides[1] = {static_cast<cuuint64_t>(x_ld) * 2};
    const cuuint32_t box[2] = {static_cast<cuuint32_t>(bk), static_cast<cuuint32_t>(a_rows)};
    const cuuint32_t estr[2] = {1, 1};
    cr = enc_tiled(&ta, CU_TENSOR_MAP_DATA_TYPE_FLOAT16, 2, const_cast<void*>(x), dims, strides, box, estr,
                   CU_TENSOR_MAP_INTERLEAVE_NONE, swz, CU_TENSOR_MAP_L2_PROMOTION_L2_128B, CU_TENSOR_MAP_FLOAT_OOB_FILL_NONE);
    if (cr != CUDA_SUCCESS) return fail(YB_ERR_DRIVER, "cuTensorMapEncodeTiled(A) failed (%d)", static_cast<int>(cr));
  }
  {
    const cuuint64_t k_total = static_cast<cuuint64_t>(ksize) * ksize * cin;
    const cuuint64_t dims[2] = {k_total, static_cast<cuuint64_t>(cout)};
    const cuuint64_t strides[1] = {k_total * 2};
    const cuuint32_t box[2] = {static_cast<cuuint32_t>(bk), static_cast<cuuint32_t>(bn)};
    const cuuint32_t estr[2] = {1, 1};
    cr = enc_tiled(&tb, CU_TENSOR_MAP_DATA_TYPE_FLOAT16, 2, const_cast<void*>(w), dims, strides, box, estr,
                   CU_TENSOR_MAP_INTERLEAVE_NONE, swz, CU_TENSOR_MAP_L2_PROMOTION_L2_256B, CU_TENSOR_MAP_FLOAT_OOB_FILL_NONE);
    if (cr != CUDA_SUCCESS) return fail(YB_ERR_DRIVER, "cuTensorMapEncodeTiled(W) failed (%d)", static_cast<int>(cr));
  }

  alignas(64) CUtensorMap ty;
  memset(&ty, 0, sizeof(ty));
  p.tma_store = (out_mode == 0 && lo_ch_off < 0 && ((flags >> 29) & 1) == 0) ? 1 : 0;
  if (p.tma_store) {
    const cuuint64_t dims[2] = {static_cast<cuuint64_t>(cout), static_cast<cuuint64_t>(p.m_total)};
    const cuuint64_t strides[1] = {static_cast<cuuint64_t>(y_ld) * 2};
    const cuuint32_t box[2] = {64, 32};
    const cuuint32_t estr[2] = {1, 1};
    cr = enc_tiled(&ty, CU_TENSOR_MAP_DATA_TYPE_FLOAT16, 2, static_cast<__half*>(y) + y_ch_off, dims, strides, box, estr,
                   CU_TENSOR_MAP_INTERLEAVE_NONE, CU_TENSOR_MAP_SWIZZLE_128B, CU_TENSOR_MAP_L2_PROMOTION_NONE, CU_TENSOR_MAP_FLOAT_OOB_FILL_NONE);
    if (cr != CUDA_SUCCESS) return fail(YB_ERR_DRIVER, "cuTensorMapEncodeTiled(Y) failed (%d)", static_cast<int>(cr));
  }
  if (bk == 64) return dispatch_conv<64>(bn, mt, ch.grid, ta, tb, ty, p, pre ? &pre_act : nullptr, stream);
  return dispatch_conv<32>(bn, mt, ch.grid, ta, tb, ty, p, pre ? &pre_act : nullptr, stream);
}

__global__ void conv_ref_kernel(const __half* __restrict__ x, const __half* __restrict__ w, ConvParams p, int x_ld) {
  const long long idx = static_cast<long long>(blockIdx.x) * blockDim.x + threadIdx.x;
  const long long total = static_cast<long long>(p.m_total) * p.cout;
  if (idx >= total) return;
  const int co = static_cast<int>(idx % p.cout);
  const int row = static_cast<int>(idx / p.cout);
  const int img = row / p.hw;
  const int pix = row - img * p.hw;
  const int h = pix / p.width;
  const int wq = pix - h * p.width;
  float acc = 0.f;
  for (int r = 0; r < p.ksize; ++r) {
    const int hi = h + r - p.pad;
    if (hi < 0 || hi >= p.height) continue;
    for (int s = 0; s < p.ksize; ++s) {
      const int wi = wq + s - p.pad;
      if (wi < 0 || wi >= p.width) continue;
      const __half* xp = x + (static_cast<long long>(img) * p.hw + static_cast<long long>(hi) * p.width + wi) * x_ld;
      const __half* wp = w + (static_cast<long long>(co) * p.ksize * p.ksize + r * p.ksize + s) * p.cin;
      for (int c = 0; c < p.cin; ++c) acc += __half2float(xp[c]) * __half2float(wp[c]);
    }
  }
  float v = acc * p.scale[co] + p.shift[co];
  v = v > 0.f ? v : v * p.slope;
  if (p.out_mode == 0) {
    reinterpret_cast<__half*>(p.y)[static_cast<long long>(row) * p.y_ld + p.y_ch_off + co] = __float2half_rn(v);
  } else {
    reinterpret_cast<float*>(p.y)[(static_cast<long long>(img) * p.cout + co) * p.hw + pix] = v;
  }
}

int conv_ref_forward(const void* x, const void* w, const float* scale, const float* shift, float slope, void* y, int batch,
                     int height, int width, int cin, int cout, int ksize, int x_ld, long long y_ld, int y_ch_off, int out_mode,
                     cudaStream_t stream) {
  YB_REQUIRE(x && w && scale && shift && y, "conv_ref: null pointer");
  ConvParams p;
  memset(&p, 0, sizeof(p));
  p.m_total = batch * height * width;
  p.height = height; p.width = width; p.cin = cin; p.cout = cout; p.ksize = ksize; p.pad = (ksize - 1) / 2;
  p.scale = scale; p.shift = shift; p.slope = slope; p.y = y; p.y_ld = y_ld; p.y_ch_off = y_ch_off; p.out_mode = out_mode;
  p.hw = height * width;
  const long long total = static_cast<long long>(p.m_total) * cout;
  conv_ref_kernel<<<static_cast<unsigned>((total + 255) / 256), 256, 0, stream>>>(reinterpret_cast<const __half*>(x),
                                                                                  reinterpret_cast<const __half*>(w), p, x_ld);
  return check_launch("conv_ref_kernel");
}

}
```

### yolo2-pytorch_b200/csrc/yb_common.h

```cpp
#pragma once
#include <cuda_runtime.h>
#include <stdio.h>
#include <string.h>

#define YB_ERR_BAD_ARG (-1)
#define YB_ERR_UNSUPPORTED (-2)
#define YB_ERR_DRIVER (-3)

namespace yb {
char* err_buf();
int fail(int code, const char* fmt, ...);
int check_launch(const char* what);
int sm_count();
int* debug_word_device();
}

#define YB_REQUIRE(cond, ...)                                   \
  do {                                                          \
    if (!(cond)) return yb::fail(YB_ERR_BAD_ARG, __VA_ARGS__);  \
  } while (0)

#define YB_CUDA(expr)                                                                          \
  do {                                                                                         \
    cudaError_t _e = (expr);                                                                   \
    if (_e != cudaSuccess) return yb::fail(static_cast<int>(_e), "%s: %s", #expr, cudaGetErrorString(_e)); \
  } while (0)
```

Before: 18180.

## Chain trunk convolutions with per-row-block dependency counters and PDL overlap

Adds a dependent-launch mode to the implicit-GEMM and wide conv kernels. Producer CTAs publish per-M-block completion counters with release semantics, and consumer launches under programmatic dependent launch wait only on the rows they need. This lets consecutive trunk layers at stride 32 overlap instead of serialising at kernel boundaries. It costs a counter-reset memset per forward, spin-waits in consumer CTAs, and extra templated kernel variants. It also adds an optional tile-timing log.

```diff
diff --git a/include/yolo2_b200.h b/include/yolo2_b200.h
--- a/include/yolo2_b200.h
+++ b/include/yolo2_b200.h
@@ -30,6 +30,7 @@
 const char* yb_last_error(void);
 int yb_debug_read(int out[4]);
 int yb_conv_set_trace(void* dev_buf);
+int yb_conv_set_tile_log(void* dev_buf);
 
 int yb_pack_weight_f16(const float* w_oihw, void* w_f16, int cout, int cin, int ksize, int mode, yb_stream_t stream);
 int yb_bn_fold(const float* gamma, const float* beta, const float* running_mean, const float* running_var, float eps, float* scale,
@@ -50,6 +51,11 @@
 int yb_conv_bn_act_fwd_ws(const void* x, const void* w, const float* scale, const float* shift, float slope, void* y, int batch,
                           int height, int width, int cin, int cout, int ksize, int x_ld, long long y_ld, int y_ch_off, int out_mode,
                           int flags, void* workspace, long long workspace_bytes, yb_stream_t stream);
+int yb_conv_bn_act_dep_fwd(const void* x, const void* w, const float* scale, const float* shift, float slope, void* y, int batch,
+                           int height, int width, int cin, int cout, int ksize, int x_ld, long long y_ld, int y_ch_off, int out_mode,
+                           int flags, void* workspace, long long workspace_bytes, const unsigned* dep_in, unsigned dep_target,
+                           unsigned* dep_out, unsigned* dep_done, yb_stream_t stream);
+int yb_conv_dep_reset(void* counters, long long bytes, yb_stream_t stream);
 int yb_conv_bn_act_split_fwd(const void* x, const void* w_split, const float* scale, const float* shift, float slope, void* y, int batch,
                              int height, int width, int k_channels, int a_channels, int cout, int ksize, int x_ld, long long y_ld,
                              int y_ch_off, int lo_ch_off, int out_mode, int flags, void* workspace, long long workspace_bytes,
diff --git a/yolo2-pytorch_b200/b200/engine.py b/yolo2-pytorch_b200/b200/engine.py
--- a/yolo2-pytorch_b200/b200/engine.py
+++ b/yolo2-pytorch_b200/b200/engine.py
@@ -117,6 +117,7 @@
         self.l3 = torch.empty(batch, h, w, units3[0].cout, **f16)
         self.feature = torch.empty(batch, units3[1].cout, h, w, dtype=torch.float32, device=device)
         self.workspace = ops.conv_workspace(device)
+        self.trunk_deps = None
 
 
 class DarknetEngine(object):
@@ -190,7 +191,36 @@
             u._wver = None
             u._bver = None
 
-    def forward(self, x, conv_flags=0, ref=False, collect=None, plan_id=0):
+    def trunk(self, p):
+        trunk = [(u, p.x1_pool if i == 0 else None, out, {}) for i, (u, out) in enumerate(zip(self.units2[:-1], p.l2))]
+        trunk.append((self.units2[-1], None, p.cat, dict(y_ch_off=self.unit_pt.cout * 4)))
+        trunk.append((self.units3[0], p.cat, p.l3, {}))
+        trunk.append((self.units3[1], p.l3, p.feature, dict(out_mode=ops.OUT_F32_NCHW)))
+        return trunk
+
+    def _trunk_deps(self, p, trunk):
+        if p.trunk_deps is None:
+            b, h, w = p.batch, p.h32, p.w32
+            nt = [ops.chain_n_tiles(b, h, w, u.cin, u.cout, u.ksize, kw.get('out_mode', ops.OUT_F16_NHWC)) for u, _, _, kw in trunk]
+            blocks = (b * h * w + 127) // 128
+            pub = [nt[i] is not None and trunk[i][3].get('out_mode', ops.OUT_F16_NHWC) == ops.OUT_F16_NHWC and i + 1 < len(trunk)
+                   and nt[i + 1] is not None for i in range(len(trunk))]
+            words = sum(blocks for q in pub if q) + sum(1 for i in range(1, len(trunk)) if pub[i - 1])
+            buf = torch.zeros(max(words, 1), dtype=torch.int32, device=p.feature.device)
+            deps, off = [], 0
+            for i in range(len(trunk)):
+                d = {}
+                if pub[i]:
+                    d['dep_out'] = buf[off:off + blocks]
+                    off += blocks
+                if i > 0 and pub[i - 1]:
+                    d.update(dep_in=deps[i - 1]['dep_out'], dep_target=nt[i - 1], dep_done=buf[off:off + 1])
+                    off += 1
+                deps.append(d)
+            p.trunk_deps = (buf if words else None, deps)
+        return p.trunk_deps
+
+    def forward(self, x, conv_flags=0, ref=False, collect=None, plan_id=0, overlap=True):
         if not x.is_cuda:
             raise RuntimeError('Darknet: input must be a CUDA tensor; there is no CPU fallback')
         u8 = x.dtype == torch.uint8
@@ -209,7 +239,13 @@
         def conv(u, src, dst, **kw):
             return ops.conv_bn_act(src, u.w16, u.scale, u.shift, u.slope, out=dst, flags=conv_flags, ref=ref, workspace=p.workspace, **kw)
 
+        trunk = self.trunk(p)
+        counters, deps = None, [{}] * len(trunk)
+        if overlap and collect is None and not ref and conv_flags == 0:
+            counters, deps = self._trunk_deps(p, trunk)
         u0 = self.units1[0]
+        if counters is not None:
+            ops.conv_dep_reset(counters)
         conv0 = ops.conv0_u8_bn_leaky_pool if u8 else ops.conv0_bn_leaky_pool
         cur = conv0(x, u0.w16, u0.scale, u0.shift, u0.slope, out=p.a0)
         if collect is not None:
@@ -233,14 +269,12 @@
             collect['passthrough'] = p.pt
         ops.reorg_f16(p.pt, p.cat, 0)
         cur = ops.maxpool2x2(x1, out=p.x1_pool)
-        for u, out, key in zip(self.units2[:-1], p.l2, self._k2):
-            conv(u, cur, out)
-            if collect is not None:
+        keys = self._k2[:-1] + [None] * 3
+        for (u, src, out, kw), d, key in zip(trunk, deps, keys):
+            conv(u, cur if src is None else src, out, **kw, **d)
+            if collect is not None and key is not None:
                 collect[key] = out
             cur = out
-        conv(self.units2[-1], cur, p.cat, y_ch_off=self.unit_pt.cout * 4)
-        conv(self.units3[0], p.cat, p.l3)
-        conv(self.units3[1], p.l3, p.feature, out_mode=ops.OUT_F32_NCHW)
         if collect is not None:
             collect['cat'] = p.cat
             collect['layers3.0'] = p.l3
diff --git a/yolo2-pytorch_b200/b200/lib.py b/yolo2-pytorch_b200/b200/lib.py
--- a/yolo2-pytorch_b200/b200/lib.py
+++ b/yolo2-pytorch_b200/b200/lib.py
@@ -21,6 +21,10 @@
     'yb_conv_choice': [c_int, c_int, c_int, c_int, c_int, c_int, c_int, c_int, c_int, ctypes.POINTER(c_int * 6)],
     'yb_conv_bn_act_fwd_ws': [P, P, P, P, c_float, P, c_int, c_int, c_int, c_int, c_int, c_int, c_int, c_longlong, c_int, c_int, c_int, P,
                               c_longlong, P],
+    'yb_conv_bn_act_dep_fwd': [P, P, P, P, c_float, P, c_int, c_int, c_int, c_int, c_int, c_int, c_int, c_longlong, c_int, c_int, c_int, P,
+                               c_longlong, P, ctypes.c_uint, P, P, P],
+    'yb_conv_dep_reset': [P, c_longlong, P],
+    'yb_conv_set_tile_log': [P],
     'yb_conv_bn_act_split_fwd': [P, P, P, P, c_float, P, c_int, c_int, c_int, c_int, c_int, c_int, c_int, c_int, c_longlong, c_int, c_int, c_int,
                                  c_int, P, c_longlong, P],
     'yb_pack_weight_split_f16': [P, P, c_int, c_int, c_int, c_int, c_int, P],
diff --git a/yolo2-pytorch_b200/b200/ops.py b/yolo2-pytorch_b200/b200/ops.py
--- a/yolo2-pytorch_b200/b200/ops.py
+++ b/yolo2-pytorch_b200/b200/ops.py
@@ -141,7 +141,8 @@
     return dict(kernel=CONV_KERNELS[out[0]], bk=out[1], bn=out[2], rows=out[3], streamk=bool(out[4]), grid=out[5])
 
 
-def conv_bn_act(x, w, scale, shift, slope, out=None, out_mode=OUT_F16_NHWC, y_ch_off=0, cin=None, flags=0, ref=False, workspace=None):
+def conv_bn_act(x, w, scale, shift, slope, out=None, out_mode=OUT_F16_NHWC, y_ch_off=0, cin=None, flags=0, ref=False, workspace=None,
+                dep_in=None, dep_target=0, dep_out=None, dep_done=None):
     _req(x, torch.float16, 'x'); _req(w, torch.float16, 'w'); _req(scale, torch.float32, 'scale'); _req(shift, torch.float32, 'shift')
     b, h, wd, x_ld = x.shape
     cout, k, _, wcin = w.shape
@@ -158,9 +159,38 @@
     else:
         _req(out, torch.float32, 'out')
         y_ld = 0
+    if dep_in is not None or dep_out is not None:
+        if ref:
+            raise ValueError('conv_bn_act: the CUDA-core reference does not chain')
+        for n, t in (('dep_in', dep_in), ('dep_out', dep_out), ('dep_done', dep_done)):
+            if t is not None:
+                _req(t, torch.int32, n)
+        ws_ptr, ws_bytes = (None, 0) if workspace is None else (_p(_req(workspace, torch.uint8, 'workspace')), workspace.numel())
+        _ck(_l.load().yb_conv_bn_act_dep_fwd(_p(x), _p(w), _p(scale), _p(shift), float(slope), _p(out), b, h, wd, cin, cout, k, x_ld, y_ld, y_ch_off,
+                                             out_mode, flags, ws_ptr, ws_bytes, _p(dep_in), int(dep_target), _p(dep_out), _p(dep_done), _s()),
+            'yb_conv_bn_act_dep_fwd')
+        return out
     _conv_common('yb_conv_ref_fwd' if ref else 'yb_conv_bn_act_fwd', x, w, scale, shift, slope, out, b, h, wd, cin, cout, k, x_ld, y_ld,
                  y_ch_off, out_mode, flags, workspace=None if ref else workspace)
     return out
+
+
+def chain_n_tiles(batch, height, width, cin, cout, k, out_mode=OUT_F16_NHWC, workspace=True):
+    c = conv_choice(batch, height, width, cin, cout, k, out_mode, 0, workspace)
+    if c['streamk'] or c['kernel'] not in ('conv_igemm_kernel', 'conv_wide_kernel'):
+        return None
+    return (cout + c['bn'] - 1) // c['bn']
+
+
+def conv_dep_reset(counters):
+    _req(counters, torch.int32, 'counters')
+    _ck(_l.load().yb_conv_dep_reset(_p(counters), counters.numel() * 4, _s()), 'yb_conv_dep_reset')
+
+
+def conv_set_tile_log(buf):
+    if buf is not None:
+        _req(buf, torch.int64, 'tile log')
+    _l.check(_l.load().yb_conv_set_tile_log(_p(buf)), 'yb_conv_set_tile_log')
 
 
 def conv1x1_preact(x, w, pre_scale, pre_shift, pre_relu, scale, shift, slope, out=None, out_mode=OUT_F16_NHWC, y_ch_off=0, cin=None, flags=0,
diff --git a/yolo2-pytorch_b200/b200/pipeline.py b/yolo2-pytorch_b200/b200/pipeline.py
--- a/yolo2-pytorch_b200/b200/pipeline.py
+++ b/yolo2-pytorch_b200/b200/pipeline.py
@@ -39,7 +39,7 @@
         return slot % self.lanes
 
     def _forward(self, x, plan_id=0):
-        feature = self.engine.forward(x, plan_id=plan_id)
+        feature = self.engine.forward(x, plan_id=plan_id, overlap=self.lanes == 1)
         a = self.anchors.size(0)
         per = feature.size(1) // a
         num_cls = per - 5 if per > 5 else 1
diff --git a/yolo2-pytorch_b200/csrc/capi.cu b/yolo2-pytorch_b200/csrc/capi.cu
--- a/yolo2-pytorch_b200/csrc/capi.cu
+++ b/yolo2-pytorch_b200/csrc/capi.cu
@@ -61,7 +61,7 @@
 long long conv_workspace_bytes();
 int conv_choice(int, int, int, int, int, int, int, int, int, int*);
 int conv_igemm_forward(const void*, const void*, const float*, const float*, float, void*, int, int, int, int, int, int, int, long long,
-                       int, int, int, void*, long long, double*, int, int, const float*, const float*, int, cudaStream_t);
+                       int, int, int, void*, long long, double*, int, int, const float*, const float*, int, const ConvDeps*, cudaStream_t);
 int bn_relu_avgpool2x2(const void*, int, const float*, const float*, void*, int, int, int, int, cudaStream_t);
 int maxpool3x3_s2_ld(const void*, void*, int, int, int, int, int, int, cudaStream_t);
 int pack_weight_split(const float*, void*, int, int, int, int, int, cudaStream_t);
@@ -71,6 +71,7 @@
 int pack_weight(const float*, void*, int, int, int, int, int, cudaStream_t);
 int pack_weights_batch(const void*, int, int, cudaStream_t);
 void conv_set_trace(void*);
+void conv_set_tile_log(void*);
 int bn_fold(const float*, const float*, const float*, const float*, float, float*, float*, int, cudaStream_t);
 int conv0_tc_forward(const void*, int, const float*, const float*, const float*, float, void*, int, int, int, int, int, double*, cudaStream_t);
 int maxpool2x2(const void*, void*, int, int, int, int, int, cudaStream_t);
@@ -172,15 +173,32 @@
                        int height, int width, int cin, int cout, int ksize, int x_ld, long long y_ld, int y_ch_off, int out_mode,
                        int flags, yb_stream_t stream) {
   return yb::conv_igemm_forward(x, w, scale, shift, slope, y, batch, height, width, cin, cout, ksize, x_ld, y_ld, y_ch_off, out_mode,
-                                flags, nullptr, 0, nullptr, 0, -1, nullptr, nullptr, 0, S(stream));
+                                flags, nullptr, 0, nullptr, 0, -1, nullptr, nullptr, 0, nullptr, S(stream));
 }
 
 int yb_conv_bn_act_stats_fwd(const void* x, const void* w, const float* scale, const float* shift, float slope, void* y, int batch,
                              int height, int width, int cin, int cout, int ksize, int x_ld, long long y_ld, int y_ch_off, int flags,
                              double* sums, yb_stream_t stream) {
   return yb::conv_igemm_forward(x, w, scale, shift, slope, y, batch, height, width, cin, cout, ksize, x_ld, y_ld, y_ch_off, 0, flags, nullptr, 0,
-                                sums, 0, -1, nullptr, nullptr, 0, S(stream));
-}
+                                sums, 0, -1, nullptr, nullptr, 0, nullptr, S(stream));
+}
+
+int yb_conv_bn_act_dep_fwd(const void* x, const void* w, const float* scale, const float* shift, float slope, void* y, int batch,
+                           int height, int width, int cin, int cout, int ksize, int x_ld, long long y_ld, int y_ch_off, int out_mode,
+                           int flags, void* workspace, long long workspace_bytes, const unsigned* dep_in, unsigned dep_target,
+                           unsigned* dep_out, unsigned* dep_done, yb_stream_t stream) {
+  const yb::ConvDeps deps{dep_in, dep_target, dep_out, dep_done};
+  return yb::conv_igemm_forward(x, w, scale, shift, slope, y, batch, height, width, cin, cout, ksize, x_ld, y_ld, y_ch_off, out_mode,
+                                flags, workspace, workspace_bytes, nullptr, 0, -1, nullptr, nullptr, 0, &deps, S(stream));
+}
+
+int yb_conv_dep_reset(void* counters, long long bytes, yb_stream_t stream) {
+  if (counters == nullptr || bytes < 0) return yb::fail(YB_ERR_BAD_ARG, "conv_dep_reset: bad buffer");
+  YB_CUDA(cudaMemsetAsync(counters, 0, static_cast<size_t>(bytes), S(stream)));
+  return 0;
+}
+
+int yb_conv_set_tile_log(void* dev_buf) { yb::conv_set_tile_log(dev_buf); return 0; }
 
 long long yb_conv_workspace_bytes(void) { return yb::conv_workspace_bytes(); }
 
@@ -192,7 +210,7 @@
                           int height, int width, int cin, int cout, int ksize, int x_ld, long long y_ld, int y_ch_off, int out_mode,
                           int flags, void* workspace, long long workspace_bytes, yb_stream_t stream) {
   return yb::conv_igemm_forward(x, w, scale, shift, slope, y, batch, height, width, cin, cout, ksize, x_ld, y_ld, y_ch_off, out_mode,
-                                flags, workspace, workspace_bytes, nullptr, 0, -1, nullptr, nullptr, 0, S(stream));
+                                flags, workspace, workspace_bytes, nullptr, 0, -1, nullptr, nullptr, 0, nullptr, S(stream));
 }
 
 int yb_conv_bn_act_split_fwd(const void* x, const void* w_split, const float* scale, const float* shift, float slope, void* y, int batch,
@@ -201,7 +219,7 @@
                              yb_stream_t stream) {
   return yb::conv_igemm_forward(x, w_split, scale, shift, slope, y, batch, height, width, k_channels, cout, ksize, x_ld, y_ld, y_ch_off,
                                 out_mode, flags, workspace, workspace_bytes, nullptr, a_channels, lo_ch_off, nullptr, nullptr, 0,
-                                S(stream));
+                                nullptr, S(stream));
 }
 
 int yb_conv1x1_preact_fwd(const void* x, const void* w, const float* pre_scale, const float* pre_shift, int pre_relu, const float* scale,
@@ -209,7 +227,7 @@
                           int y_ch_off, int out_mode, int flags, void* workspace, long long workspace_bytes, yb_stream_t stream) {
   if (pre_scale == nullptr) return yb::fail(YB_ERR_BAD_ARG, "conv_preact: null pre_scale");
   return yb::conv_igemm_forward(x, w, scale, shift, slope, y, batch, height, width, cin, cout, 1, x_ld, y_ld, y_ch_off, out_mode, flags,
-                                workspace, workspace_bytes, nullptr, 0, -1, pre_scale, pre_shift, pre_relu, S(stream));
+                                workspace, workspace_bytes, nullptr, 0, -1, pre_scale, pre_shift, pre_relu, nullptr, S(stream));
 }
 
 int yb_bn_relu_avgpool2x2_f16(const void* x, int x_ld, const float* scale, const float* shift, void* y, int batch, int height, int width,
diff --git a/yolo2-pytorch_b200/csrc/conv_igemm.cu b/yolo2-pytorch_b200/csrc/conv_igemm.cu
--- a/yolo2-pytorch_b200/csrc/conv_igemm.cu
+++ b/yolo2-pytorch_b200/csrc/conv_igemm.cu
@@ -32,6 +32,11 @@
   int a_wrap;
   long long lo_off;
   int tma_store;
+  unsigned* dep_out;
+  const unsigned* dep_in;
+  unsigned dep_target;
+  unsigned* dep_done;
+  unsigned long long* tile_log;
 };
 
 #define YB_TRACE(role, slot) do { if (p.trace != nullptr && blockIdx.x == 0 && (slot) < 256) p.trace[(role) * 256 + (slot)] = clock64(); } while (0)
@@ -82,6 +87,55 @@
 }
 __device__ __forceinline__ void st_release_gpu(unsigned* p, unsigned v) {
   asm volatile("st.release.gpu.global.u32 [%0], %1;" :: "l"(p), "r"(v) : "memory");
+}
+
+__device__ __forceinline__ void red_release_gpu_add(unsigned* p, unsigned v) {
+  asm volatile("red.release.gpu.global.add.u32 [%0], %1;" :: "l"(p), "r"(v) : "memory");
+}
+__device__ __forceinline__ void fence_proxy_async_global() { asm volatile("fence.proxy.async.global;" ::: "memory"); }
+
+__device__ __forceinline__ void dep_publish(unsigned* dep_out, int blk) {
+  tma_store_wait<0>();
+  fence_proxy_async_global();
+  red_release_gpu_add(dep_out + blk, 1u);
+}
+
+__device__ __forceinline__ void dep_wait_rows(const ConvParams& p, int m0, int rows) {
+  const int halo = p.pad * (p.width + 1);
+  const int lo = m0 - halo > 0 ? m0 - halo : 0;
+  const int hi = m0 + rows + halo < p.m_total ? m0 + rows + halo : p.m_total;
+  for (int b = lo / BM; b * BM < hi; ++b) {
+    uint32_t spins = 0;
+    uint64_t t0 = 0;
+    while (ld_acquire_gpu(p.dep_in + b) < p.dep_target) {
+      if ((++spins & 0x3FFu) == 0) {
+        const uint64_t now = globaltimer_ns();
+        if (t0 == 0) t0 = now;
+        if (now - t0 > 4000000000ull) {
+          if (p.dbg != nullptr) { p.dbg[0] = 0x0BAD0900; p.dbg[1] = static_cast<int>(blockIdx.x); p.dbg[2] = b; p.dbg[3] = m0; __threadfence_system(); }
+          __trap();
+        }
+      }
+    }
+  }
+  fence_proxy_async_global();
+}
+
+__device__ __forceinline__ void dep_finish(const ConvParams& p) {
+  if (atomicAdd(p.dep_done, 1u) == gridDim.x - 1) pdl_wait();
+}
+
+__device__ __forceinline__ bool mbar_test(uint32_t bar, uint32_t parity) {
+  uint32_t ok;
+  asm volatile("{\n\t.reg .pred p;\n\tmbarrier.test_wait.parity.shared::cta.b64 p, [%1], %2;\n\tselp.u32 %0, 1, 0, p;\n\t}"
+               : "=r"(ok) : "r"(bar), "r"(parity) : "memory");
+  return ok != 0;
+}
+
+__device__ __forceinline__ uint32_t smid() {
+  uint32_t v;
+  asm volatile("mov.u32 %0, %%smid;" : "=r"(v));
+  return v;
 }
 
 template <int BN, int BK, int MT, int kPreCh = 0>
@@ -142,7 +196,7 @@
   }
 }
 
-template <int BN, int BK, int MT, bool kPre>
+template <int BN, int BK, int MT, bool kPre, bool kDep>
 __device__ __forceinline__ void conv_igemm_body(const CUtensorMap& tmap_a, const CUtensorMap& tmap_b, const CUtensorMap& tmap_y,
                                                 const ConvParams p, const PreAct pre) {
   using Cfg = ConvCfg<BN, BK, MT, kPre ? kPreMaxCh : 0>;
@@ -185,7 +239,7 @@
   }
   __syncthreads();
   pdl_trigger();
-  pdl_wait();
+  if (!kDep || p.dep_in == nullptr) pdl_wait();
 
   if (warp == kProducerWarp) {
     if (lane == 0) {
@@ -211,6 +265,8 @@
         if (p.skip & 1) nsub = 0;
         if (kMergedA && nsub) nsub = MT;
         const uint32_t tx_bytes = nsub * Cfg::kASubBytes + ((p.skip & 2) ? 0 : Cfg::kBBytes);
+        if (kDep && p.dep_in != nullptr) dep_wait_rows(p, m_cta, Cfg::kRowsPerTile);
+        if (kDep && p.tile_log != nullptr) { p.tile_log[3 * tile] = globaltimer_ns(); p.tile_log[3 * tile + 2] = smid(); }
         for (int kb = it.kb0; kb < it.kb1; ++kb) {
           const int tap = kb / p.kb_per_tap;
           const int c0 = (kb - tap * p.kb_per_tap) * BK;
@@ -456,6 +512,11 @@
               tma_store_2d(&tmap_y, smem_o + q * 4096, n0 + c2 * 64, m_cta + t * BM + q * 32);
               tma_store_commit();
             }
+          }
+          if (kDep && p.dep_out != nullptr) {
+            if (lane == 0) { tma_store_wait<0>(); fence_proxy_async_global(); }
+            asm volatile("bar.sync 1, %0;" :: "n"(kEpiThreads) : "memory");
+            if (et == 0) red_release_gpu_add(p.dep_out + (m_cta + t * BM) / BM, 1u);
           }
           continue;
         }
@@ -566,24 +627,26 @@
         asm volatile("bar.sync 1, %0;" :: "n"(kEpiThreads) : "memory");
         for (int j = sk_lo + et; j < static_cast<int>(blockIdx.x); j += kEpiThreads) p.flags[j] = 0u;
       }
+      if (kDep && p.tile_log != nullptr && et == 0) p.tile_log[3 * tile + 1] = globaltimer_ns();
       acc_phase ^= 1;
     }
     if (p.tma_store && lane == 0) tma_store_wait<0>();
-  }
-}
-
-template <int BN, int BK, int MT>
+    if (kDep && p.dep_in != nullptr && et == 0) dep_finish(p);
+  }
+}
+
+template <int BN, int BK, int MT, bool kDep>
 __global__ void __launch_bounds__(kThreads, 1)
 conv_igemm_kernel(const __grid_constant__ CUtensorMap tmap_a, const __grid_constant__ CUtensorMap tmap_b,
                   const __grid_constant__ CUtensorMap tmap_y, const ConvParams p) {
-  conv_igemm_body<BN, BK, MT, false>(tmap_a, tmap_b, tmap_y, p, PreAct{nullptr, nullptr, 0});
+  conv_igemm_body<BN, BK, MT, false, kDep>(tmap_a, tmap_b, tmap_y, p, PreAct{nullptr, nullptr, 0});
 }
 
 template <int BN, int BK, int MT>
 __global__ void __launch_bounds__(kThreads, 1)
 conv_preact_kernel(const __grid_constant__ CUtensorMap tmap_a, const __grid_constant__ CUtensorMap tmap_b,
                    const __grid_constant__ CUtensorMap tmap_y, const ConvParams p, const PreAct pre) {
-  conv_igemm_body<BN, BK, MT, true>(tmap_a, tmap_b, tmap_y, p, pre);
+  conv_igemm_body<BN, BK, MT, true, false>(tmap_a, tmap_b, tmap_y, p, pre);
 }
 
 constexpr int kWideThreads = 384;
@@ -604,7 +667,7 @@
   static_assert(kStages >= 3, "shared memory budget");
 };
 
-template <int BK>
+template <int BK, bool kDep>
 __global__ void __launch_bounds__(kWideThreads, 1)
 conv_wide_kernel(const __grid_constant__ CUtensorMap tmap_a, const __grid_constant__ CUtensorMap tmap_b,
                  const __grid_constant__ CUtensorMap tmap_y, const ConvParams p) {
@@ -634,7 +697,7 @@
   }
   __syncthreads();
   pdl_trigger();
-  pdl_wait();
+  if (!kDep || p.dep_in == nullptr) pdl_wait();
 
   if (threadIdx.x < 128) {
     setmaxnreg_dec<40>();
@@ -648,6 +711,8 @@
         const int rem = m_cta - img * p.hw;
         const int h0 = rem / p.width;
         const int w0 = rem - h0 * p.width;
+        if (kDep && p.dep_in != nullptr) dep_wait_rows(p, m_cta, kWideRows);
+        if (kDep && p.tile_log != nullptr) { p.tile_log[3 * it.tile] = globaltimer_ns(); p.tile_log[3 * it.tile + 2] = smid(); }
         for (int kb = it.kb0; kb < it.kb1; ++kb) {
           const int tap = kb / p.kb_per_tap;
           const int c0 = (kb - tap * p.kb_per_tap) * BK;
@@ -677,9 +742,11 @@
   float acc[2][64];
   int stage = 0;
   uint32_t phase = 0;
+  int pub_blk = -1;
   for (WorkIter it(p, unit_id, num_units, num_tiles); it.valid(); it.next()) {
     const int kb_first = it.kb0, kb_last = it.kb1 - 1;
     int prev = -1;
+    if (kDep && t == 0 && pub_blk >= 0 && !mbar_test(bar_full + 8 * stage, phase)) { dep_publish(p.dep_out, pub_blk); pub_blk = -1; }
     for (int kb = kb_first; kb <= kb_last; ++kb) {
       mbar_wait(bar_full + 8 * stage, phase, p.dbg, 0x700 | stage);
       const uint64_t bdesc = make_kmajor_desc<Cfg::kSwizzle>(smem_b + stage * Cfg::kBBytes);
@@ -692,6 +759,7 @@
           wgmma_f16<kWideBN>(acc[h], adesc + 2 * k, bdesc + 2 * k, ((kb - kb_first) | k) != 0);
       }
       wgmma_commit();
+      if (kDep && t == 0 && pub_blk >= 0) { dep_publish(p.dep_out, pub_blk); pub_blk = -1; }
       wgmma_wait<1>();
       if (prev >= 0) { __syncwarp(); if (lane == 0) mbar_arrive(bar_empty + 8 * prev); }
       prev = stage;
@@ -787,12 +855,18 @@
         }
       }
     }
+    if (kDep && t == 0 && p.dep_out != nullptr && m_base < p.m_total) pub_blk = m_base / BM;
+    if (kDep && p.tile_log != nullptr && leader) p.tile_log[3 * tile + 1] = globaltimer_ns();
     if (sk_collect) {
       asm volatile("bar.sync 1, 256;" ::: "memory");
       for (int j = sk_lo + t + 128 * cw; j < static_cast<int>(blockIdx.x); j += 256) p.flags[j] = 0u;
     }
   }
-  if (t == 0) tma_store_wait<0>();
+  if (t == 0) {
+    if (kDep && pub_blk >= 0) dep_publish(p.dep_out, pub_blk);
+    else tma_store_wait<0>();
+  }
+  if (kDep && p.dep_in != nullptr && leader) dep_finish(p);
 }
 
 struct C32Params {
@@ -1053,6 +1127,8 @@
 
 static unsigned long long* g_conv_trace = nullptr;
 void conv_set_trace(void* dev_ptr) { g_conv_trace = static_cast<unsigned long long*>(dev_ptr); }
+static unsigned long long* g_tile_log = nullptr;
+void conv_set_tile_log(void* dev_ptr) { g_tile_log = static_cast<unsigned long long*>(dev_ptr); }
 
 typedef CUresult (*EncodeTiledFn)(CUtensorMap*, CUtensorMapDataType, cuuint32_t, void*, const cuuint64_t*, const cuuint64_t*,
                                   const cuuint32_t*, const cuuint32_t*, CUtensorMapInterleave, CUtensorMapSwizzle,
@@ -1089,7 +1165,8 @@
   using PreCfg = ConvCfg<BN, BK, MT, kPreMaxCh>;
   static bool attr_set = false, pre_attr_set = false;
   if (pre == nullptr && !attr_set) {
-    YB_CUDA(cudaFuncSetAttribute(conv_igemm_kernel<BN, BK, MT>, cudaFuncAttributeMaxDynamicSharedMemorySize, Cfg::kSmemBytes));
+    YB_CUDA(cudaFuncSetAttribute(conv_igemm_kernel<BN, BK, MT, false>, cudaFuncAttributeMaxDynamicSharedMemorySize, Cfg::kSmemBytes));
+    YB_CUDA(cudaFuncSetAttribute(conv_igemm_kernel<BN, BK, MT, true>, cudaFuncAttributeMaxDynamicSharedMemorySize, Cfg::kSmemBytes));
     attr_set = true;
   }
   if (pre != nullptr && !pre_attr_set) {
@@ -1102,7 +1179,7 @@
   cudaLaunchAttribute attr[1];
   int nattr = 0;
   static const int use_pdl = getenv("YB_PDL") ? atoi(getenv("YB_PDL")) : 0;
-  if (use_pdl) {
+  if (use_pdl || p.dep_in != nullptr) {
     attr[nattr].id = cudaLaunchAttributeProgrammaticStreamSerialization;
     attr[nattr].val.programmaticStreamSerializationAllowed = 1;
     ++nattr;
@@ -1117,7 +1194,8 @@
     YB_CUDA(cudaLaunchKernelEx(&cfg, conv_preact_kernel<BN, BK, MT>, ta, tb, ty, p, *pre));
     return check_launch("conv_preact_kernel");
   }
-  YB_CUDA(cudaLaunchKernelEx(&cfg, conv_igemm_kernel<BN, BK, MT>, ta, tb, ty, p));
+  if (p.dep_in != nullptr || p.dep_out != nullptr || p.tile_log != nullptr) YB_CUDA(cudaLaunchKernelEx(&cfg, conv_igemm_kernel<BN, BK, MT, true>, ta, tb, ty, p));
+  else YB_CUDA(cudaLaunchKernelEx(&cfg, conv_igemm_kernel<BN, BK, MT, false>, ta, tb, ty, p));
   return check_launch("conv_igemm_kernel");
 }
 
@@ -1126,7 +1204,8 @@
   using Cfg = WideCfg<BK>;
   static bool attr_set = false;
   if (!attr_set) {
-    YB_CUDA(cudaFuncSetAttribute(conv_wide_kernel<BK>, cudaFuncAttributeMaxDynamicSharedMemorySize, Cfg::kSmemBytes));
+    YB_CUDA(cudaFuncSetAttribute(conv_wide_kernel<BK, false>, cudaFuncAttributeMaxDynamicSharedMemorySize, Cfg::kSmemBytes));
+    YB_CUDA(cudaFuncSetAttribute(conv_wide_kernel<BK, true>, cudaFuncAttributeMaxDynamicSharedMemorySize, Cfg::kSmemBytes));
     attr_set = true;
   }
   cudaLaunchConfig_t cfg;
@@ -1134,7 +1213,7 @@
   cudaLaunchAttribute attr[1];
   int nattr = 0;
   static const int use_pdl = getenv("YB_PDL") ? atoi(getenv("YB_PDL")) : 0;
-  if (use_pdl) {
+  if (use_pdl || p.dep_in != nullptr) {
     attr[nattr].id = cudaLaunchAttributeProgrammaticStreamSerialization;
     attr[nattr].val.programmaticStreamSerializationAllowed = 1;
     ++nattr;
@@ -1144,7 +1223,8 @@
   cfg.dynamicSmemBytes = Cfg::kSmemBytes;
   cfg.stream = stream;
   cfg.attrs = attr; cfg.numAttrs = nattr;
-  YB_CUDA(cudaLaunchKernelEx(&cfg, conv_wide_kernel<BK>, ta, tb, ty, p));
+  if (p.dep_in != nullptr || p.dep_out != nullptr || p.tile_log != nullptr) YB_CUDA(cudaLaunchKernelEx(&cfg, conv_wide_kernel<BK, true>, ta, tb, ty, p));
+  else YB_CUDA(cudaLaunchKernelEx(&cfg, conv_wide_kernel<BK, false>, ta, tb, ty, p));
   return check_launch("conv_wide_kernel");
 }
 
@@ -1310,7 +1390,7 @@
 int conv_igemm_forward(const void* x, const void* w, const float* scale, const float* shift, float slope, void* y, int batch,
                        int height, int width, int cin, int cout, int ksize, int x_ld, long long y_ld, int y_ch_off, int out_mode,
                        int flags, void* workspace, long long workspace_bytes, double* stats, int a_channels, int lo_ch_off,
-                       const float* pre_scale, const float* pre_shift, int pre_relu, cudaStream_t stream) {
+                       const float* pre_scale, const float* pre_shift, int pre_relu, const ConvDeps* deps, cudaStream_t stream) {
   YB_REQUIRE(x && w && scale && shift && y, "conv: null pointer");
   const bool pre = pre_scale != nullptr;
   if (pre) {
@@ -1343,6 +1423,14 @@
   int rc = conv_choose(batch, height, width, cin, cout, ksize, a_channels, out_mode, flags, ws_ok, stats != nullptr, lo_ch_off >= 0, pre, &ch);
   if (rc) return rc;
   YB_REQUIRE(!pre || ch.kernel == kKernelIgemm, "conv_preact: no pre-activation form of kernel %d", ch.kernel);
+  const ConvDeps dep = deps != nullptr ? *deps : ConvDeps{nullptr, 0u, nullptr, nullptr};
+  if (dep.dep_in != nullptr || dep.dep_out != nullptr) {
+    YB_REQUIRE((ch.kernel == kKernelIgemm || ch.kernel == kKernelWide) && !ch.streamk && stats == nullptr && !pre && lo_ch_off < 0 &&
+               a_channels == cin && ((flags >> 24) & 0xF) == 0,
+               "conv: a chained launch needs a whole-tile implicit-GEMM conv without stream-K, statistics, split operands or pre-activation");
+    YB_REQUIRE(dep.dep_in == nullptr || (dep.dep_done != nullptr && dep.dep_target > 0), "conv: dep_in needs dep_done and dep_target > 0");
+    YB_REQUIRE(dep.dep_out == nullptr || (out_mode == 0 && ((flags >> 29) & 1) == 0), "conv: dep_out needs the fp16 NHWC TMA-store output");
+  }
   if (ch.kernel == kKernelC32)
     return conv_c32_forward(x, w, scale, shift, slope, y, batch, height, width, cout, x_ld, y_ld, y_ch_off, (flags >> 4) & 1, flags, stats, stream);
   const int bk = ch.bk, bn = ch.bn, mt = ch.mt, streamk = ch.streamk;
@@ -1375,6 +1463,8 @@
   p.a_wrap = a_channels;
   p.lo_off = lo_ch_off >= 0 ? static_cast<long long>(lo_ch_off - y_ch_off) : 0;
   p.sk_base = 0; p.sk_rem = 0; p.ws = nullptr; p.flags = nullptr;
+  p.dep_in = dep.dep_in; p.dep_target = dep.dep_target; p.dep_out = dep.dep_out; p.dep_done = dep.dep_done;
+  p.tile_log = g_tile_log;
   if (streamk) {
     const long long units = static_cast<long long>(p.m_tiles) * p.n_tiles * p.num_kb;
     YB_REQUIRE(units < (1ll << 31), "conv: stream-K unit count overflows");
diff --git a/yolo2-pytorch_b200/csrc/yb_common.h b/yolo2-pytorch_b200/csrc/yb_common.h
--- a/yolo2-pytorch_b200/csrc/yb_common.h
+++ b/yolo2-pytorch_b200/csrc/yb_common.h
@@ -13,6 +13,12 @@
 int check_launch(const char* what);
 int sm_count();
 int* debug_word_device();
+struct ConvDeps {
+  const unsigned* dep_in;
+  unsigned dep_target;
+  unsigned* dep_out;
+  unsigned* dep_done;
+};
 }
 
 #define YB_REQUIRE(cond, ...)                                   \
```

New measurement: 18190 (median of 6 runs). Within noise of the previous version (+0.0%).
